# vocdoni/zk-franchise-proof-circuit

Hardware: AMD Instinct MI355X
Metric: zkCensus proofs/sec (nLevels=160) (higher is better)
Workload: dtype u256 (8 x u32 Montgomery, BN254 Fr/Fq)

## Files before the change

### include/zkcensus.h

```cpp
#ifndef ZKCENSUS_H
#define ZKCENSUS_H
#include <stddef.h>
#include <stdint.h>
#ifdef __cplusplus
extern "C" {
#endif

typedef struct zkc_ctx zkc_ctx;
typedef struct zkc_zkey zkc_zkey;

enum {
    ZKC_OK = 0,
    ZKC_ERR_GENERIC = 1,
    ZKC_ERR_SHORT_BUFFER = 2,
    ZKC_ERR_INVALID_WITNESS_LENGTH = 3,
    ZKC_ERR_BAD_ARG = 4,
    ZKC_ERR_FORMAT = 5,
    ZKC_ERR_HIP = 6,
    ZKC_ERR_WITNESS = 7
};
enum {
    ZKC_W_OK = 0, ZKC_W_ERR_WEIGHT = 1 , ZKC_W_ERR_SIK_ROOT = 2 ,
    ZKC_W_ERR_CENSUS_ROOT = 3 , ZKC_W_ERR_NULLIFIER = 4 , ZKC_W_ERR_LAST_SIBLING = 5 ,
    ZKC_W_ERR_INPUT_RANGE = 6 ,
// ... 70 lines not shown
int groth16_prover(const void* zkey_buffer, unsigned long zkey_size, const void* wtns_buffer, unsigned long wtns_size,
                   char* proof_buffer, unsigned long* proof_size, char* public_buffer, unsigned long* public_size,
                   char* error_msg, unsigned long error_msg_maxsize);

int groth16_fullprove(const void* zkey_buffer, unsigned long zkey_size, const void* wasm_buffer, unsigned long wasm_size, const char* inputs_json, unsigned long inputs_size,
                      char* proof_buffer, unsigned long* proof_size, char* public_buffer, unsigned long* public_size,
                      char* error_msg, unsigned long error_msg_maxsize);

int zkc_verify(const char* vkey_json, const char* public_json, const char* proof_json);
int zkc_verify_bin(const uint8_t* vk, int nPublic, const uint8_t* pub, const uint8_t* proof);

int zkc_pairing_bin(const uint8_t g1[64], const uint8_t g2[128], uint8_t out[384]);

int zkc_verify_batch(zkc_ctx* ctx, const uint8_t* vk, int nPublic, const uint8_t* pubs, const uint8_t* proofs, int N, const uint8_t* seed32);
const char* zkc_verify_last_error(void);

int zkc_proof_to_json(const uint8_t proof[256], const uint8_t* pub, int nPublic, char* proof_buf, unsigned long* proof_size,
                      char* public_buf, unsigned long* public_size);
int zkc_proof_from_json(const char* proof_json, const char* public_json, uint8_t proof[256], uint8_t* pub, int* nPublic);
int zkc_vkey_from_json(const char* vkey_json, uint8_t* vk, unsigned long* vk_size, int* nPublic);
int zkc_wtns_parse(const void* wtns_bytes, unsigned long size, const uint8_t** payload, uint32_t* nWitness);
unsigned long zkc_wtns_write(const void* payload, uint32_t nWitness, void* out, unsigned long out_size);

typedef struct zkc_msm zkc_msm;
int zkc_ntt_dev(zkc_ctx* ctx, const void* d_src, void* d_dst, int logn, int nvec, int inverse);
int zkc_g1_mul_batch_dev(zkc_ctx* ctx, const uint8_t base_std[64], const void* d_scalars, uint32_t n, void* d_out);
int zkc_msm_g1_load_dev(zkc_ctx* ctx, const void* d_bases_std, uint32_t n, zkc_msm** out);
int zkc_msm_g1_dev(zkc_msm* m, const void* d_scalars, uint8_t out[64]);
void zkc_msm_g1_free(zkc_msm* m);

int zkc_debug_stage(zkc_zkey* zk, const void* d_wtns, int stage, void* host_out);
unsigned long long zkc_debug_early_retries(void);
int zkc_msm_debug(zkc_zkey* zk, int which, const void* d_scalars, uint32_t count, void* host_out);
int zkc_debug_pairing_dev(zkc_ctx* ctx, const uint8_t* g1, const uint8_t* g2, const uint8_t* weights, int N, uint8_t product_out[384], uint8_t* folded_out,
                          int32_t* member_out, int* bad_out, const uint32_t* nodes, size_t count, uint8_t* node_out);

int zkc_poseidon_batch(zkc_ctx* ctx, int n_inputs, const void* inputs, size_t B, void* out);
int zkc_smt_build(zkc_ctx* ctx, const void* keys, const void* values, size_t n, int nLevels, uint8_t root[32], void* siblings, int32_t* depths);
int zkc_census_inputs(zkc_ctx* ctx, size_t n, int nLevels, const uint8_t election_id[64], const void* address, const void* password, const void* signature,
                      const void* available_weight, const void* vote_weight, const void* vote_hash, void* inputs_out, void* d_inputs_out, uint8_t* roots_out);

typedef struct zkc_tree zkc_tree;
enum {
    ZKC_TREE_OK = 0,
    ZKC_TREE_KEY_EXISTS = 1,
    ZKC_TREE_KEY_ABSENT = 2,
    ZKC_TREE_COLLISION = 3,
    ZKC_TREE_NOT_BELOW_R = 4,
    ZKC_TREE_NOT_IN_CENSUS = 5,
    ZKC_TREE_NOT_IN_SIK = 6,
    ZKC_TREE_SIK_MISMATCH = 7
};
int  zkc_tree_create(zkc_ctx* ctx, int nLevels, zkc_tree** out);
void zkc_tree_free(zkc_tree* tree);
int  zkc_tree_add(zkc_tree* tree, const void* keys, const void* values, size_t n, int32_t* status);
int  zkc_tree_update(zkc_tree* tree, const void* keys, const void* values, size_t n, int32_t* status);
int  zkc_tree_root(zkc_tree* tree, uint8_t root[32]);
int  zkc_tree_size(zkc_tree* tree, size_t* leaves);
int  zkc_tree_get(zkc_tree* tree, const void* keys, size_t n, void* values_out, int32_t* exists);
int  zkc_tree_gen_proof(zkc_tree* tree, const void* keys, size_t n, uint8_t root[32], void* siblings, int32_t* depths, int32_t* exists);
int  zkc_tree_census_inputs(zkc_tree* census, zkc_tree* sik, size_t n, const uint8_t election_id[64], const void* address, const void* password, const void* signature,
                            const void* vote_weight, const void* vote_hash, void* inputs_out, void* d_inputs_out, uint8_t roots_out[64], int32_t* status);
int  zkc_tree_stats(zkc_tree* tree, double ms[2]);

enum {
    ZKC_SMT_VALID = 0,
// ... 30 lines not shown
```

### zk-franchise-proof-circuit_amd/_native.py

```python
import ctypes
import os

_HERE = os.path.dirname(os.path.abspath(__file__))
LIB_PATH = os.environ.get('ZKCENSUS_LIB') or os.path.join(_HERE, 'libzkcensus.so')
_lib = None


class ZkcError(RuntimeError):
    def __init__(self, code, msg):
        super().__init__('libzkcensus error %d: %s' % (code, msg))
        self.code = code


def load():
    global _lib
    if _lib is not None:
        return _lib
    if not os.path.exists(LIB_PATH):
        raise ImportError('libzkcensus.so is not built (run `python -c "import __graft_entry__ as g; g.build()"`); '
                          'there is no CPU fallback for the product path')
    try:
        import torch
    except ImportError:
        pass
    L = ctypes.CDLL(LIB_PATH)
    vp, i32p = ctypes.c_void_p, ctypes.POINTER(ctypes.c_int32)
    L.zkc_ctx_create.argtypes = [ctypes.c_int, ctypes.POINTER(vp)]
    L.zkc_ctx_destroy.argtypes = [vp]
    L.zkc_last_error.argtypes = [vp]; L.zkc_last_error.restype = ctypes.c_char_p
    L.zkc_ctx_stream.argtypes = [vp]; L.zkc_ctx_stream.restype = vp
    L.zkc_witness.argtypes = [vp, ctypes.c_int, vp, ctypes.c_int, vp, i32p]
    L.zkc_witness_dev.argtypes = [vp, ctypes.c_int, vp, ctypes.c_int, vp, vp]
    u8p, u32p = ctypes.c_char_p, ctypes.POINTER(ctypes.c_uint32)
    L.zkc_zkey_load.argtypes = [vp, ctypes.c_char_p, ctypes.c_size_t, ctypes.POINTER(vp)]
    L.zkc_zkey_free.argtypes = [vp]; L.zkc_zkey_free.restype = None
    L.zkc_zkey_info.argtypes = [vp, u32p, u32p, u32p]
    L.zkc_zkey_pass_info.argtypes = [vp, ctypes.POINTER(ctypes.c_int), ctypes.POINTER(ctypes.c_int)]
    L.zkc_zkey_call_streams.argtypes = [vp, ctypes.POINTER(ctypes.c_int)]
    L.zkc_witness_status_text.argtypes = [ctypes.c_int, ctypes.c_int32]; L.zkc_witness_status_text.restype = ctypes.c_char_p
    L.zkc_prove.argtypes = [vp, ctypes.c_char_p, ctypes.c_uint32, u8p, u8p, ctypes.c_char_p, ctypes.c_char_p]
    L.zkc_prove_dev.argtypes = [vp, vp, ctypes.c_uint32, u8p, u8p, ctypes.c_char_p, ctypes.c_char_p]
    L.zkc_prove_batch_dev.argtypes = [vp, vp, ctypes.c_uint32, ctypes.c_int, ctypes.c_char_p, ctypes.c_char_p, ctypes.c_char_p]
    L.zkc_fullprove_batch_dev.argtypes = [vp, vp, ctypes.c_int, vp, vp, ctypes.c_char_p, ctypes.c_char_p, ctypes.c_char_p]
    L.zkc_debug_stage.argtypes = [vp, vp, ctypes.c_int, ctypes.c_char_p]
    L.zkc_debug_early_retries.argtypes = []; L.zkc_debug_early_retries.restype = ctypes.c_ulonglong
    L.zkc_msm_debug.argtypes = [vp, ctypes.c_int, vp, ctypes.c_uint32, ctypes.c_char_p]
    L.zkc_debug_pairing_dev.argtypes = [vp, ctypes.c_char_p, ctypes.c_char_p, ctypes.c_char_p, ctypes.c_int, ctypes.c_char_p, ctypes.c_char_p, i32p, ctypes.POINTER(ctypes.c_int),
                                        ctypes.POINTER(ctypes.c_uint32), ctypes.c_size_t, ctypes.c_char_p]
    ulp = ctypes.POINTER(ctypes.c_ulong)
    L.groth16_prover.argtypes = [ctypes.c_char_p, ctypes.c_ulong, ctypes.c_char_p, ctypes.c_ulong, ctypes.c_char_p, ulp, ctypes.c_char_p, ulp, ctypes.c_char_p, ctypes.c_ulong]
    L.zkc_verify.argtypes = [ctypes.c_char_p, ctypes.c_char_p, ctypes.c_char_p]
    L.zkc_verify_bin.argtypes = [ctypes.c_char_p, ctypes.c_int, ctypes.c_char_p, ctypes.c_char_p]
    L.zkc_verify_batch.argtypes = [vp, ctypes.c_char_p, ctypes.c_int, ctypes.c_char_p, ctypes.c_char_p, ctypes.c_int, ctypes.c_char_p]
    L.zkc_verify_batch_each.argtypes = [vp, ctypes.c_char_p, ctypes.c_int, ctypes.c_char_p, ctypes.c_char_p, ctypes.c_int, ctypes.c_char_p, i32p]
    L.zkc_verify_each_stats.argtypes = [vp, ctypes.POINTER(ctypes.c_uint64)]
    L.zkc_verify_last_error.restype = ctypes.c_char_p
    L.zkc_proof_to_json.argtypes = [ctypes.c_char_p, ctypes.c_char_p, ctypes.c_int, ctypes.c_char_p, ulp, ctypes.c_char_p, ulp]
    L.zkc_proof_from_json.argtypes = [ctypes.c_char_p, ctypes.c_char_p, ctypes.c_char_p, ctypes.c_char_p, ctypes.POINTER(ctypes.c_int)]
    L.zkc_vkey_from_json.argtypes = [ctypes.c_char_p, ctypes.c_char_p, ulp, ctypes.POINTER(ctypes.c_int)]
    L.zkc_wtns_parse.argtypes = [ctypes.c_char_p, ctypes.c_ulong, ctypes.POINTER(ctypes.c_void_p), ctypes.POINTER(ctypes.c_uint32)]
    L.zkc_wtns_write.argtypes = [ctypes.c_char_p, ctypes.c_uint32, ctypes.c_char_p, ctypes.c_ulong]; L.zkc_wtns_write.restype = ctypes.c_ulong
    L.zkc_poseidon_batch.argtypes = [vp, ctypes.c_int, ctypes.c_char_p, ctypes.c_size_t, ctypes.c_char_p]
    L.zkc_smt_build.argtypes = [vp, ctypes.c_char_p, ctypes.c_char_p, ctypes.c_size_t, ctypes.c_int, ctypes.c_char_p, ctypes.c_char_p, i32p]
    L.zkc_census_inputs.argtypes = [vp, ctypes.c_size_t, ctypes.c_int, ctypes.c_char_p, ctypes.c_char_p, ctypes.c_char_p, ctypes.c_char_p, ctypes.c_char_p, ctypes.c_char_p, ctypes.c_char_p, vp, vp, ctypes.c_char_p]
    sz = ctypes.c_size_t
    L.zkc_tree_create.argtypes = [vp, ctypes.c_int, ctypes.POINTER(vp)]
    L.zkc_tree_free.argtypes = [vp]; L.zkc_tree_free.restype = None
    L.zkc_tree_add.argtypes = [vp, ctypes.c_char_p, ctypes.c_char_p, sz, i32p]
    L.zkc_tree_update.argtypes = [vp, ctypes.c_char_p, ctypes.c_char_p, sz, i32p]
    L.zkc_tree_delete.argtypes = [vp, ctypes.c_char_p, sz, i32p]
    L.zkc_tree_refs.argtypes = [vp, ctypes.POINTER(sz)]
    L.zkc_tree_snapshot.argtypes = [vp, ctypes.POINTER(vp)]
    L.zkc_tree_snapshot_count.argtypes = [vp, ctypes.POINTER(sz)]
    L.zkc_tree_gen_absence_proof.argtypes = [vp, ctypes.c_char_p, sz, ctypes.c_char_p, vp, i32p, vp, vp, i32p, i32p]
    L.zkc_tree_root.argtypes = [vp, ctypes.c_char_p]
    L.zkc_tree_size.argtypes = [vp, ctypes.POINTER(sz)]
    L.zkc_tree_get.argtypes = [vp, ctypes.c_char_p, sz, vp, i32p]
    L.zkc_tree_gen_proof.argtypes = [vp, ctypes.c_char_p, sz, ctypes.c_char_p, vp, i32p, i32p]
    L.zkc_tree_census_inputs.argtypes = [vp, vp, sz, ctypes.c_char_p, ctypes.c_char_p, ctypes.c_char_p, ctypes.c_char_p, ctypes.c_char_p, ctypes.c_char_p, vp, vp, ctypes.c_char_p, i32p]
# ... 88 lines not shown
```

### zk-franchise-proof-circuit_amd/csrc/zkc_fold.hip

```cpp
#include "zkc_prover.h"
#include "zkc_host_util.h"
#include "zkc_kernels.h"
#include <ctime>
#include <cstdio>
#include <algorithm>

using namespace zkc;

extern "C" __global__ void __launch_bounds__(64)
zkc_fold_check(WitnessLayout L, const uint32_t* __restrict__ wtns, const uint32_t* __restrict__ tmpl, uint32_t* __restrict__ flags, int B, int stride) {
    const int n = L.n, g = blockIdx.x, tree = blockIdx.y, b = blockIdx.z;
    const int blk = tree == 0 ? L.off_census : L.off_sikver;
    int start, end;
    if (g < n - 1) {
        const int nctrl = (g == n - 3) + (g > 0 && g < n - 2) + 1;
        start = blk + L.lvl_off(g) + nctrl; end = blk + (g + 1 < n - 1 ? L.lvl_off(g + 1) : L.lvl_off(n - 1));
    } else { start = blk + L.off_n2bold; end = start + 253 + 127 + 133; }
    const uint4* w = reinterpret_cast<const uint4*>(wtns + (size_t)b * L.nWires * 8) + 2 * (size_t)start;
    const uint4* t = reinterpret_cast<const uint4*>(tmpl) + 2 * (size_t)start;
    uint32_t diff = 0;
    for (int i = threadIdx.x; i < 2 * (end - start); i += 64) { uint4 x = w[i], y = t[i]; diff |= (x.x ^ y.x) | (x.y ^ y.y) | (x.z ^ y.z) | (x.w ^ y.w); }
    if (g == n - 1 && tree == 0 && threadIdx.x < 2) {
        const uint4 x = reinterpret_cast<const uint4*>(wtns + (size_t)b * L.nWires * 8)[threadIdx.x], y = reinterpret_cast<const uint4*>(tmpl)[threadIdx.x];
        diff |= (x.x ^ y.x) | (x.y ^ y.y) | (x.z ^ y.z) | (x.w ^ y.w);
    }
    const unsigned long long any = __ballot(diff != 0);
    if (threadIdx.x == 0) flags[(size_t)b * stride + (size_t)tree * n + g] = any ? 1u : 0u;
}

extern "C" __global__ void __launch_bounds__(256)
zkc_top_check(TopCheckArgs a, const uint32_t* __restrict__ wtns, uint32_t* __restrict__ flags, int stride, int off) {
    __shared__ uint32_t s_valid;
    const int tree = blockIdx.x, b = blockIdx.y;
    const uint32_t* w = wtns + (size_t)b * a.nWires * 8;
    uint32_t h = 2166136261u;
// ... 215 lines not shown
    zkc_ctx* ctx = zk->ctx; const uint32_t nv = zk->nVars, np = zk->nPub;
    std::vector<uint32_t> v; zkc_zkey::Fold::VMap m;
    m.offA = 0; for (uint32_t w = 0; w < nv; w++) if (!zk->fold.infA[w]) v.push_back(w); m.nA = (uint32_t)v.size();
    m.offB = (uint32_t)v.size(); for (uint32_t w = 0; w < nv; w++) if (!zk->fold.infB[w]) v.push_back(w); m.nB = (uint32_t)v.size() - m.offB;
    m.offC = (uint32_t)v.size(); for (uint32_t w = np + 1; w < nv; w++) if (!zk->fold.infC[w]) v.push_back(w); m.nC = (uint32_t)v.size() - m.offC;
    if ((size_t)m.nA + m.nB + m.nC + (size_t)nv / 50 < 3 * (size_t)nv - np - 1) {
        if (int rc = list_upload(ctx, v, ctx->stream, &m.d)) return rc;
    }
    zk->fold.vmaps[{-1, -1, -1, -1}] = m; *out = m;
    return ZKC_OK;
}

int zkc::abc_template(zkc_zkey* zk, const uint32_t* tmpl) {
    if (zk->fold.d_abc_tmpl) return ZKC_OK;
    zkc_ctx* ctx = zk->ctx; const uint32_t n = zk->n; Fr *d_abc = nullptr, *d_wm = nullptr; int rc;
    if ((rc = dmalloc(ctx, &d_abc, 3 * (size_t)n))) return rc;
    if ((rc = dmalloc(ctx, &d_wm, 3 * (size_t)n))) { (void)hipFree(d_abc); return rc; }
    matvec_launch(zk, d_abc, d_wm, tmpl, 1, ctx->stream);
    hipError_t e = hipGetLastError(); if (e == hipSuccess) e = hipStreamSynchronize(ctx->stream);
    (void)hipFree(d_wm);
    if (e != hipSuccess) { (void)hipFree(d_abc); return zkc_fail(ctx, ZKC_ERR_HIP, std::string("abc_template: ") + hipGetErrorString(e)); }
    zk->fold.d_abc_tmpl = d_abc;
    return ZKC_OK;
}
int zkc::abc_rows(zkc_zkey* zk, int Dc, int Ds, zkc_zkey::Fold::AbcRows* out) {
    auto& f = zk->fold;
    auto it = f.abc_rows.find({Dc, Ds});
    if (it != f.abc_rows.end()) { *out = it->second; return ZKC_OK; }
    zkc_ctx* ctx = zk->ctx;
    const abc::VoterRows v = abc::voter_rows(f.abc_cls, f.abc_perm.data(), zk->nlong, zk->n, f.abc_rowptr.data(), f.abc_col.data(), zk->nVars, Dc, Ds);
    zkc_zkey::Fold::AbcRows m; m.nrows = (uint32_t)v.rows.size(); m.nlong = v.nlong; m.offC = m.nrows; m.nC = (uint32_t)v.crows.size(); m.offW = m.offC + m.nC; m.nW = (uint32_t)v.wires.size();
    std::vector<uint32_t> all(v.rows); all.insert(all.end(), v.crows.begin(), v.crows.end()); all.insert(all.end(), v.wires.begin(), v.wires.end());
    if (int rc = list_upload(ctx, all, ctx->stream, &m.d)) return rc;
    if (sw::on<sw::ZKC_TRACE_HOST>()) fprintf(stderr, "[zkc host] abc rows at depths (%d, %d): %u of %zu A/B rows listed (%u long), %u C rows, %u wires\n", Dc, Ds, m.nrows, f.abc_cls.size(), m.nlong, m.nC, m.nW);
    f.abc_rows[{Dc, Ds}] = m; *out = m;
    return ZKC_OK;
}
void zkc::fold_free(zkc_zkey* zk) {
    for (auto& kv : zk->fold.vmaps) if (kv.second.d) (void)hipFree(kv.second.d);
    for (auto& kv : zk->fold.abc_rows) if (kv.second.d) (void)hipFree(kv.second.d);
    if (zk->fold.d_abc_tmpl) (void)hipFree(zk->fold.d_abc_tmpl);
    { auto& tp = zk->fold.top; for (void* q : {(void*)tp.d_copy[0], (void*)tp.d_copy[1], (void*)tp.d_valid, (void*)tp.d_A, (void*)tp.d_B1, (void*)tp.d_C, (void*)tp.d_B2}) if (q) (void)hipFree(q); }
    for (void* q : {(void*)zk->fold.d_foldA, (void*)zk->fold.d_foldB1, (void*)zk->fold.d_foldC, (void*)zk->fold.d_foldB2}) if (q) (void)hipFree(q);
}
```

### zk-franchise-proof-circuit_amd/csrc/zkc_kernels.h

```cpp
#pragma once
#include "zkc_field.h"
#include "zkc_curve.h"
#include "zkc_device.h"
#include "zkc_jds.h"

namespace zkc {

__device__ __forceinline__ Fr ld_fr(const Fr* p) {
    const uint4* d = reinterpret_cast<const uint4*>(p); uint4 a = d[0], b = d[1];
    Fr r; r.v[0] = a.x; r.v[1] = a.y; r.v[2] = a.z; r.v[3] = a.w; r.v[4] = b.x; r.v[5] = b.y; r.v[6] = b.z; r.v[7] = b.w; return r;
}
__device__ __forceinline__ void st_fr(Fr* p, const Fr& r) {
    uint4* d = reinterpret_cast<uint4*>(p);
    d[0] = make_uint4(r.v[0], r.v[1], r.v[2], r.v[3]); d[1] = make_uint4(r.v[4], r.v[5], r.v[6], r.v[7]);
}
__device__ __forceinline__ Fr mv_term(const Fr* __restrict__ val, const Fr* __restrict__ w, const Fr* __restrict__ wm, uint32_t idx, uint32_t c) {
    if (wm && (c & MV_UNIT)) { const Fr x = ld_fr(wm + (c & MV_COL)); return (c & MV_NEG) ? fp_neg(x) : x; }
    return ld_fr(val + idx) * ld_fr(w + (c & MV_COL));
}

extern "C" __global__ void zkc_wtns_mont(const Fr* wtns_std, size_t wtns_stride, Fr* wm, size_t wm_stride, uint32_t nv);
extern "C" __global__ void zkc_wtns_mont_list(const Fr* wtns_std, size_t wtns_stride, Fr* wm, size_t wm_stride, const uint32_t* list, uint32_t nlist);
extern "C" __global__ void zkc_abc_fill(const uint4* tmpl, uint4* abc, uint32_t per);
extern "C" __global__ void zkc_matvec_jds(const uint32_t* perm, const uint32_t* rowlen, const uint32_t* jdptr, const uint32_t* col, const Fr* val, const Fr* wtns_std,
                                          size_t wtns_stride, Fr* abc, int n, uint32_t nlong, const Fr* wm_all, size_t wm_stride, const uint32_t* list, uint32_t nrows);
extern "C" __global__ void zkc_pointwise_mul(Fr* abc, int n, const uint32_t* list, uint32_t count);
extern "C" __global__ void zkc_join_abc(const Fr* abc, uint32_t* p_std, int n);

struct TopCheckArgs;
extern "C" __global__ void zkc_fold_check(WitnessLayout L, const uint32_t* wtns, const uint32_t* tmpl, uint32_t* flags, int B, int stride);
extern "C" __global__ void zkc_top_check(TopCheckArgs a, const uint32_t* wtns, uint32_t* flags, int stride, int off);
extern "C" __global__ void zkc_input_depths(const uint32_t* inputs, int nInputs, int n, uint32_t* out);

extern "C" __global__ void zkc_witness_chains(WitnessLayout L, PoseidonTable tab, const uint32_t* inputs, uint32_t* wtns, int32_t* status, int B, int tmpl_mode);
extern "C" __global__ void zkc_witness_chains_wave(WitnessLayout L, PoseidonTable tab, const uint32_t* inputs, uint32_t* wtns, int32_t* status, int B, int tmpl_mode);
extern "C" __global__ void zkc_witness_fill(const uint4* tmpl, uint4* wtns, int nWires, int B);
extern "C" __global__ void zkc_witness_tostd(uint32_t* wtns, size_t nwires_total);
extern "C" __global__ void zkc_poseidon_batch_kernel(PoseidonTable tab, const uint32_t* in, uint32_t* out, int nin, size_t B);

extern "C" __global__ void zkc_census_hash(PoseidonTable tab, int kind, const uint32_t* a, const uint32_t* b, const uint32_t* c, uint32_t* out, size_t n);
extern "C" __global__ void zkc_tree_leaves(PoseidonTable tab, const uint32_t* slot, const uint32_t* key, const uint32_t* value, uint32_t count, uint32_t* val);
extern "C" __global__ void zkc_tree_level(PoseidonTable tab, const uint32_t* trip, uint32_t count, uint32_t* val);
extern "C" __global__ void zkc_tree_narrow(PoseidonTable tab, const uint32_t* trip, const uint32_t* off, uint32_t ndepths, uint32_t count, uint32_t* val);
extern "C" __global__ void zkc_census_scatter(const uint32_t* val, const uint2* pairs, size_t count, uint32_t* out);
extern "C" __global__ void zkc_census_scalars(const uint32_t* eid, const uint32_t* nullifier, const uint32_t* avail, const uint32_t* vhash, const uint32_t* sik_root,
                                              const uint32_t* census_root, const uint32_t* address, const uint32_t* password, const uint32_t* signature,
                                              const uint32_t* vweight, size_t n, int nIn, uint32_t* out);

extern "C" __global__ void zkc_smt_check(PoseidonTable tab, const uint32_t* keys, const uint32_t* values, const uint32_t* roots, uint32_t root_stride, const uint32_t* off,
                                         const uint32_t* sib, uint32_t count, int32_t* status);
extern "C" __global__ void zkc_smt_check_wave(PoseidonTable tab, const uint32_t* keys, const uint32_t* values, const uint32_t* roots, uint32_t root_stride,
                                              const uint32_t* off, const uint32_t* sib, uint32_t count, int32_t* status);
extern "C" __global__ void zkc_smt_check_absent(PoseidonTable tab, const uint32_t* keys, const uint32_t* old_keys, const uint32_t* values, const uint32_t* old0,
                                                const uint32_t* roots, uint32_t root_stride, const uint32_t* off, const uint32_t* sib, uint32_t count, int32_t* status);
extern "C" __global__ void zkc_smt_check_absent_wave(PoseidonTable tab, const uint32_t* keys, const uint32_t* old_keys, const uint32_t* values, const uint32_t* old0,
                                                     const uint32_t* roots, uint32_t root_stride, const uint32_t* off, const uint32_t* sib, uint32_t count, int32_t* status);

extern "C" __global__ void zkc_r1cs_range(const Fr* wtns_std, size_t wtns_stride, uint32_t nWires, uint32_t* flag);
extern "C" __global__ void zkc_r1cs_check_rows(const uint4* rows, const uint32_t* jdptr, const uint32_t* col, const Fr* val, const Fr* wtns_std, size_t wtns_stride,
                                               const Fr* wm_all, size_t wm_stride, uint32_t nCons, uint32_t nlong, uint32_t* first, uint32_t* count, const uint32_t* flag);
// ... 3 lines not shown
```

### zk-franchise-proof-circuit_amd/csrc/zkc_msm.hip

```cpp
#include <cstdio>
#include <cstddef>
#include <ctime>
#include <cstdlib>
#include <cstring>
#include <string.h>
#include <vector>
#include "zkc_prover.h"
#include "zkc_f29.h"
#include "zkc_f29_g1.h"
#include "zkc_f29_g2.h"
#include "zkc_point_ops.h"

namespace zkc {

template <class F> struct PointIO;
template <class PP> struct PointIO<Fp<PP>> {
    typedef Fp<PP> Fq;
    static __device__ __forceinline__ Affine<Fq> load(const Affine<Fq>* p) {
        const uint4* d = reinterpret_cast<const uint4*>(p); uint4 a = d[0], b = d[1], c = d[2], e = d[3];
        Affine<Fq> r;
        r.x.v[0] = a.x; r.x.v[1] = a.y; r.x.v[2] = a.z; r.x.v[3] = a.w; r.x.v[4] = b.x; r.x.v[5] = b.y; r.x.v[6] = b.z; r.x.v[7] = b.w;
        r.y.v[0] = c.x; r.y.v[1] = c.y; r.y.v[2] = c.z; r.y.v[3] = c.w; r.y.v[4] = e.x; r.y.v[5] = e.y; r.y.v[6] = e.z; r.y.v[7] = e.w;
        return r;
    }
// ... 381 lines not shown
        if (!b.is_inf()) Sk = f29g2_pt_from_xyzz(b);
    }
    sh[threadIdx.x] = Sk; __syncthreads();
    for (int o = 1; o < nt; o <<= 1) {
        Acc29G2 v; f29g2_pt_set_inf(v);
        if ((int)threadIdx.x + o < nt) v = sh[threadIdx.x + o];
        __syncthreads();
        if ((int)threadIdx.x + o < nt) { Acc29G2 t = sh[threadIdx.x]; f29g2_pt_add(t, t, v); sh[threadIdx.x] = t; }
        __syncthreads();
    }
    Acc29G2 y; f29g2_pt_set_inf(y);
    if (threadIdx.x >= 1 && (int)threadIdx.x < nt) { y = sh[threadIdx.x]; if (!f29g2_pt_is_inf(y)) for (uint32_t k = vw; k > 1; k >>= 1) f29g2_pt_dbl(y, y); }
    f29g2_pt_add(y, y, Wk);
    __syncthreads();
    sh[threadIdx.x] = y; __syncthreads();
    for (int st = nt / 2; st > 0; st >>= 1) {
        if ((int)threadIdx.x < st) { Acc29G2 t = sh[threadIdx.x]; f29g2_pt_add(t, t, sh[threadIdx.x + st]); sh[threadIdx.x] = t; }
        __syncthreads();
    }
    if (threadIdx.x == 0) results[j] = f29g2_pt_is_inf(sh[0]) ? XYZZ<Fq2>::inf() : f29g2_pt_to_xyzz(sh[0]);
}

template <class F>
__global__ void __launch_bounds__(128)
zkc_msm_shift_bases(const Affine<F>* __restrict__ prev, Affine<F>* __restrict__ next, uint32_t count, int c) {
    const uint32_t i = blockIdx.x * blockDim.x + threadIdx.x;
    if (i >= count) return;
    Affine<F> a = PointIO<F>::load(prev + i);
    XYZZ<F> p = xyzz_dbl_affine(a);
    for (int k = 1; k < c; k++) p = xyzz_dbl(p);
    next[i] = xyzz_to_affine(p);
}
template <class F>
static int precompute(zkc_ctx* ctx, uint32_t count, Affine<F>* d_table, int c) {
    for (int w = 1; w < msm_nw(c); w++) {
        hipLaunchKernelGGL(HIP_KERNEL_NAME(zkc_msm_shift_bases<F>), dim3((count + 127) / 128), dim3(128), 0, ctx->stream,
                           d_table + (size_t)(w - 1) * count, d_table + (size_t)w * count, count, c);
        hipError_t e = hipGetLastError();
        if (e != hipSuccess) return zkc_fail(ctx, ZKC_ERR_HIP, std::string("zkc_msm_shift_bases: ") + hipGetErrorString(e));
    }
    return ZKC_OK;
}
int msm_precompute_g1(zkc_ctx* ctx, uint32_t count, G1Affine* d_table, int c) { return precompute<Fq>(ctx, count, d_table, c); }
int msm_precompute_g2(zkc_ctx* ctx, uint32_t count, G2Affine* d_table, int c) { return precompute<Fq2>(ctx, count, d_table, c); }
int msm_g2_rows29(zkc_ctx* ctx, const G2Affine* d_points, size_t n, const char* what, uint32_t** out) {
    DevBuf rows; int rc;
    if ((rc = rows.alloc(ctx, n * G2ROW_WORDS * sizeof(uint32_t))) || (rc = msm_g2_table29(ctx, d_points, rows.as<uint32_t>(), n))) return rc;
    const hipError_t e = hipStreamSynchronize(ctx->stream);
    if (e != hipSuccess) return zkc_fail(ctx, ZKC_ERR_HIP, std::string(what) + ": " + hipGetErrorString(e));
    *out = (uint32_t*)rows.release();
    return ZKC_OK;
}
int msm_g2_window_table29(zkc_ctx* ctx, const G2Affine* d_bases, uint32_t count, int c, const char* what, uint32_t** out) {
    const size_t n = (size_t)msm_nw(c) * count;
    DevBuf shifted; int rc;
    if ((rc = shifted.alloc(ctx, n * sizeof(G2Affine)))) return rc;
    const hipError_t e = hipMemcpyAsync(shifted.p, d_bases, (size_t)count * sizeof(G2Affine), hipMemcpyDeviceToDevice, ctx->stream);
    if (e != hipSuccess) return zkc_fail(ctx, ZKC_ERR_HIP, std::string(what) + ": " + hipGetErrorString(e));
    if ((rc = msm_precompute_g2(ctx, count, shifted.as<G2Affine>(), c))) return rc;
    return msm_g2_rows29(ctx, shifted.as<G2Affine>(), n, what, out);
}

__device__ __forceinline__ uint32_t limb_of(const uint32_t k[8], int i) {
    uint32_t w = 0;
#pragma unroll
    for (int q = 0; q < 8; q++) w = (q == i) ? k[q] : w;
    return w;
}
template <class F>
__global__ void __launch_bounds__(64)
zkc_fold_mul(const Affine<F>* __restrict__ tbl, const uint32_t* __restrict__ scalars, const uint32_t* __restrict__ wires, uint32_t nw,
             int32_t pt_shift, XYZZ<F>* __restrict__ out, uint32_t pt_mod) {
    const uint32_t i = blockIdx.x * blockDim.x + threadIdx.x;
    if (i >= nw) return;
    const uint32_t wire = wires[i];
    const uint4* sp = reinterpret_cast<const uint4*>(scalars + 8 * (size_t)wire); uint4 a = sp[0], b = sp[1];
// ... 8 lines not shown
        if ((limb_of(k, bit >> 5) >> (bit & 31)) & 1) r = xyzz_add_affine(r, p);
    }
    out[i] = r;
}
template <class F>
__global__ void __launch_bounds__(64)
zkc_fold_gsum(const XYZZ<F>* __restrict__ in, const uint32_t* __restrict__ gstart, uint32_t ngroups, XYZZ<F>* __restrict__ out) {
    const uint32_t g = blockIdx.x * blockDim.x + threadIdx.x;
    if (g >= ngroups) return;
    XYZZ<F> acc = XYZZ<F>::inf();
    for (uint32_t i = gstart[g], e = gstart[g + 1]; i < e; i++) acc = xyzz_add(acc, in[i]);
    out[g] = acc;
}
template <class F>
static int fold_group_sums_ws(zkc_ctx* ctx, const Affine<F>* tbl, const uint32_t* d_scalars, const uint32_t* d_wires, uint32_t nw, int32_t pt_shift,
                              const uint32_t* d_gstart, uint32_t ngroups, XYZZ<F>* tmp, XYZZ<F>* out, XYZZ<F>* h_out, uint32_t pt_mod, hipStream_t st) {
    hipLaunchKernelGGL(HIP_KERNEL_NAME(zkc_fold_mul<F>), dim3((nw + 63) / 64), dim3(64), 0, st, tbl, d_scalars, d_wires, nw, pt_shift, tmp, pt_mod);
    ZKC_HIP_CHECK(ctx, hipGetLastError());
    hipLaunchKernelGGL(HIP_KERNEL_NAME(zkc_fold_gsum<F>), dim3((ngroups + 63) / 64), dim3(64), 0, st, tmp, d_gstart, ngroups, out);
    ZKC_HIP_CHECK(ctx, hipGetLastError());
    ZKC_HIP_CHECK(ctx, hipMemcpyAsync(h_out, out, (size_t)ngroups * sizeof(XYZZ<F>), hipMemcpyDeviceToHost, st));
    ZKC_HIP_CHECK(ctx, hipStreamSynchronize(st));
    return ZKC_OK;
}
template <class F>
static int fold_group_sums(zkc_ctx* ctx, const Affine<F>* tbl, const uint32_t* d_scalars, const uint32_t* d_wires, uint32_t nw, int32_t pt_shift,
                           const uint32_t* d_gstart, uint32_t ngroups, XYZZ<F>* h_out, uint32_t pt_mod, hipStream_t st) {
    DevBuf tmp, out; int rc;
    if ((rc = tmp.alloc(ctx, (size_t)nw * sizeof(XYZZ<F>))) || (rc = out.alloc(ctx, (size_t)ngroups * sizeof(XYZZ<F>)))) return rc;
    return fold_group_sums_ws<F>(ctx, tbl, d_scalars, d_wires, nw, pt_shift, d_gstart, ngroups, tmp.as<XYZZ<F>>(), out.as<XYZZ<F>>(), h_out, pt_mod, st ? st : ctx->stream);
}
int fold_group_sums_g1(zkc_ctx* ctx, const G1Affine* tbl, const uint32_t* s, const uint32_t* w, uint32_t nw, int32_t sh, const uint32_t* gs, uint32_t ng, G1XYZZ* o, uint32_t pt_mod, hipStream_t st) {
    return fold_group_sums<Fq>(ctx, tbl, s, w, nw, sh, gs, ng, o, pt_mod, st);
}
int fold_group_sums_g1_ws(zkc_ctx* ctx, const G1Affine* tbl, const uint32_t* s, const uint32_t* w, uint32_t nw, const uint32_t* gs, uint32_t ng, G1XYZZ* d_tmp, G1XYZZ* d_out, G1XYZZ* h_out) {
    return fold_group_sums_ws<Fq>(ctx, tbl, s, w, nw, 0, gs, ng, d_tmp, d_out, h_out, 0u, ctx->stream);
}
int fold_group_sums_g2(zkc_ctx* ctx, const G2Affine* tbl, const uint32_t* s, const uint32_t* w, uint32_t nw, int32_t sh, const uint32_t* gs, uint32_t ng, G2XYZZ* o, uint32_t pt_mod, hipStream_t st) {
    return fold_group_sums<Fq2>(ctx, tbl, s, w, nw, sh, gs, ng, o, pt_mod, st);
}

static int msm_work_alloc_impl(zkc_ctx* ctx, MsmWork& w, size_t max_entries, size_t max_buckets, int max_jobs, bool g2) {
    w.max_entries = max_entries; w.max_jobs = max_jobs; w.max_buckets = max_buckets; w.xyzz_size = g2 ? sizeof(G2XYZZ) : sizeof(G1XYZZ);
    const size_t nb = max_buckets;
    w.max_segments = std::max<size_t>(max_entries / MSM_SEG + 1, (size_t)32 * 8192) + nb + 64;
    w.max_bins = (size_t)max_jobs << MSM_MAX_HBITS;
    ZKC_HIP_CHECK(ctx, hipMalloc((void**)&w.vals, max_entries * 4 + 16)); ZKC_HIP_CHECK(ctx, hipMalloc((void**)&w.vals2, max_entries * 4 + 16));
    ZKC_HIP_CHECK(ctx, hipMalloc((void**)&w.hist, w.max_bins * 4)); ZKC_HIP_CHECK(ctx, hipMalloc((void**)&w.bin_start, w.max_bins * 4));
    w.max_tilecnt = max_entries / 8 + ((size_t)max_jobs << MSM_MAX_HBITS);
    ZKC_HIP_CHECK(ctx, hipMalloc((void**)&w.tilecnt, w.max_tilecnt * 4));
    ZKC_HIP_CHECK(ctx, hipMalloc((void**)&w.off, (nb + 2) * 4)); ZKC_HIP_CHECK(ctx, hipMalloc((void**)&w.bcnt, (nb + 2) * 4)); ZKC_HIP_CHECK(ctx, hipMalloc((void**)&w.segcnt, (nb + 2) * 4));
    ZKC_HIP_CHECK(ctx, hipMalloc((void**)&w.segoff, (nb + 2) * 4)); ZKC_HIP_CHECK(ctx, hipMalloc((void**)&w.seg2bucket, w.max_segments * 4));
    ZKC_HIP_CHECK(ctx, hipMalloc((void**)&w.seglen, w.max_segments * 4)); ZKC_HIP_CHECK(ctx, hipMalloc((void**)&w.perm, w.max_segments * 4));
    w.max_lencnt = (size_t)(MSM_SEG + 1) * (w.max_segments / 256 + 2);
    ZKC_HIP_CHECK(ctx, hipMalloc((void**)&w.lencnt, w.max_lencnt * 4));
    ZKC_HIP_CHECK(ctx, hipMalloc((void**)&w.scan_blk, (std::max(nb + 2, w.max_lencnt) / 1024 + 2) * 4));
    ZKC_HIP_CHECK(ctx, hipMalloc((void**)&w.heavy, (MSM_MAX_HEAVY + 1) * 4));
    ZKC_HIP_CHECK(ctx, hipMalloc((void**)&w.d_jobs, sizeof(MsmJobList)));
    ZKC_HIP_CHECK(ctx, hipMalloc(&w.partial, w.max_segments * w.xyzz_size));
    const size_t max_vw = max_buckets / MSM_VW_MIN + (size_t)max_jobs;
    ZKC_HIP_CHECK(ctx, hipMalloc(&w.wres, 2 * max_vw * w.xyzz_size));
    ZKC_HIP_CHECK(ctx, hipMalloc((void**)&w.d_windows, max_vw * sizeof(MsmWindow))); w.max_windows = max_vw;
    w.max_tiles = max_entries / (8 * MSM_TILE_SCALARS) + (size_t)max_jobs + 1;
    ZKC_HIP_CHECK(ctx, hipMalloc((void**)&w.d_tilejob, w.max_tiles * 2));
    for (int s = 0; s < 2; s++) {
        ZKC_HIP_CHECK(ctx, hipHostMalloc((void**)&w.h_tilejob[s], w.max_tiles * 2));
// ... 22 lines not shown
static const bool g_debug_sync = sw::on<sw::ZKC_DEBUG_SYNC>();
#define ZKC_LAUNCH_CHECK(ctx, name)                                                                        \
    do { hipError_t _e = hipGetLastError(); if (_e != hipSuccess)                                          \
        return zkc_fail((ctx), ZKC_ERR_HIP, std::string(name ": ") + hipGetErrorString(_e));               \
        if (g_debug_sync) { timespec _t0, _t1; clock_gettime(CLOCK_MONOTONIC, &_t0);                        \
            _e = hipStreamSynchronize(st); clock_gettime(CLOCK_MONOTONIC, &_t1);                \
            fprintf(stderr, "[zkc] %-22s %8.3f ms  %s\n", name, (_t1.tv_sec - _t0.tv_sec) * 1e3 + (_t1.tv_nsec - _t0.tv_nsec) * 1e-6, \
                    hipGetErrorString(_e)); fflush(stderr); } } while (0)

template <class F>
static int msm_pass(zkc_zkey* zk, MsmWork& w, const Affine<F>* table, const MsmJobList& jl_in, int slot, bool to_host, hipStream_t st, hipEvent_t ev_sorted, hipEvent_t wait_before_acc = nullptr, hipEvent_t ev_acc = nullptr,
                    hipStream_t st_red = nullptr, hipEvent_t ev_red = nullptr) {
    zkc_ctx* ctx = zk->ctx;
    const int nj = jl_in.njobs;
    if (nj <= 0 || nj > w.max_jobs) return zkc_fail(ctx, ZKC_ERR_BAD_ARG, "msm_pass: job count");
    static thread_local MsmJobList jl;
    jl = jl_in;
    if (!jl.finish()) {
        std::string d = "msm_pass: jobs need at most two window sizes (the larger first) and tables that fit the entry word [" + std::to_string(nj) + " jobs:";
        for (int j = 0; j < nj && j < 16; j++) d += " c" + std::to_string(jl.job[j].c) + "/" + std::to_string(jl.job[j].count) + "/" + std::to_string(jl.job[j].tbl_count);
        return zkc_fail(ctx, ZKC_ERR_BAD_ARG, d + "]");
    }
    const size_t total = jl.total_entries;
    const uint32_t nb = jl.total_buckets;
    if (total > w.max_entries || nb > w.max_buckets) return zkc_fail(ctx, ZKC_ERR_BAD_ARG, "msm_pass: too many entries for the work space");
    const uint32_t seg = (uint32_t)std::min<size_t>(MSM_SEG, std::max<size_t>(MSM_SEG_MIN, total / 131072));
    typedef typename GroupOf<F>::Ops G; constexpr bool kG2 = GroupOf<F>::g2;
    const uint32_t bw_slices = (uint32_t)std::min<size_t>(32, w.max_segments / std::max<uint32_t>(nb, 1u));
    const uint32_t* const g2_table29 = (kG2 && jl.job[0].c == (uint32_t)MSM_C_G2_LONE) ? zk->d_g2_29_lone : (kG2 && zk->c_deep && jl.job[0].c == (uint32_t)zk->c_deep) ? zk->d_g2_29_deep : zk->d_g2_29;
    const bool bucket_wave = kG2 && sw::on<sw::ZKC_G2_BUCKET_WAVE>() && nb <= 8192 && bw_slices >= 1;
    uint64_t alg_bytes = 0; uint32_t maxcount = 0;
    uint64_t streamed_bytes = 0;
    for (int j = 0; j < nj; j++) {
        alg_bytes += (uint64_t)jl.job[j].tbl_count * (sizeof(Affine<F>) + 32);
        streamed_bytes += (uint64_t)jl.job[j].count * (sizeof(Affine<F>) + 32);
        maxcount = std::max(maxcount, jl.job[j].count);
    }
    const size_t seg_bound = total / seg + nb;
    if (!bucket_wave && seg_bound > w.max_segments) return zkc_fail(ctx, ZKC_ERR_BAD_ARG, "msm_pass: more segments than the work space holds");
    {
        zkc_prof_scope _ps(ctx, ZKC_PROF_MSM_SORT, 0, st);
        if (jl.total_windows > w.max_windows) return zkc_fail(ctx, ZKC_ERR_BAD_ARG, "msm_pass: too many virtual windows for the work space");
        const int hs = w.h_next; w.h_next ^= 1;
        ZKC_HIP_CHECK(ctx, zkc_wait_event(w.h_ev[hs]));
        MsmWindow* wins = w.h_windows[hs]; uint32_t nwin = 0;
        for (int j = 0; j < nj; j++) for (uint32_t k = 0; k < (uint32_t)msm_half((int)jl.job[j].c) / jl.job[j].vw; k++)
            wins[nwin++] = MsmWindow{jl.id_of(k * jl.job[j].vw, (uint32_t)j), jl.job[j].win_off + k, jl.job[j].vw / 64};
        memcpy(w.h_jobs[hs], &jl, offsetof(MsmJobList, job) + (size_t)nj * sizeof(MsmJob)); w.h_jobs[hs]->njobs = jl.njobs;
        memcpy(&w.h_jobs[hs]->njobs, &jl.njobs, sizeof(MsmJobList) - offsetof(MsmJobList, njobs));
        ZKC_HIP_CHECK(ctx, hipMemcpyAsync(w.d_jobs, w.h_jobs[hs], sizeof(MsmJobList), hipMemcpyHostToDevice, st));
        ZKC_HIP_CHECK(ctx, hipMemcpyAsync(w.d_windows, wins, (size_t)nwin * sizeof(MsmWindow), hipMemcpyHostToDevice, st));
        if (jl.total_tiles > w.max_tiles) return zkc_fail(ctx, ZKC_ERR_BAD_ARG, "msm_pass: too many tiles for the work space");
        { uint16_t* tj = w.h_tilejob[hs]; uint32_t k = 0; for (int j = 0; j < nj; j++) { const uint32_t nt = (jl.job[j].count + MSM_TILE_SCALARS - 1) / MSM_TILE_SCALARS; for (uint32_t i = 0; i < nt; i++) tj[k++] = (uint16_t)j; } }
        ZKC_HIP_CHECK(ctx, hipMemcpyAsync(w.d_tilejob, w.h_tilejob[hs], (size_t)jl.total_tiles * 2, hipMemcpyHostToDevice, st));
        ZKC_HIP_CHECK(ctx, hipEventRecord(w.h_ev[hs], st));
        unsigned long long* ectr = (!kG2 && ((ctx->prof.mask >> ZKC_PROF_MSM_ACC_G1) & 1)) ? ctx->d_prof_entries : nullptr;
        int rc = msm_bucket_entries(ctx, w, jl, st, ectr); if (rc) return rc;
        if (g_debug_sync) { hipError_t _e = hipStreamSynchronize(st); fprintf(stderr, "[zkc] bucket entries: %s\n", hipGetErrorString(_e)); }
        if (!bucket_wave) { rc = msm_build_segments(ctx, w, jl, seg, seg_bound, st); if (rc) return rc; }
        if (g_debug_sync) { hipError_t _e = hipStreamSynchronize(st); fprintf(stderr, "[zkc] segments: %s\n", hipGetErrorString(_e)); }
        if (ev_sorted) ZKC_HIP_CHECK(ctx, hipEventRecord(ev_sorted, st));
    }
    XYZZ<F>* partial = reinterpret_cast<XYZZ<F>*>(w.partial);
    XYZZ<F>* wres = reinterpret_cast<XYZZ<F>*>(w.wres);
    XYZZ<F>* results = reinterpret_cast<XYZZ<F>*>(w.results) + (size_t)slot * w.max_jobs;
    if (wait_before_acc) ZKC_HIP_CHECK(ctx, hipStreamWaitEvent(st, wait_before_acc, 0));
    const bool acc_chain = !kG2 && sw::on<sw::ZKC_ACC_CHAIN>() && total >= ((size_t)1 << 22);
// ... 66 lines not shown
```

### zk-franchise-proof-circuit_amd/csrc/zkc_ntt.hip

```cpp
#include "zkc_internal.h"
#include "zkc_prover.h"
#include "zkc_f29.h"
#include "zkc_host_util.h"
#include "zkc_kernels.h"

namespace zkc {

extern "C" __global__ void __launch_bounds__(256)
zkc_wtns_mont(const Fr* __restrict__ wtns_std, size_t wtns_stride, Fr* __restrict__ wm, size_t wm_stride, uint32_t nv) {
    const uint32_t i = blockIdx.x * blockDim.x + threadIdx.x;
    if (i >= nv) return;
    Fr r2;
#pragma unroll
    for (int k = 0; k < 8; k++) r2.v[k] = FrParams::r2[k];
    st_fr(wm + (size_t)blockIdx.y * wm_stride + i, ld_fr(wtns_std + (size_t)blockIdx.y * wtns_stride + i) * r2);
}
extern "C" __global__ void __launch_bounds__(256)
zkc_wtns_mont_list(const Fr* __restrict__ wtns_std, size_t wtns_stride, Fr* __restrict__ wm, size_t wm_stride, const uint32_t* __restrict__ list, uint32_t nlist) {
    const uint32_t e = blockIdx.x * blockDim.x + threadIdx.x;
    if (e >= nlist) return;
    const uint32_t i = list[e];
    Fr r2;
#pragma unroll
    for (int k = 0; k < 8; k++) r2.v[k] = FrParams::r2[k];
    st_fr(wm + (size_t)blockIdx.y * wm_stride + i, ld_fr(wtns_std + (size_t)blockIdx.y * wtns_stride + i) * r2);
}
extern "C" __global__ void __launch_bounds__(256)
zkc_abc_fill(const uint4* __restrict__ tmpl, uint4* __restrict__ abc, uint32_t per) {
    uint4* __restrict__ dst = abc + (size_t)blockIdx.y * per;
    for (uint32_t i = blockIdx.x * blockDim.x + threadIdx.x; i < per; i += gridDim.x * blockDim.x) dst[i] = tmpl[i];
}
extern "C" __global__ void __launch_bounds__(256)
zkc_matvec_jds(const uint32_t* __restrict__ perm, const uint32_t* __restrict__ rowlen, const uint32_t* __restrict__ jdptr,
               const uint32_t* __restrict__ col, const Fr* __restrict__ val, const Fr* __restrict__ wtns_std, size_t wtns_stride,
               Fr* __restrict__ abc, int n, uint32_t nlong, const Fr* __restrict__ wm_all, size_t wm_stride, const uint32_t* __restrict__ list, uint32_t nrows) {
    const uint32_t t = blockIdx.x * blockDim.x + threadIdx.x, lane = threadIdx.x & 63u;
    const Fr* __restrict__ w = wtns_std + (size_t)blockIdx.y * wtns_stride;
    const Fr* __restrict__ wm = wm_all ? wm_all + (size_t)blockIdx.y * wm_stride : nullptr;
    Fr acc = Fr::zero();
    if ((t >> 6) < nlong) {
        const uint32_t r = list ? list[t >> 6] : t >> 6, len = rowlen[r];
        for (uint32_t k = lane; k < len; k += 64) { const uint32_t idx = jdptr[k] + r; acc = acc + mv_term(val, w, wm, idx, col[idx]); }
        for (int d = 32; d > 0; d >>= 1) {
            Fr o;
#pragma unroll
            for (int i = 0; i < 8; i++) o.v[i] = (uint32_t)__shfl_down((int)acc.v[i], d, 64);
            acc = acc + o;
        }
        if (lane == 0) st_fr(abc + (size_t)blockIdx.y * 3 * n + perm[r], acc);
        return;
    }
    const uint32_t e = t - nlong * 63u;
    if (e >= nrows) return;
    const uint32_t r = list ? list[e] : e;
    const uint32_t len = rowlen[r];
    for (uint32_t k = 0; k < len; k++) { const uint32_t idx = jdptr[k] + r; acc = acc + mv_term(val, w, wm, idx, col[idx]); }
    st_fr(abc + (size_t)blockIdx.y * 3 * n + perm[r], acc);
}
extern "C" __global__ void __launch_bounds__(256)
zkc_pointwise_mul(Fr* __restrict__ abc, int n, const uint32_t* __restrict__ list, uint32_t count) {
    const uint32_t e = blockIdx.x * blockDim.x + threadIdx.x;
    Fr* a = abc + (size_t)blockIdx.y * 3 * n;
    if (e >= count) return;
    const uint32_t i = list ? list[e] : e;
    st_fr(a + 2 * (size_t)n + i, ld_fr(a + i) * ld_fr(a + n + i));
}
struct JoinDom { static constexpr L9 D27 = f29_dominator<FrParams>(1u << 29, 1u << 27); };
extern "C" __global__ void __launch_bounds__(256)
zkc_join_abc(const Fr* __restrict__ abc, uint32_t* __restrict__ p_std, int n) {
    const int i = blockIdx.x * blockDim.x + threadIdx.x;
    if (i >= n) return;
    const Fr* a = abc + (size_t)blockIdx.y * 3 * n;
    const Fr av = ld_fr(a + i), bv = ld_fr(a + n + i), cv = ld_fr(a + 2 * (size_t)n + i);
    uint32_t A[9], B[9], C[9], T[9];
    f29_from_fp_shl5(A, av.v); f29_from_fp_shl5(B, bv.v); f29_from_fp_shl5(C, cv.v);
#pragma unroll
    for (int k = 0; k < 9; k++) C[k] = JoinDom::D27.l[k] - C[k];
    f29_mul_addhi<FrParams>(T, A, B, C);
    uint64_t col[18];
#pragma unroll
    for (int k = 0; k < 9; k++) { col[k] = T[k]; col[9 + k] = 0; }
    f29_reduce_cols<FrParams>(T, col);
    Fr r;
    r.v[0] = f29_word<0>(T); r.v[1] = f29_word<32>(T); r.v[2] = f29_word<64>(T); r.v[3] = f29_word<96>(T);
    r.v[4] = f29_word<128>(T); r.v[5] = f29_word<160>(T); r.v[6] = f29_word<192>(T); r.v[7] = f29_word<224>(T);
    fp_reduce_once<FrParams>(r.v);
    uint4* d = reinterpret_cast<uint4*>(p_std + 8 * ((size_t)blockIdx.y * n + i));
    d[0] = make_uint4(r.v[0], r.v[1], r.v[2], r.v[3]); d[1] = make_uint4(r.v[4], r.v[5], r.v[6], r.v[7]);
}

constexpr int NTT_TILE = 1024;
constexpr int TW29_WORDS = 12;
extern "C" __global__ void __launch_bounds__(256) zkc_tw29(const Fr* __restrict__ tw, uint32_t* __restrict__ out, uint32_t count) {
    const uint32_t i = blockIdx.x * blockDim.x + threadIdx.x;
    if (i >= count) return;
    const Fr x = ld_fr(tw + i);
    uint32_t t[9], r[9]; f29_from_fp_shl5(t, x.v); f29_mul<FrParams>(r, t, F29K<FrParams>::one.l);
    uint4* o = reinterpret_cast<uint4*>(out + (size_t)TW29_WORDS * i);
    o[0] = make_uint4(r[0], r[1], r[2], r[3]); o[1] = make_uint4(r[4], r[5], r[6], r[7]); o[2] = make_uint4(r[8], 0, 0, 0);
}
struct NttDom { static constexpr L9 D24 = f29_dominator<FrParams>(1u << 29, 1u << 24); static constexpr L9 D27 = f29_dominator<FrParams>(1u << 29, 1u << 27); };
__device__ __forceinline__ void ntt_ld_w(uint32_t w[9], const uint32_t* __restrict__ tw29, size_t e) {
    const uint4* wp = reinterpret_cast<const uint4*>(tw29 + (size_t)TW29_WORDS * e);
    const uint4 w0 = wp[0], w1 = wp[1], w2 = wp[2];
    w[0] = w0.x; w[1] = w0.y; w[2] = w0.z; w[3] = w0.w; w[4] = w1.x; w[5] = w1.y; w[6] = w1.z; w[7] = w1.w; w[8] = w2.x;
}
__device__ __forceinline__ void ntt_bfly(uint32_t* pu, uint32_t* pv, const uint32_t w[9], bool plain, bool carry) {
    uint32_t u[9], v[9], tt[9];
#pragma unroll
    for (int i = 0; i < 9; i++) { u[i] = pu[i]; v[i] = pv[i]; }
    if (plain) {
#pragma unroll
        for (int i = 0; i < 9; i++) { const uint32_t vi = v[i]; v[i] = u[i] + NttDom::D27.l[i] - vi; u[i] += vi; }
    } else {
        f29_mul<FrParams>(tt, v, w);
#pragma unroll
        for (int i = 0; i < 9; i++) { v[i] = u[i] + NttDom::D24.l[i] - tt[i]; u[i] += tt[i]; }
    }
    if (carry) { f29_carry(u); f29_carry(v); }
#pragma unroll
    for (int i = 0; i < 9; i++) { pu[i] = u[i]; pv[i] = v[i]; }
}
__device__ __forceinline__ void ntt_r4(uint32_t* p0, uint32_t* p1, uint32_t* p2, uint32_t* p3, const uint32_t wa[9], const uint32_t wb[9], const uint32_t wc[9], bool swap_mid) {
    uint32_t a[9], b[9], c[9], d[9], t[9];
#pragma unroll
    for (int i = 0; i < 9; i++) { a[i] = p0[i]; b[i] = p1[i]; c[i] = p2[i]; d[i] = p3[i]; }
    f29_mul<FrParams>(t, b, wa);
#pragma unroll
    for (int i = 0; i < 9; i++) { b[i] = a[i] + NttDom::D24.l[i] - t[i]; a[i] += t[i]; }
    f29_mul<FrParams>(t, d, wa);
#pragma unroll
    for (int i = 0; i < 9; i++) { d[i] = c[i] + NttDom::D24.l[i] - t[i]; c[i] += t[i]; }
    f29_mul<FrParams>(t, c, wb);
#pragma unroll
    for (int i = 0; i < 9; i++) { c[i] = a[i] + NttDom::D24.l[i] - t[i]; a[i] += t[i]; }
    f29_mul<FrParams>(t, d, wc);
#pragma unroll
    for (int i = 0; i < 9; i++) { d[i] = b[i] + NttDom::D24.l[i] - t[i]; b[i] += t[i]; }
    f29_carry(a); f29_carry(b); f29_carry(c); f29_carry(d);
    (void)swap_mid;
#pragma unroll
    for (int i = 0; i < 9; i++) { p0[i] = a[i]; p1[i] = b[i]; p2[i] = c[i]; p3[i] = d[i]; }
}
extern "C" __global__ void __launch_bounds__(256)
zkc_ntt_pass(const Fr* src_all, Fr* dst_all, const uint32_t* __restrict__ tw29, const Fr* __restrict__ scale,
             int logn, int s0, int b, int first) {
    const Fr* src = src_all + ((size_t)blockIdx.y << logn);
    Fr* dst = dst_all + ((size_t)blockIdx.y << logn);
    extern __shared__ uint32_t tile[];
    const int mid_n = 1 << b;
    const int lo_bits = s0;
    const int lo_t = (NTT_TILE >> b) < (1 << lo_bits) ? (NTT_TILE >> b) : (1 << lo_bits);
    const int tiles_per_hi = (1 << lo_bits) / lo_t;
    const int hi = blockIdx.x / tiles_per_hi, lo0 = (blockIdx.x % tiles_per_hi) * lo_t;
    const int elems = mid_n * lo_t;
    const size_t base = (size_t)hi << (s0 + b);
    for (int e = threadIdx.x; e < elems; e += blockDim.x) {
        const int mid = e / lo_t, l = e - mid * lo_t;
        size_t gi = base + ((size_t)mid << s0) + lo0 + l;
        if (first) gi = __brev((unsigned)gi) >> (32 - logn);
        const Fr x = ld_fr(src + gi);
        uint32_t t[9]; f29_from_fp_shl5(t, x.v);
#pragma unroll
        for (int k = 0; k < 9; k++) tile[9 * e + k] = t[k];
    }
    __syncthreads();
    int t = 1;
    auto single = [&](int t1, bool carry) {
        const int half = 1 << (t1 - 1);
        const int s = s0 + t1;
        for (int q = threadIdx.x; q < elems / 2; q += blockDim.x) {
            const int l = q % lo_t, pr = q / lo_t;
            const int j = pr & (half - 1), blk = pr >> (t1 - 1);
            const int m0 = (blk << t1) + j, m1 = m0 + half;
            const unsigned k = ((unsigned)j << s0) + lo0 + l;
            uint32_t w[9]; ntt_ld_w(w, tw29, (size_t)k << (logn - s));
            ntt_bfly(tile + 9 * (m0 * lo_t + l), tile + 9 * (m1 * lo_t + l), w, s == 1, carry);
        }
        __syncthreads();
    };
    if (s0 == 0) { single(1, true); t = 2; }
// ... 38 lines not shown
            uint32_t w[9] = {0, 0, 0, 0, 0, 0, 0, 0, 0};
            ntt_bfly(tile + 9 * slot(j, l), tile + 9 * slot(j + span, l), w, true, true);
        }
        __syncthreads();
        r = 1;
    }
    for (; RADIX >= 4 && r + 1 < b; r += 2) {
        const int q = q0 + r, span = mid_n >> (r + 1), hspan = span >> 1, units = (mid_n >> 2) * lo_t;
        for (int x = threadIdx.x; x < units; x += blockDim.x) {
            const int l = x % lo_t, u = x / lo_t;
            const int blk = u / hspan, j = u - blk * hspan;
            const int m = blk * 2 * span + j;
            const uint32_t i = ((prefix_of_l0 + (uint32_t)(prefix_per_l * l)) << r) | (uint32_t)blk;
            uint32_t wa[9], wb[9], wc[9];
            ntt_ld_w(wa, tw29, tw_of(q, i)); ntt_ld_w(wb, tw29, tw_of(q + 1, 2 * i)); ntt_ld_w(wc, tw29, tw_of(q + 1, 2 * i + 1));
            ntt_r4(tile + 9 * slot(m, l), tile + 9 * slot(m + span, l), tile + 9 * slot(m + hspan, l), tile + 9 * slot(m + span + hspan, l), wa, wb, wc, false);
        }
        __syncthreads();
    }
    for (; r < b; r++) {
        const int q = q0 + r, span = mid_n >> (r + 1), pairs = (mid_n >> 1) * lo_t;
        for (int x = threadIdx.x; x < pairs; x += blockDim.x) {
            const int l = x % lo_t, pr = x / lo_t;
            const int blk = pr / span, j = pr - blk * span;
            const int m0 = blk * 2 * span + j;
            const uint32_t i = ((prefix_of_l0 + (uint32_t)(prefix_per_l * l)) << r) | (uint32_t)blk;
            uint32_t w[9]; ntt_ld_w(w, tw29, tw_of(q, i));
            ntt_bfly(tile + 9 * slot(m0, l), tile + 9 * slot(m0 + span, l), w, false, RADIX >= 4 || (r & 1) == 1 || r == b - 1);
        }
        __syncthreads();
    }
}
template <int RADIX>
__device__ __forceinline__ void ntt_nr_head_body(const Fr* src_all, Fr* dst_all, const uint32_t* __restrict__ tw29, int logn, int q0, int b) {
    const Fr* src = src_all + ((size_t)blockIdx.y << logn);
    Fr* dst = dst_all + ((size_t)blockIdx.y << logn);
    extern __shared__ uint32_t tile[];
    const int mid_n = 1 << b, sh = logn - q0 - b, lo_t = NTT_TILE >> b, elems = mid_n * lo_t;
    const int bpp = (1 << sh) / lo_t;
    const uint32_t prefix = blockIdx.x / bpp;
    const size_t base = ((size_t)prefix << (logn - q0)) + (size_t)(blockIdx.x % bpp) * lo_t;
    for (int e = threadIdx.x; e < elems; e += blockDim.x) {
        const int mid = e / lo_t, l = e - mid * lo_t;
        const Fr x = ld_fr(src + (base + ((size_t)mid << sh) + l));
        uint32_t t[9]; f29_from_fp_shl5(t, x.v);
#pragma unroll
        for (int k = 0; k < 9; k++) tile[9 * e + k] = t[k];
    }
    __syncthreads();
    ntt_nr_stages<RADIX>(tile, [lo_t](int mid, int l) { return mid * lo_t + l; }, b, lo_t, q0, prefix, 0, tw29, logn, q0 == 0);
    for (int e = threadIdx.x; e < elems; e += blockDim.x) {
        const int mid = e / lo_t, l = e - mid * lo_t;
        uint32_t r[9];
#pragma unroll
        for (int k = 0; k < 9; k++) r[k] = tile[9 * e + k];
        f29_reduce_small<FrParams>(r);
        st_fr(dst + (base + ((size_t)mid << sh) + l), f29_to_fp<FrParams>(r));
    }
}
extern "C" __global__ void __launch_bounds__(256)
zkc_ntt_nr_head(const Fr* src_all, Fr* dst_all, const uint32_t* __restrict__ tw29, int logn, int q0, int b) { ntt_nr_head_body<1>(src_all, dst_all, tw29, logn, q0, b); }
extern "C" __global__ void __launch_bounds__(256)
zkc_ntt_nr_head_r4(const Fr* src_all, Fr* dst_all, const uint32_t* __restrict__ tw29, int logn, int q0, int b) { ntt_nr_head_body<4>(src_all, dst_all, tw29, logn, q0, b); }
extern "C" __global__ void __launch_bounds__(256)
zkc_ntt_mid(Fr* __restrict__ data_all, const uint32_t* __restrict__ tw_inv29, const uint32_t* __restrict__ tw_fwd29, const Fr* __restrict__ scale_br, int logn) {
    Fr* __restrict__ data = data_all + ((size_t)blockIdx.y << logn);
    extern __shared__ uint32_t tile[];
    constexpr int B = 9, MID = 1 << B, NSUB = NTT_TILE / MID;
    const size_t base = (size_t)blockIdx.x * NTT_TILE;
    for (int e = threadIdx.x; e < NTT_TILE; e += blockDim.x) {
        const Fr x = ld_fr(data + base + e);
        uint32_t t[9]; f29_from_fp_shl5(t, x.v);
#pragma unroll
        for (int k = 0; k < 9; k++) tile[9 * e + k] = t[k];
    }
    __syncthreads();
    ntt_nr_stages<4>(tile, [](int mid, int l) { return l * MID + mid; }, B, NSUB, logn - B, (uint32_t)blockIdx.x * NSUB, 1, tw_inv29, logn, false);
    for (int e = threadIdx.x; e < NTT_TILE; e += blockDim.x) {
        uint32_t r[9], s29[9], o[9];
#pragma unroll
        for (int k = 0; k < 9; k++) r[k] = tile[9 * e + k];
        const Fr sc = ld_fr(scale_br + base + e);
        f29_from_fp_shl5(s29, sc.v); f29_mul<FrParams>(o, r, s29);
#pragma unroll
        for (int k = 0; k < 9; k++) tile[9 * e + k] = o[k];
    }
    __syncthreads();
    for (int x = threadIdx.x; x < NTT_TILE / 2; x += blockDim.x) {
        const int l = x / (MID / 2), pr = x - l * (MID / 2);
        uint32_t w[9] = {0, 0, 0, 0, 0, 0, 0, 0, 0};
        ntt_bfly(tile + 9 * (l * MID + 2 * pr), tile + 9 * (l * MID + 2 * pr + 1), w, true, true);
    }
    __syncthreads();
    for (int t = 2; t + 1 <= B; t += 2) {
        const int half = 1 << (t - 1);
        for (int x = threadIdx.x; x < NTT_TILE / 4; x += blockDim.x) {
            const int l = x / (MID / 4), u = x - l * (MID / 4);
            const int j = u & (half - 1), blk = u >> (t - 1);
            const int m = (blk << (t + 1)) + j;
            uint32_t wa[9], wb[9], wc[9];
            ntt_ld_w(wa, tw_fwd29, (size_t)j << (logn - t)); ntt_ld_w(wb, tw_fwd29, (size_t)j << (logn - t - 1)); ntt_ld_w(wc, tw_fwd29, (size_t)(j + half) << (logn - t - 1));
            uint32_t* p = tile + 9 * (l * MID + m);
            ntt_r4(p, p + 9 * half, p + 9 * 2 * half, p + 9 * 3 * half, wa, wb, wc, false);
        }
        __syncthreads();
    }
    for (int e = threadIdx.x; e < NTT_TILE; e += blockDim.x) {
        uint32_t r[9];
#pragma unroll
        for (int k = 0; k < 9; k++) r[k] = tile[9 * e + k];
        f29_reduce_small<FrParams>(r);
        st_fr(data + base + e, f29_to_fp<FrParams>(r));
    }
}
extern "C" __global__ void __launch_bounds__(256)
zkc_bitrev_copy(const Fr* __restrict__ src, Fr* __restrict__ dst, int logn) {
    const uint32_t i = blockIdx.x * blockDim.x + threadIdx.x;
    if (i >> logn) return;
    st_fr(dst + i, ld_fr(src + (__brev(i) >> (32 - logn))));
}
int ntt_bitrev_table(zkc_ctx* ctx, const Fr* d_src, Fr** out, int logn) {
    ZKC_HIP_CHECK(ctx, hipMalloc((void**)out, sizeof(Fr) << logn));
    hipLaunchKernelGGL(zkc_bitrev_copy, dim3(((1u << logn) + 255) / 256), dim3(256), 0, ctx->stream, d_src, *out, logn);
    ZKC_HIP_CHECK(ctx, hipGetLastError());
    return ZKC_OK;
}
int ntt_pair_run(zkc_ctx* ctx, hipStream_t st, Fr* data, const uint32_t* tw_inv29, const uint32_t* tw_fwd29, const Fr* scale_br, int logn, int nvec) {
    if (logn < 12 || logn > 27) return zkc_fail(ctx, ZKC_ERR_BAD_ARG, "ntt_pair_run: 12 <= logn <= 27");
    const int bh = logn - 9;
    const int b1 = bh <= 9 ? bh : (bh + 1) / 2, b2 = bh - b1;
    const unsigned blocks = (1u << logn) / NTT_TILE;
    const int radix = (int)sw::value<sw::ZKC_NTT_RADIX>(4);
    auto head = radix >= 4 ? zkc_ntt_nr_head_r4 : zkc_ntt_nr_head;
    hipLaunchKernelGGL(head, dim3(blocks, nvec), dim3(256), (size_t)NTT_TILE * 36, st, (const Fr*)data, data, tw_inv29, logn, 0, b1);
    if (b2) hipLaunchKernelGGL(head, dim3(blocks, nvec), dim3(256), (size_t)NTT_TILE * 36, st, (const Fr*)data, data, tw_inv29, logn, b1, b2);
    hipLaunchKernelGGL(zkc_ntt_mid, dim3(blocks, nvec), dim3(256), (size_t)NTT_TILE * 36, st, data, tw_inv29, tw_fwd29, scale_br, logn);
    hipLaunchKernelGGL(zkc_ntt_pass, dim3(blocks, nvec), dim3(256), (size_t)NTT_TILE * 36, st, (const Fr*)data, data, tw_fwd29, (const Fr*)nullptr, logn, 9, b1, 0);
    if (b2) hipLaunchKernelGGL(zkc_ntt_pass, dim3(blocks, nvec), dim3(256), (size_t)NTT_TILE * 36, st, (const Fr*)data, data, tw_fwd29, (const Fr*)nullptr, logn, 9 + b1, b2, 0);
    hipError_t e = hipGetLastError();
    if (e != hipSuccess) return zkc_fail(ctx, ZKC_ERR_HIP, std::string("ntt_pair_run: ") + hipGetErrorString(e));
    return ZKC_OK;
}

int ntt_make_tw29(zkc_ctx* ctx, const Fr* d_tw, uint32_t count, uint32_t** out) {
    ZKC_HIP_CHECK(ctx, hipMalloc((void**)out, (size_t)count * TW29_WORDS * 4));
    hipLaunchKernelGGL(zkc_tw29, dim3((count + 255) / 256), dim3(256), 0, ctx->stream, d_tw, *out, count);
    ZKC_HIP_CHECK(ctx, hipGetLastError());
    ZKC_HIP_CHECK(ctx, hipStreamSynchronize(ctx->stream));
    return ZKC_OK;
}

int ntt_twiddle_tables(zkc_ctx* ctx, int logn, bool keep_fr, TwiddleTables* out, bool with_29) {
    const uint32_t half = 1u << (logn - 1);
    const Fr w = fr_root_of_unity(logn), wi = fp_inv<FrParams>(w);
    std::vector<Fr> f(half), b(half);
    f[0] = b[0] = Fr::one(); for (uint32_t i = 1; i < half; i++) { f[i] = f[i - 1] * w; b[i] = b[i - 1] * wi; }
    DevBuf d_f, d_b, d_f29, d_b29; int rc;
    if ((rc = d_f.alloc(ctx, half * sizeof(Fr))) || (rc = d_b.alloc(ctx, half * sizeof(Fr)))) return rc;
    ZKC_HIP_CHECK(ctx, hipMemcpy(d_f.p, f.data(), half * sizeof(Fr), hipMemcpyHostToDevice));
    ZKC_HIP_CHECK(ctx, hipMemcpy(d_b.p, b.data(), half * sizeof(Fr), hipMemcpyHostToDevice));
    if (with_29 && ((rc = ntt_make_tw29(ctx, d_f.as<Fr>(), half, (uint32_t**)&d_f29.p)) || (rc = ntt_make_tw29(ctx, d_b.as<Fr>(), half, (uint32_t**)&d_b29.p)))) return rc;
    out->fwd29 = (uint32_t*)d_f29.release(); out->inv29 = (uint32_t*)d_b29.release();
    out->fwd = keep_fr ? (Fr*)d_f.release() : nullptr; out->inv = keep_fr ? (Fr*)d_b.release() : nullptr;
    return ZKC_OK;
}

int ntt_run(zkc_ctx* ctx, hipStream_t st, const Fr* src, Fr* dst, const uint32_t* tw29, const Fr* scale, int logn, int nvec) {
    int s0 = 0; bool first = true;
    while (s0 < logn) {
        int b = logn - s0 < 9 ? logn - s0 : 9;
        if (logn - s0 > 9 && logn - s0 < 18) b = (logn - s0 + 1) / 2;
        if (b > 9) b = 9;
        const int lo_t = (NTT_TILE >> b) < (1 << s0) ? (NTT_TILE >> b) : (1 << s0);
        const int nblocks = (1 << logn) / ((1 << b) * lo_t);
        const bool last = s0 + b == logn;
        hipLaunchKernelGGL(zkc_ntt_pass, dim3(nblocks, nvec), dim3(256), (size_t)(1 << b) * lo_t * 36, st,
                           first ? src : dst, dst, tw29, last ? scale : nullptr, logn, s0, b, first ? 1 : 0);
        hipError_t e = hipGetLastError();
        if (e != hipSuccess) return zkc_fail(ctx, ZKC_ERR_HIP, std::string("zkc_ntt_pass: ") + hipGetErrorString(e));
        s0 += b; first = false;
    }
    return ZKC_OK;
}

}
```

### zk-franchise-proof-circuit_amd/csrc/zkc_pass_plan.h

```cpp
#pragma once
#include "zkc_top_fold.h"
#include <cstddef>
#include <cstdint>
#include <vector>

namespace zkc {
constexpr int MSM_C_G2_LONE = 8;
constexpr int msm_nw(int c) { return (254 + c) / c; }
constexpr int msm_half(int c) { return 1 << (c - 1); }

namespace plan {

struct CallSplit { int npasses, per_pass; };
inline CallSplit call_split(int B, int max_inflight) {
    const int npasses = (B + max_inflight - 1) / max_inflight;
    return {npasses, (B + npasses - 1) / npasses};
}

constexpr int FOREIGN = -1;
inline int row_depth(const uint32_t* f, int n) {
    if (f[n - 1]) return FOREIGN;
    int D = 0; for (int g = 0; g < n - 1; g++) if (f[g]) D = g + 1;
    return D;
}
// ... 36 lines not shown
};
struct PassShape {
    uint32_t vws, vwb, vw_g2;
    bool deep; int cw;
    uint32_t oA, oB1, oC;
    int c2;
    bool tree; int per;
};
template <class Lists> inline PassShape pass_shape(const KeyShape& k, int nb, const Lists* lists, const LaneCaps& cap, const Switches& s) {
    const uint32_t nv = k.nv, nc = nv - k.np - 1;
    PassShape p;
    p.vws = nb <= 4 ? 64u : s.vw_small ? s.vw_small : nb < 32 ? 256u : 2048u; p.vwb = nb <= 4 ? 256u : s.vw_big ? s.vw_big : nb < 32 ? 1024u : 4096u;
    size_t lone_entries = 0; for (int q = 0; q < nb; q++) lone_entries += (size_t)msm_nw(MSM_C_G2_LONE) * (lists ? lists[q].nB : nv);
    size_t live_wires = 0; for (int q = 0; q < nb; q++) live_wires += lists ? (size_t)lists[q].nA + lists[q].nB + lists[q].nC : 2 * (size_t)nv + nc;
    p.deep = k.c_deep != 0 && nb > 2 && live_wires >= 3 * s.deep_wires * (size_t)nb;
    p.cw = p.deep ? k.c_deep : k.c_sec;
    p.oA = p.deep ? k.offA_deep : k.offA; p.oB1 = p.deep ? k.offB1_deep : k.offB1; p.oC = p.deep ? k.offC_deep : k.offC;
    p.c2 = (nb <= 2 && k.lone_table && lone_entries <= cap.w2_entries) ? MSM_C_G2_LONE : p.cw;
    p.vw_g2 = p.c2 == MSM_C_G2_LONE ? 128u : (s.vw_g2 && nb >= 32) ? s.vw_g2 : p.vws;
    size_t tree_entries = 0; for (int q = 0; q < nb; q++) tree_entries += (size_t)msm_nw(k.c_h) * k.n + (size_t)msm_nw(k.c_sec) * (lists ? 2 * (size_t)lists[q].nA + 2 * (size_t)lists[q].nB + lists[q].nC : 4 * (size_t)nv + nc);
    p.tree = k.fb4 && nb <= 2 && 6 * nb <= cap.w1_jobs && tree_entries <= cap.w1_entries && (size_t)nb * (5 * msm_half(k.c_sec) + msm_half(k.c_h)) <= cap.w1_buckets;
    p.per = p.tree ? 5 : 3;
    return p;
}

struct SectionView { const uint32_t* scalars; const uint32_t* vmap; uint32_t count, tbl_off, tbl_count; int32_t pt_shift; };
struct ProofViews { SectionView A, B1, C; };
template <class Lists> inline ProofViews proof_views(const KeyShape& k, const PassShape& p, const uint32_t* w, const Lists* vm) {
    const uint32_t nv = k.nv, np = k.np, nc = nv - np - 1;
    if (vm) return {{w, vm->d + vm->offA, vm->nA, p.oA, nv, 0}, {w, vm->d + vm->offB, vm->nB, p.oB1, nv, 0}, {w, vm->d + vm->offC, vm->nC, p.oC, nc, (int32_t)np + 1}};
    return {{w, nullptr, nv, p.oA, nv, 0}, {w, nullptr, nv, p.oB1, nv, 0}, {w + 8ull * (np + 1), nullptr, nc, p.oC, nc, 0}};
}

struct StreamOrder {
    bool mv_prefetch;
    bool mv_done;
    bool g2_acc_with_sort;
    bool red_split;
    bool blind_on_st;
};
inline StreamOrder stream_order(int nb, bool one_lane, int pass, int npasses, int lane0, bool tree, const Switches& s) {
    StreamOrder o;
    o.mv_prefetch = !s.matvec_inline && one_lane;
    o.mv_done = o.mv_prefetch && pass > 0;
    o.g2_acc_with_sort = s.g2_acc_hold || ((nb < 32 || !one_lane) && !s.g2_acc_early);
    o.red_split = s.reduce_stream && !s.serial_streams && nb >= 32;
    o.blind_on_st = (tree || lane0 >= 0) && npasses == 1;
    return o;
}

enum LaneStream { ON_ST = 0, ON_ST2 = 1, ON_FIN = 2, ON_RED = 3 };
struct LaneRoles {
    int g1;
    int g2;
    int blind;
    int red;
    int streams;
};
inline LaneRoles lane_roles(int nb, bool one_lane, int pass, int npasses, int lane0, bool tree, int lanes, const Switches& s) {
    const StreamOrder o = stream_order(nb, one_lane, pass, npasses, lane0, tree, s);
    const bool rotates = !one_lane && lanes > 1;
    const int want = !rotates ? 3 : (s.lane_streams >= 1 && s.lane_streams <= 3) ? s.lane_streams : 1;
    LaneRoles r;
    r.g1 = ON_ST;
    r.g2 = want >= 2 ? ON_ST2 : ON_ST;
    r.blind = (o.blind_on_st || want <= 2) ? ON_ST : ON_FIN;
// ... 7 lines not shown
```

### zk-franchise-proof-circuit_amd/csrc/zkc_prove.hip

```cpp
#include "zkc_prover.h"
#include "zkc_fixedbase.h"
#include "zkc_hostparse.h"
#include "zkc_host_util.h"
#include "zkc_kernels.h"
#include "zkc_f29_g2.h"
#include <cstring>
#include <ctime>
#include <cstdio>
#include <algorithm>
#include <atomic>

using namespace zkc;

void zkc::matvec_launch(zkc_zkey* zk, Fr* d_abc, Fr* d_wm, const uint32_t* d_wtns0, int nb, hipStream_t mv, const zkc_zkey::Fold::AbcRows* al) {
    const uint32_t n = zk->n, nv = zk->nVars;
    const bool units = zk->n_unit_coeffs > 0 && nv <= 3 * (size_t)n && sw::on<sw::ZKC_MATVEC_UNITS>();
    const Fr* wm = units ? (const Fr*)d_wm : (const Fr*)nullptr;
    if (al) {
        const uint32_t per = 6 * n;
        hipLaunchKernelGGL(zkc_abc_fill, dim3((per + 1023) / 1024, nb), dim3(256), 0, mv, (const uint4*)zk->fold.d_abc_tmpl, (uint4*)d_abc, per);
        if (units && al->nW) hipLaunchKernelGGL(zkc_wtns_mont_list, dim3((al->nW + 255) / 256, nb), dim3(256), 0, mv, (const Fr*)d_wtns0, (size_t)nv, d_wm, 3 * (size_t)n, al->d + al->offW, al->nW);
        if (al->nrows) hipLaunchKernelGGL(zkc_matvec_jds, dim3((al->nrows + 63 * al->nlong + 255) / 256, nb), dim3(256), 0, mv, zk->d_perm, zk->d_rowlen, zk->d_jdptr, zk->d_col, zk->d_val,
                                          (const Fr*)d_wtns0, (size_t)nv, d_abc, (int)n, al->nlong, wm, 3 * (size_t)n, (const uint32_t*)al->d, al->nrows);
        if (al->nC) hipLaunchKernelGGL(zkc_pointwise_mul, dim3((al->nC + 255) / 256, nb), dim3(256), 0, mv, d_abc, (int)n, (const uint32_t*)(al->d + al->offC), al->nC);
        return;
    }
    if (units) hipLaunchKernelGGL(zkc_wtns_mont, dim3((nv + 255) / 256, nb), dim3(256), 0, mv, (const Fr*)d_wtns0, (size_t)nv, d_wm, 3 * (size_t)n, nv);
    hipLaunchKernelGGL(zkc_matvec_jds, dim3((2 * n + 63 * zk->nlong + 255) / 256, nb), dim3(256), 0, mv, zk->d_perm, zk->d_rowlen, zk->d_jdptr, zk->d_col, zk->d_val,
                       (const Fr*)d_wtns0, (size_t)nv, d_abc, (int)n, zk->nlong, wm, 3 * (size_t)n, (const uint32_t*)nullptr, 2 * n);
    hipLaunchKernelGGL(zkc_pointwise_mul, dim3((n + 255) / 256, nb), dim3(256), 0, mv, d_abc, (int)n, (const uint32_t*)nullptr, n);
}
static constexpr uint32_t MATVEC_LONG = 16;

namespace {
uint32_t rd32(const uint8_t* p) { uint32_t v; memcpy(&v, p, 4); return v; }
uint64_t rd64(const uint8_t* p) { uint64_t v; memcpy(&v, p, 8); return v; }
G1Affine rd_g1(const uint8_t* p) { G1Affine a; (void)rd_g1_mont(a, p); return a; }
G2Affine rd_g2(const uint8_t* p) { G2Affine a; (void)rd_g2_mont(a, p); return a; }
}

extern "C" void zkc_zkey_free(zkc_zkey* zk) {
    if (!zk) return;
    ZKC_LOCK(zk->ctx);
    (void)hipSetDevice(zk->ctx->device);
    (void)hipStreamSynchronize(zk->ctx->stream);
    void* ptrs[] = {zk->d_perm, zk->d_rowlen, zk->d_jdptr, zk->d_col, zk->d_val, zk->d_tw_fwd, zk->d_tw_inv, zk->d_tw_fwd29, zk->d_tw_inv29, zk->d_coset, zk->d_coset_br, zk->d_g1, zk->d_g2, zk->d_g2_29, zk->d_g2_29_lone, zk->d_g2_29_deep,
                    zk->d_tblDelta1, zk->d_tblAlpha1, zk->d_tblBeta1, zk->d_tblDelta2, zk->d_fb4, zk->d_fb4g2, zk->d_depths};
    for (void* p : ptrs) if (p) (void)hipFree(p);
    fold_free(zk);
    if (zk->h_depths) (void)hipHostFree(zk->h_depths);
    for (auto& c : zk->call) { for (void* q : {(void*)c.d_rs, (void*)c.d_proofs, (void*)c.d_flags, (void*)c.d_status3}) if (q) (void)hipFree(q); if (c.h_flags) (void)hipHostFree(c.h_flags); if (c.h_out) (void)hipHostFree(c.h_out); if (c.h_rs) (void)hipHostFree(c.h_rs); if (c.h_xyzz) (void)hipHostFree(c.h_xyzz); if (c.h_early) (void)hipHostFree(c.h_early); if (c.d_xyzz) (void)hipFree(c.d_xyzz); for (hipEvent_t e : c.ev_done) if (e) (void)hipEventDestroy(e); for (hipEvent_t e : c.ev_chunk) (void)hipEventDestroy(e); }
    if (zk->ctx->lanes) for (int l = 0; l < zk->nlanes; l++) for (hipStream_t q : {zk->ctx->lanes[l].st, zk->ctx->lanes[l].st2, zk->ctx->lanes[l].fin, zk->ctx->lanes[l].red}) if (q) (void)hipStreamSynchronize(q);
    delete zk;
}

static size_t dev_free_bytes() { size_t f = 0, t = 0; if (hipMemGetInfo(&f, &t) != hipSuccess) { (void)hipGetLastError(); return 0; } return f; }
struct LaneNeed { size_t abc, p, fin, bs, e1, b1, e2, b2; int j1, j2; };
static LaneNeed lane_need(const zkc_zkey* zk, int inflight) {
    const uint32_t n = zk->n, nv = zk->nVars; const int NWS = msm_nw(zk->c_sec), NWB = msm_nw(zk->c_h);
    const size_t per_proof_entries = (size_t)NWS * 3 * nv + (size_t)NWB * n;
    const size_t per_proof_buckets = 3 * (size_t)msm_half(std::max(zk->c_sec, zk->c_deep)) + msm_half(zk->c_h);
    LaneNeed nd; nd.abc = 3 * (size_t)n * inflight; nd.p = 8 * (size_t)n * inflight; nd.fin = finalize_scratch_bytes(inflight); nd.bs = 2 * 2 * 8 * (size_t)nv;
    nd.e1 = per_proof_entries * inflight; nd.b1 = per_proof_buckets * inflight; nd.j1 = 4 * inflight;
    nd.e2 = (size_t)NWS * nv * inflight; nd.b2 = (size_t)msm_half(std::max(zk->c_sec, zk->c_deep)) * inflight; nd.j2 = inflight;
    return nd;
}
static bool lane_holds(const zkc_lane& L, const LaneNeed& nd) {
    return L.cap_abc >= nd.abc && L.cap_p >= nd.p && L.cap_fin >= nd.fin && L.cap_bs >= nd.bs && L.w1.max_entries >= nd.e1 && L.w1.max_buckets >= nd.b1 && L.w1.max_jobs >= nd.j1 &&
           L.w2.max_entries >= nd.e2 && L.w2.max_buckets >= nd.b2 && L.w2.max_jobs >= nd.j2;
}
static void lane_release(zkc_lane& L) {
    for (void** q : {(void**)&L.d_abc, (void**)&L.d_t, (void**)&L.d_p, &L.d_fin, (void**)&L.d_bs}) if (*q) { (void)hipFree(*q); *q = nullptr; }
    msm_work_free(L.w1); msm_work_free(L.w2);
    L.cap_abc = L.cap_p = L.cap_fin = L.cap_bs = 0; L.bytes = 0;
}
static zkc_lane* ctx_lanes(zkc_ctx* ctx) { if (!ctx->lanes) ctx->lanes = new zkc_lane[MAX_LANES]; return ctx->lanes; }
static size_t ctx_work_bytes(const zkc_ctx* ctx) { size_t t = 0; if (ctx->lanes) for (int l = 0; l < MAX_LANES; l++) t += ctx->lanes[l].bytes; return t; }
void zkc_ctx_lanes_destroy(zkc_ctx* ctx) {
    if (!ctx->lanes) return;
    for (int l = 0; l < MAX_LANES; l++) {
        zkc_lane& L = ctx->lanes[l];
        lane_release(L);
        for (hipEvent_t e : {L.ev_msm, L.ev_msm2, L.ev_sorted, L.ev_ntt, L.ev_mv, L.ev_acc, L.ev_fin[0], L.ev_fin[1], L.ev_red}) if (e) (void)hipEventDestroy(e);
    }
    delete[] ctx->lanes; ctx->lanes = nullptr;
}
static int lane_init(zkc_ctx* ctx, int l) {
    zkc_lane& L = ctx_lanes(ctx)[l];
    if (L.made) return ZKC_OK;
    zkc_ctx::LaneStreams ls; int rc = zkc_lane_streams(ctx, l, sw::on<sw::ZKC_REDUCE_STREAM>(), &ls); if (rc) return rc;
    L.st = ls.st; L.st2 = ls.st2; L.fin = ls.fin; L.red = ls.red;
    for (hipEvent_t* e : {&L.ev_msm, &L.ev_msm2, &L.ev_sorted, &L.ev_ntt, &L.ev_mv, &L.ev_acc, &L.ev_fin[0], &L.ev_fin[1], &L.ev_red}) if (!*e) ZKC_HIP_CHECK(ctx, hipEventCreateWithFlags(e, hipEventDisableTiming));
    L.made = true; return ZKC_OK;
}
struct LaneSt { hipStream_t st, st2, fin, red; };
// ... 98 lines not shown
            (rc = dmalloc(ctx, &zk->d_col, jcol.size() + 1)) || (rc = dmalloc(ctx, &zk->d_val, jval.size() + 1))) return bail(rc);
        ZKC_UP(zk->d_perm, perm.data(), nrows * 4); ZKC_UP(zk->d_rowlen, rowlen.data(), nrows * 4); ZKC_UP(zk->d_jdptr, jdptr.data(), jdptr.size() * 4);
        ZKC_UP(zk->d_col, jcol.data(), jcol.size() * 4);
        ZKC_UP(zk->d_val, jval.data(), jval.size() * sizeof(Fr));
        if (zk->nLevels >= 0 && sw::on<sw::ZKC_ABC_FOLD>()) {
            const WitnessLayout WL = WitnessLayout::make(zk->nLevels);
            const std::vector<std::pair<int, int>> rg[2] = {abc::fold_group_ranges(WL, 0), abc::fold_group_ranges(WL, 1)};
            zk->fold.abc_cls = abc::classify_rows(nrows, rowptr.data(), col.data(), abc::wire_groups(nv, rg), WL.n);
            zk->fold.abc_rowptr = std::move(rowptr); zk->fold.abc_col = std::move(col); zk->fold.abc_perm = perm;
            if (sw::on<sw::ZKC_TRACE_HOST>()) { const abc::RowCounts rc0 = abc::row_counts(zk->fold.abc_cls);
                fprintf(stderr, "[zkc host] abc rows: %zu of %zu A/B rows never constant, %zu constant when every level folds\n", rc0.never, nrows, rc0.constant_at_0); }
        }
    }
    {
        TwiddleTables tw;
        if ((rc = ntt_twiddle_tables(ctx, (int)zk->logn, true, &tw))) return bail(rc);
        zk->d_tw_fwd = tw.fwd; zk->d_tw_inv = tw.inv; zk->d_tw_fwd29 = tw.fwd29; zk->d_tw_inv29 = tw.inv29;
        const Fr g = fr_root_of_unity((int)zk->logn + 1), ninv = fp_inv<FrParams>(fp_from_u32<FrParams>(n));
        std::vector<Fr> cs(n);
        cs[0] = ninv; for (uint32_t i = 1; i < n; i++) cs[i] = cs[i - 1] * g;
        if ((rc = dmalloc(ctx, &zk->d_coset, n))) return bail(rc);
        ZKC_UP(zk->d_coset, cs.data(), cs.size() * sizeof(Fr));
        if ((rc = ntt_bitrev_table(ctx, zk->d_coset, &zk->d_coset_br, (int)zk->logn))) return bail(rc);
    }
    { const auto e_c = sw::given<sw::ZKC_C_SECTIONS>(); zk->c_sec = e_c ? (int)*e_c : zk->nLevels >= 0 ? MSM_C_SMALL : msm_c_for(nv); }
    { const auto e_h = sw::given<sw::ZKC_C_H>(); zk->c_h = e_h ? (int)*e_h : zk->nLevels >= 0 ? MSM_C_BIG : std::max(msm_c_for(n), n >= 12000 ? 15 : 12); }
    const int NWS = msm_nw(zk->c_sec);
    { const int dt = (int)sw::value<sw::ZKC_DEEP_TABLES>(1); const auto e_c = sw::given<sw::ZKC_C_DEEP>();
      const int cd = e_c ? (int)*e_c : msm_c_for(dt == 2 ? (size_t)40000 : (size_t)nv * 4 / 5);
      zk->c_deep = (zk->nLevels >= 0 && (nv >= (1u << 16) || dt == 2) && zk->c_sec < cd && dt != 0) ? cd : 0; }
    zk->c_h = std::max(zk->c_h, std::max(zk->c_sec, zk->c_deep));
    const int NWB = msm_nw(zk->c_h);
    zk->offA = 0; zk->offB1 = NWS * nv; zk->offC = 2 * NWS * nv; zk->offH = 2 * NWS * nv + NWS * nc;
    const int NWD = zk->c_deep ? msm_nw(zk->c_deep) : 0;
    zk->offA_deep = zk->offH + NWB * n; zk->offB1_deep = zk->offA_deep + NWD * nv; zk->offC_deep = zk->offB1_deep + NWD * nv;
    const size_t g1_points = (size_t)NWS * (2 * (size_t)nv + nc) + (size_t)NWB * n + (size_t)NWD * (2 * (size_t)nv + nc);
    if (g1_points >= (1ull << 31)) return bail(zkc_fail(ctx, ZKC_ERR_FORMAT, "zkey too large for 31-bit point indices"));
    if ((rc = dmalloc(ctx, &zk->d_g1, g1_points)) || (rc = dmalloc(ctx, &zk->d_g2, (size_t)NWS * nv))) return bail(rc);
    ZKC_UP(zk->d_g1 + zk->offA, sec[5], 64ull * nv); ZKC_UP(zk->d_g1 + zk->offB1, sec[6], 64ull * nv);
    ZKC_UP(zk->d_g1 + zk->offC, sec[8], 64ull * nc); ZKC_UP(zk->d_g1 + zk->offH, sec[9], 64ull * n);
    ZKC_UP(zk->d_g2, sec[7], 128ull * nv);
    if ((rc = msm_precompute_g1(ctx, nv, zk->d_g1 + zk->offA, zk->c_sec)) || (rc = msm_precompute_g1(ctx, nv, zk->d_g1 + zk->offB1, zk->c_sec)) ||
        (rc = msm_precompute_g1(ctx, nc, zk->d_g1 + zk->offC, zk->c_sec)) || (rc = msm_precompute_g1(ctx, n, zk->d_g1 + zk->offH, zk->c_h)) ||
        (rc = msm_precompute_g2(ctx, nv, zk->d_g2, zk->c_sec))) return bail(rc);
    if ((rc = dmalloc(ctx, &zk->d_g2_29, G2ROW_WORDS * (size_t)NWS * nv)) || (rc = msm_g2_table29(ctx, zk->d_g2, zk->d_g2_29, (size_t)NWS * nv))) return bail(rc);
    if (zk->c_deep) {
        ZKC_UP(zk->d_g1 + zk->offA_deep, sec[5], 64ull * nv); ZKC_UP(zk->d_g1 + zk->offB1_deep, sec[6], 64ull * nv); ZKC_UP(zk->d_g1 + zk->offC_deep, sec[8], 64ull * nc);
        if ((rc = msm_precompute_g1(ctx, nv, zk->d_g1 + zk->offA_deep, zk->c_deep)) || (rc = msm_precompute_g1(ctx, nv, zk->d_g1 + zk->offB1_deep, zk->c_deep)) ||
            (rc = msm_precompute_g1(ctx, nc, zk->d_g1 + zk->offC_deep, zk->c_deep))) return bail(rc);
        if ((rc = msm_g2_window_table29(ctx, zk->d_g2, nv, zk->c_deep, "second section tables", &zk->d_g2_29_deep))) return bail(rc);
    }
    {
        if (sw::on<sw::ZKC_G2_LONE_TABLE>() && (zk->nLevels >= 0 || nv < (1u << 16))) {
            if ((rc = msm_g2_window_table29(ctx, zk->d_g2, nv, MSM_C_G2_LONE, "lone-proof G2 table", &zk->d_g2_29_lone))) return bail(rc);
        }
    }
    const auto e_inf = sw::given<sw::ZKC_INFLIGHT>();
    zk->max_inflight = opt_inflight > 0 ? std::min(opt_inflight, MSM_MAX_JOBS / 4) : e_inf ? (int)*e_inf : zk->nLevels >= 0 ? 64 : 96;
    {
        const size_t per_proof_entries = (size_t)NWS * 3 * nv + (size_t)NWB * n, census_pass = 96ull * (22ull * 3 * 82754 + 15ull * 131072);
        const int fit = (int)std::max<size_t>(1, census_pass / std::max<size_t>(per_proof_entries, 1));
        zk->max_inflight = std::min(zk->max_inflight, fit);
    }
    { const auto e_l = sw::given<sw::ZKC_LANES>(); zk->nlanes = opt_lanes > 0 ? std::min(opt_lanes, (int)MAX_LANES) : e_l ? (int)*e_l : zk->nLevels >= 0 ? (int)MAX_LANES : 1; }
    zk->serial_streams = sw::on<sw::ZKC_SERIAL_STREAMS>();
    zk->lane_streams = (int)sw::value<sw::ZKC_LANE_STREAMS>(0);
    if ((rc = lanes_ensure(zk, 1, 0, 1))) return bail(rc);
    {
        FixedBase<Fq> td(zk->delta1), ta(zk->alpha1), tb(zk->beta1); FixedBase<Fq2> t2(zk->delta2);
        if ((rc = dmalloc(ctx, &zk->d_tblDelta1, td.tab.size())) || (rc = dmalloc(ctx, &zk->d_tblAlpha1, ta.tab.size())) ||
            (rc = dmalloc(ctx, &zk->d_tblBeta1, tb.tab.size())) || (rc = dmalloc(ctx, &zk->d_tblDelta2, t2.tab.size()))) return bail(rc);
        ZKC_UP(zk->d_tblDelta1, td.tab.data(), td.tab.size() * sizeof(G1Affine)); ZKC_UP(zk->d_tblAlpha1, ta.tab.data(), ta.tab.size() * sizeof(G1Affine));
        ZKC_UP(zk->d_tblBeta1, tb.tab.data(), tb.tab.size() * sizeof(G1Affine)); ZKC_UP(zk->d_tblDelta2, t2.tab.data(), t2.tab.size() * sizeof(G2Affine));
    }
    ZKC_HIP_BAIL(hipStreamSynchronize(ctx->stream));
    if (zk->nLevels >= 0 && (rc = fold_prepare(zk))) return bail(rc);
    if (zk->nLevels >= 0 && (rc = top_prepare(zk))) return bail(rc);
    if ((rc = fb4_prepare(zk))) return bail(rc);
    { const size_t f = dev_free_bytes(), grown = ctx_work_bytes(ctx) > work_at_entry ? ctx_work_bytes(ctx) - work_at_entry : 0; zk->bytes_tables = free_at_entry > f + grown ? free_at_entry - f - grown : 0; }
    *out = zk;
    return ZKC_OK;
#undef ZKC_UP
#undef ZKC_HIP_BAIL
}

int zkc::prove_reserve(zkc_zkey* zk, int inflight) {
    if (!zk) return ZKC_ERR_BAD_ARG;
    ZKC_LOCK(zk->ctx);
    ZKC_HIP_CHECK(zk->ctx, hipSetDevice(zk->ctx->device));
    return lanes_ensure(zk, inflight);
}
extern "C" int zkc_zkey_pass_info(const zkc_zkey* zk, int* pass_size, int* lanes) {
    if (!zk) return ZKC_ERR_BAD_ARG;
    if (pass_size) *pass_size = zk->max_inflight; if (lanes) *lanes = zk->nlanes;
    return ZKC_OK;
}
extern "C" int zkc_zkey_call_streams(const zkc_zkey* zk, int* streams) {
    if (!zk || !streams) return ZKC_ERR_BAD_ARG;
    ZKC_LOCK(zk->ctx);
    *streams = zk->last_call_streams;
    return ZKC_OK;
}
extern "C" int zkc_zkey_info(const zkc_zkey* zk, uint32_t* nVars, uint32_t* nPublic, uint32_t* domainSize) {
    if (!zk) return ZKC_ERR_BAD_ARG;
    if (nVars) *nVars = zk->nVars; if (nPublic) *nPublic = zk->nPub; if (domainSize) *domainSize = zk->n;
    return ZKC_OK;
}

static int h_matvec_dev(zkc_zkey* zk, zkc_lane& L, const uint32_t* d_wtns0, int nb, hipStream_t mv, const zkc_zkey::Fold::AbcRows* al = nullptr) {
    zkc_ctx* ctx = zk->ctx; const uint32_t n = zk->n, nv = zk->nVars;
    zkc_prof_scope _ps(ctx, ZKC_PROF_MATVEC, (uint64_t)nb * ((uint64_t)zk->nCoeffs * 68 + 3ull * n * 32), mv);
    matvec_launch(zk, L.d_abc, L.d_t, d_wtns0, nb, mv, al);
    ZKC_HIP_CHECK(ctx, hipGetLastError());
    return ZKC_OK;
}
static int h_evals_dev(zkc_zkey* zk, zkc_lane& L, hipStream_t st, const uint32_t* d_wtns0, int nb, bool with_matvec = true, const zkc_zkey::Fold::AbcRows* al = nullptr) {
    zkc_ctx* ctx = zk->ctx; const uint32_t n = zk->n;
    if (with_matvec) { int rc0 = h_matvec_dev(zk, L, d_wtns0, nb, st, al); if (rc0) return rc0; }
    zkc_prof_scope _pn(ctx, ZKC_PROF_NTT, (uint64_t)nb * (6ull * 2 * n * 32 + 4ull * n * 32), st);
    int rc;
    if (!sw::on<sw::ZKC_NTT_SEPARATE>() && zk->logn >= 12 && zk->logn <= 27) {
        if ((rc = ntt_pair_run(ctx, st, L.d_abc, zk->d_tw_inv29, zk->d_tw_fwd29, zk->d_coset_br, (int)zk->logn, 3 * nb))) return rc;
    } else {
        if ((rc = ntt_run(ctx, st, L.d_abc, L.d_t, zk->d_tw_inv29, zk->d_coset, (int)zk->logn, 3 * nb))) return rc;
        if ((rc = ntt_run(ctx, st, L.d_t, L.d_abc, zk->d_tw_fwd29, nullptr, (int)zk->logn, 3 * nb))) return rc;
    }
    hipLaunchKernelGGL(zkc_join_abc, dim3((n + 255) / 256, nb), dim3(256), 0, st, L.d_abc, L.d_p, (int)n);
    ZKC_HIP_CHECK(ctx, hipGetLastError());
    return ZKC_OK;
}

extern "C" int zkc_debug_stage(zkc_zkey* zk, const void* d_wtns, int stage, void* host_out) {
    if (!zk || !d_wtns || !host_out) return ZKC_ERR_BAD_ARG;
    zkc_ctx* ctx = zk->ctx; const uint32_t n = zk->n;
    ZKC_LOCK(ctx);
    ZKC_HIP_CHECK(ctx, hipSetDevice(ctx->device)); ZKC_HIP_CHECK(ctx, hipStreamSynchronize(ctx->stream));
    { int rc0 = lanes_ensure(zk, 1, 0, 1); if (rc0) return rc0; }
    zkc_lane& L0 = ctx->lanes[0]; const hipStream_t st0 = lane_st(zk, L0).st;
    if (stage == 0) {
        matvec_launch(zk, L0.d_abc, L0.d_t, (const uint32_t*)d_wtns, 1, st0);
        ZKC_HIP_CHECK(ctx, hipGetLastError());
        ZKC_HIP_CHECK(ctx, hipMemcpyAsync(host_out, L0.d_abc, 96ull * n, hipMemcpyDeviceToHost, st0));
    } else {
        int rc = h_evals_dev(zk, L0, st0, (const uint32_t*)d_wtns, 1); if (rc) return rc;
        ZKC_HIP_CHECK(ctx, hipMemcpyAsync(host_out, L0.d_p, 32ull * n, hipMemcpyDeviceToHost, st0));
    }
    ZKC_HIP_CHECK(ctx, hipStreamSynchronize(st0));
    return ZKC_OK;
}

extern "C" int zkc_msm_debug(zkc_zkey* zk, int which, const void* d_scalars, uint32_t count, void* host_out) {
    if (!zk || !d_scalars || !host_out || which < 0 || which > 4) return ZKC_ERR_BAD_ARG;
    zkc_ctx* ctx = zk->ctx;
    ZKC_LOCK(ctx);
    ZKC_HIP_CHECK(ctx, hipSetDevice(ctx->device)); ZKC_HIP_CHECK(ctx, hipStreamSynchronize(ctx->stream));
    { int rc0 = lanes_ensure(zk, 1, 0, 1); if (rc0) return rc0; }
    zkc_lane& L0 = ctx->lanes[0]; const hipStream_t st_l0 = lane_st(zk, L0).st;
    const uint32_t full = which == 3 ? zk->nVars - zk->nPub - 1 : which == 4 ? zk->n : zk->nVars;
    if (count != full) return zkc_fail(ctx, ZKC_ERR_BAD_ARG, "zkc_msm_debug: count must equal the section size");
    static thread_local MsmJobList jl; jl.clear(256, 1024, which == 2 ? (uint32_t)MSM_MAX_VW_PER_JOB : (uint32_t)MSM_MAX_VW_G1);
    const uint32_t offs[5] = {zk->offA, zk->offB1, 0, zk->offC, zk->offH};
    jl.add((const uint32_t*)d_scalars, nullptr, count, offs[which], full, 0, which == 4 ? zk->c_h : zk->c_sec);
    int rc = which == 2 ? msm_pass_g2(zk, L0.w2, jl, 0, true, st_l0) : msm_pass_g1(zk, L0.w1, jl, 0, true, st_l0); if (rc) return rc;
    ZKC_HIP_CHECK(ctx, hipStreamSynchronize(st_l0));
    if (which == 2) wr_g2_std((uint8_t*)host_out, xyzz_to_affine(*(G2XYZZ*)L0.w2.h_results));
    else wr_g1_std((uint8_t*)host_out, xyzz_to_affine(*(G1XYZZ*)L0.w1.h_results));
    return ZKC_OK;
}

int zkc::prove_batch_begin(zkc_zkey* zk, int cs, const void* d_wtns, uint32_t nWitness, int B, const uint8_t* rs, bool want_publics, const void* d_inputs, int32_t* d_status,
                           int lane0, hipEvent_t wait_first, const uint8_t* host_depths, bool no_early) {
    if (!zk || !d_wtns || !rs || B <= 0 || cs < 0 || cs >= CALL_SLOTS || lane0 >= zk->nlanes) return zkc_fail(zk ? zk->ctx : nullptr, ZKC_ERR_BAD_ARG, "zkc_prove_batch_dev: bad argument");
    zkc_ctx* ctx = zk->ctx;
    ZKC_LOCK(ctx);
    if (nWitness != zk->nVars) return zkc_fail(ctx, ZKC_ERR_INVALID_WITNESS_LENGTH, "Invalid witness length. Circuit: " + std::to_string(zk->nVars) + ", witness: " + std::to_string(nWitness));
    for (int b = 0; b < 2 * B; b++) { uint32_t t[8]; memcpy(t, rs + 32 * (size_t)b, 32); if (!fp_std_lt_p<FrParams>(t)) return zkc_fail(ctx, ZKC_ERR_BAD_ARG, "r or s >= field order"); }
    ZKC_HIP_CHECK(ctx, hipSetDevice(ctx->device));
    const uint32_t nv = zk->nVars, np = zk->nPub, n = zk->n;
    const bool can_fold = zk->nLevels >= 0;
    WitnessLayout L{}; int rc;
    const plan::CallSplit split = plan::call_split(B, zk->max_inflight); const int npasses = split.npasses, per_pass = split.per_pass;
    if ((rc = lanes_ensure(zk, per_pass, lane0 >= 0 ? lane0 : 0, lane0 >= 0 ? 1 : std::min(zk->nlanes, npasses)))) return rc;
    hipStream_t st0 = (lane0 >= 0 && !zk->serial_streams && B <= zk->max_inflight) ? ctx->lanes[lane0].st : ctx->stream;
    zkc_zkey::CallSlot& CS = zk->call[cs];
    if (CS.pending) return zkc_fail(ctx, ZKC_ERR_BAD_ARG, "prove_batch_begin: this call slot has a call in flight (finish it first)");
    if (CS.cap < (size_t)B) {
        if (CS.d_rs) { ZKC_HIP_CHECK(ctx, hipFree(CS.d_rs)); ZKC_HIP_CHECK(ctx, hipFree(CS.d_proofs)); ZKC_HIP_CHECK(ctx, hipHostFree(CS.h_out)); ZKC_HIP_CHECK(ctx, hipHostFree(CS.h_rs)); ZKC_HIP_CHECK(ctx, hipFree(CS.d_xyzz)); ZKC_HIP_CHECK(ctx, hipHostFree(CS.h_xyzz));
                       CS.d_rs = CS.d_proofs = CS.h_out = CS.h_rs = CS.d_xyzz = CS.h_xyzz = nullptr; CS.cap = 0; }
        const size_t want = std::max<size_t>((size_t)B, std::max<size_t>(256, std::min<size_t>(2 * CS.cap, 4096)));
        ZKC_HIP_CHECK(ctx, hipMalloc((void**)&CS.d_rs, 64 * want)); ZKC_HIP_CHECK(ctx, hipMalloc((void**)&CS.d_proofs, 256 * want));
        ZKC_HIP_CHECK(ctx, hipHostMalloc((void**)&CS.h_out, (256 + 32 * (size_t)zk->nPub) * want)); ZKC_HIP_CHECK(ctx, hipHostMalloc((void**)&CS.h_rs, 64 * want));
        ZKC_HIP_CHECK(ctx, hipMalloc((void**)&CS.d_xyzz, 512 * want)); ZKC_HIP_CHECK(ctx, hipHostMalloc((void**)&CS.h_xyzz, 512 * want)); CS.cap = want;
    }
    static const unsigned ev_host_flags = hipEventDisableTiming;
    for (int l = 0; l < zk->nlanes; l++) if (!CS.ev_done[l]) ZKC_HIP_CHECK(ctx, hipEventCreateWithFlags(&CS.ev_done[l], ev_host_flags));
    CS.as_xyzz.assign((size_t)B, 0); CS.lanes_used = 0;
    if (wait_first) ZKC_HIP_CHECK(ctx, hipStreamWaitEvent(st0, wait_first, 0));
    uint8_t* const h_pub = CS.h_out + 256ull * CS.cap;
    if (rs != CS.h_rs_copy.data()) CS.h_rs_copy.assign(rs, rs + 64 * (size_t)B);
// ... 84 lines not shown
        tr[1] = now_ms();
        const uint32_t* w0 = (const uint32_t*)d_wtns + (size_t)p0 * nv * 8;
        uint8_t dcq[MSM_MAX_JOBS / 4], dsq[MSM_MAX_JOBS / 4]; bool fold = can_fold;
        if (early) for (int q = 0; q < nb; q++) { dcq[q] = CS.early_depth[2 * q]; dsq[q] = CS.early_depth[2 * q + 1]; }
        else for (int q = 0; q < nb && fold; q++) for (int t = 0; t < 2; t++) {
            const int D = plan::row_depth(CS.h_flags + (size_t)(p0 + q) * fstride + (size_t)t * L.n, L.n);
            if (D == plan::FOREIGN) { fold = false; break; }
            (t == 0 ? dcq : dsq)[q] = (uint8_t)D;
        }
        static thread_local zkc_zkey::Fold::VMap vms[MSM_MAX_JOBS / 4];
        uint16_t tcq[MSM_MAX_JOBS / 4], tsq[MSM_MAX_JOBS / 4];
        const auto& tp = zk->fold.top; const int TK = tp.K;
        plan::top_fold(dcq, dsq, CS.h_flags + (size_t)p0 * fstride + 2 * (size_t)L.n, fstride, fold ? TK : 0, tp.nslots, tp.valid.data(), early, nb, tcq, tsq, seeds);
        if (!seeds.empty() && (rc = top_seed(zk, w0, seeds))) return rc;
        if (fold) for (int q = 0; q < nb; q++) if ((rc = fold_vmap(zk, tcq[q] != top::NO_SLOT ? TK : 0, dcq[q], tsq[q] != top::NO_SLOT ? TK : 0, dsq[q], &vms[q]))) return rc;
        const bool nofold_lists = sw::on<sw::ZKC_NOFOLD_LISTS>();
        if (!fold && nofold_lists) {
            zkc_zkey::Fold::VMap nf; if ((rc = nofold_vmap(zk, &nf))) return rc;
            for (int q = 0; q < nb; q++) vms[q] = nf;
        }
        const bool listed = fold || (nofold_lists && vms[0].d != nullptr);
        const plan::PassShape PS = plan::pass_shape(KS, nb, listed ? vms : (const zkc_zkey::Fold::VMap*)nullptr, plan::LaneCaps{LN.w1.max_entries, LN.w1.max_buckets, LN.w1.max_jobs, LN.w2.max_entries}, SW);
        const plan::StreamOrder SO = plan::stream_order(nb, one_lane, pass, npasses, lane0, PS.tree, SW);
        const PassSt PT = pass_st(LS, plan::lane_roles(nb, one_lane, pass, npasses, lane0, PS.tree, lanes, SW));
        const hipStream_t st = PT.st, st2 = PT.st2, bl = PT.bl, fin = LS.fin;
        touch(st); touch(st2); touch(bl); touch(PT.red);
        ZKC_HIP_CHECK(ctx, hipStreamWaitEvent(st, CS.ev_chunk[pass], 0)); if (st2 != st) ZKC_HIP_CHECK(ctx, hipStreamWaitEvent(st2, CS.ev_chunk[pass], 0));
        if (LN.npass >= 2) { ZKC_HIP_CHECK(ctx, wait_unless_same(st, LN.ev_fin[slot], LN.fin_on[slot])); if (st2 != st) ZKC_HIP_CHECK(ctx, wait_unless_same(st2, LN.ev_fin[slot], LN.fin_on[slot])); }
        LN.npass++;
        const bool tree = PS.tree, mv_done = SO.mv_done;
        if (mv_done) ZKC_HIP_CHECK(ctx, hipStreamWaitEvent(st, LN.ev_mv, 0));
        zkc_zkey::Fold::AbcRows ar; const bool abc_fold = fold && !mv_done && !zk->fold.abc_cls.empty() && zk->fold.d_abc_tmpl != nullptr;
        if (abc_fold) { int Dc = 0, Ds = 0; for (int q = 0; q < nb; q++) { Dc = std::max(Dc, (int)dcq[q]); Ds = std::max(Ds, (int)dsq[q]); } if ((rc = abc_rows(zk, Dc, Ds, &ar))) return rc; }
        if ((rc = h_evals_dev(zk, LN, st, w0, nb, !mv_done, abc_fold ? &ar : nullptr))) return rc;
        if (st2 != st || SO.mv_prefetch) ZKC_HIP_CHECK(ctx, hipEventRecord(LN.ev_ntt, st));
        tr[2] = now_ms();
        static thread_local MsmJobList j1, j2;
        j1.clear(PS.vws, PS.vwb, MSM_MAX_VW_G1); j2.clear(PS.vw_g2, 1024, MSM_MAX_VW_PER_JOB);
        for (int q = 0; q < nb; q++) j1.add(LN.d_p + 8 * (size_t)n * q, nullptr, n, zk->offH, n, 0, zk->c_h);
        auto add = [](MsmJobList& jl, const uint32_t* scalars, const plan::SectionView& v, int c) { jl.add(scalars, v.vmap, v.count, v.tbl_off, v.tbl_count, v.pt_shift, c); };
        BlindArgs ba{}; ba.rs = CS.d_rs + 64 * (size_t)p0; ba.nv = nv;
        for (int q = 0; q < nb; q++) {
            const uint32_t* w = w0 + (size_t)q * nv * 8;
            uint32_t* bs = tree ? LN.d_bs + (size_t)q * 2 * nv * 8 : nullptr;
            const plan::ProofViews v = plan::proof_views(KS, PS, w, listed ? &vms[q] : nullptr);
            add(j1, v.A.scalars, v.A, PS.cw); add(j1, v.B1.scalars, v.B1, PS.cw); add(j1, v.C.scalars, v.C, PS.cw);
            if (tree) { add(j1, bs, v.A, PS.cw); add(j1, bs + 8ull * nv, v.B1, PS.cw); }
            j2.add(w, v.B1.vmap, v.B1.count, 0, nv, 0, PS.c2);
            if (tree) { ba.w[q] = w; ba.out[q] = bs; ba.mapA[q] = v.A.vmap; ba.nA[q] = v.A.count; ba.mapB[q] = v.B1.vmap; ba.nB[q] = v.B1.count; }
        }
        if (tree && (rc = blind_scalars_launch(ctx, st, ba, nb))) return rc;
        FinalizeArgs fa{};
        fa.r1 = (const G1XYZZ*)LN.w1.results + (size_t)slot * LN.w1.max_jobs; fa.r2 = (const G2XYZZ*)LN.w2.results + (size_t)slot * LN.w2.max_jobs;
        fa.foldA = zk->fold.d_foldA; fa.foldB1 = zk->fold.d_foldB1; fa.foldC = zk->fold.d_foldC; fa.foldB2 = zk->fold.d_foldB2; fa.fold_n = can_fold ? L.n : 0;
        for (int q = 0; q < nb; q++) { fa.dc[q] = fold ? dcq[q] : (uint8_t)255; fa.ds[q] = fold ? dsq[q] : (uint8_t)255; fa.tc[q] = tcq[q]; fa.ts[q] = tsq[q]; }
        fa.topA = tp.d_A; fa.topB1 = tp.d_B1; fa.topC = tp.d_C; fa.topB2 = tp.d_B2;
        fa.tblDelta1 = zk->d_tblDelta1; fa.tblAlpha1 = zk->d_tblAlpha1; fa.tblBeta1 = zk->d_tblBeta1; fa.tblDelta2 = zk->d_tblDelta2;
        fa.alpha1 = zk->alpha1; fa.beta2 = zk->beta2; fa.rs = CS.d_rs + 64 * (size_t)p0; fa.out = CS.d_proofs + 256 * (size_t)p0; fa.scratch = LN.d_fin;
        fa.per = PS.per; fa.fb4 = zk->d_fb4; fa.fb4g2 = zk->d_fb4g2; fa.out_xyzz = CS.d_xyzz + 512 * (size_t)p0;
        const bool g2_early = !sw::on<sw::ZKC_G2_LATE>();
        auto g2_side = [&](hipEvent_t acc_after) -> int {
            if (LN.g2_done) ZKC_HIP_CHECK(ctx, wait_unless_same(st2, LN.g2_done, LN.g2_on));
            if ((rc = msm_pass_g2(zk, LN.w2, j2, slot, false, st2, acc_after))) return rc;
            if (tree && (rc = finalize_tree_g2_launch(ctx, st2, fa, nb))) return rc;
            if (st2 != bl) ZKC_HIP_CHECK(ctx, hipEventRecord(LN.ev_msm2, st2));
            LN.g2_on = st2; LN.g2_done = st2 != bl ? LN.ev_msm2 : LN.ev_fin[slot];
            return ZKC_OK;
        };
        if (g2_early && (rc = g2_side(SO.g2_acc_with_sort && st2 != st ? LN.ev_ntt : nullptr))) return rc;
        tr[3] = now_ms();
        ZKC_HIP_CHECK(ctx, wait_unless_same(st, LN.ev_red, LN.red_on));
        const bool want_sorted = SO.mv_prefetch || (!g2_early && st2 != st);
// ... 108 lines not shown
```

### zk-franchise-proof-circuit_amd/csrc/zkc_prover.h

```cpp
#pragma once
#include <cstring>
#include "zkc_internal.h"
#include "zkc_curve.h"
#include "zkc_abc_rows.h"
#include "zkc_top_fold.h"
#include "zkc_pass_plan.h"
#include <array>

namespace zkc {
constexpr int MSM_C_BIG = 17, MSM_C_SMALL = 12;
inline long long first_unreduced_wire(const void* w, size_t count) {
    const uint8_t* p = (const uint8_t*)w;
    for (size_t i = 0; i < count; i++) {
        uint32_t t[8]; memcpy(t, p + 32 * i, 32);
        if (t[7] >= FrParams::p[7] && !fp_std_lt_p<FrParams>(t)) return (long long)i;
    }
    return -1;
}
inline std::string unreduced_wire_msg(long long wire) { return "Witness value at wire " + std::to_string(wire) + " is not below the field order r"; }
inline int msm_c_for(size_t W) { return W < 12000 ? 12 : W < 22000 ? 13 : W < 90000 ? 15 : W < 180000 ? 16 : 17; }
constexpr int MSM_VW_MIN = 64, MSM_MAX_VW_PER_JOB = 64;
constexpr int MSM_MAX_VW_G1 = 256;
constexpr int MSM_SEG_MIN = 16;
#ifndef ZKC_MSM_SEG
// ... 113 lines not shown
    size_t max_entries = 0, max_segments = 0; int max_jobs = 0; size_t xyzz_size = 0;
};
}

struct zkc_lane {
    hipStream_t st = nullptr, st2 = nullptr, fin = nullptr;
    hipStream_t red = nullptr; hipEvent_t ev_red = nullptr;
    zkc::Fr *d_abc = nullptr, *d_t = nullptr; uint32_t* d_p = nullptr;
    void* d_fin = nullptr;
    uint32_t* d_bs = nullptr;
    zkc::MsmWork w1, w2;
    size_t cap_abc = 0, cap_p = 0, cap_fin = 0, cap_bs = 0, bytes = 0; bool made = false;
    hipEvent_t ev_msm = nullptr, ev_msm2 = nullptr, ev_sorted = nullptr, ev_ntt = nullptr, ev_mv = nullptr, ev_acc = nullptr, ev_fin[2] = {nullptr, nullptr}; int npass = 0;
    hipStream_t g2_on = nullptr; hipEvent_t g2_done = nullptr;
    hipStream_t fin_on[2] = {nullptr, nullptr}, red_on = nullptr;
};

struct zkc_zkey {
    zkc_ctx* ctx = nullptr;
    uint32_t nVars = 0, nPub = 0, n = 0, logn = 0, nCoeffs = 0;
    int nLevels = -1;
    zkc::G1Affine alpha1, beta1, delta1;
    zkc::G2Affine beta2, gamma2, delta2;
    std::vector<zkc::G1Affine> ic;
    uint32_t *d_perm = nullptr, *d_rowlen = nullptr, *d_jdptr = nullptr, *d_col = nullptr; zkc::Fr* d_val = nullptr; uint32_t nlong = 0;
    uint32_t n_unit_coeffs = 0;
    zkc::Fr *d_tw_fwd = nullptr, *d_tw_inv = nullptr, *d_coset = nullptr;
    zkc::Fr *d_coset_br = nullptr;
    uint32_t *d_tw_fwd29 = nullptr, *d_tw_inv29 = nullptr;
    zkc::G1Affine* d_g1 = nullptr; zkc::G2Affine* d_g2 = nullptr;
    uint32_t* d_g2_29 = nullptr;
    uint32_t* d_g2_29_lone = nullptr;
    uint32_t offA = 0, offB1 = 0, offC = 0, offH = 0;
    int c_deep = 0; uint32_t offA_deep = 0, offB1_deep = 0, offC_deep = 0; uint32_t* d_g2_29_deep = nullptr;
    int c_h = zkc::MSM_C_BIG;
    int c_sec = zkc::MSM_C_SMALL;
    int max_inflight = 0;
    uint8_t sha256[32] = {0};
    size_t bytes_tables = 0;
    uint8_t fingerprint[32] = {0};
    int nlanes = 1; bool serial_streams = false;
    int lane_streams = 0;
    int last_call_streams = 0;
    zkc::G1Affine *d_tblDelta1 = nullptr, *d_tblAlpha1 = nullptr, *d_tblBeta1 = nullptr; zkc::G2Affine* d_tblDelta2 = nullptr;
    uint32_t *d_depths = nullptr, *h_depths = nullptr; size_t depths_cap = 0;
    zkc::G1XYZZ* d_fb4 = nullptr; zkc::G2XYZZ* d_fb4g2 = nullptr; int fb4_bases = 0;
    struct CallSlot {
        uint8_t *d_rs = nullptr, *d_proofs = nullptr; size_t cap = 0;
        uint8_t* h_out = nullptr;
        uint8_t* h_rs = nullptr;
        uint8_t *d_xyzz = nullptr, *h_xyzz = nullptr; std::vector<uint8_t> as_xyzz;
        hipEvent_t ev_done[zkc::MAX_LANES] = {};
        std::vector<hipEvent_t> ev_chunk;
        uint32_t lanes_used = 0;
        int B = 0; bool pending = false;
        uint32_t *d_flags = nullptr, *h_flags = nullptr; size_t flags_cap = 0;
        int32_t* d_status3 = nullptr; size_t status3_cap = 0;
        int early_n = 0; std::vector<uint8_t> early_depth; uint32_t* h_early = nullptr; size_t early_cap = 0;
        const void* arg_wtns = nullptr; uint32_t arg_nw = 0; bool arg_publics = false, arg_inputs = false; int arg_lane0 = -1; hipEvent_t arg_wait = nullptr; std::vector<uint8_t> h_rs_copy;
    } call[zkc::CALL_SLOTS];
    struct Fold {
        std::vector<zkc::G1XYZZ> baseA, baseB1, baseC; std::vector<zkc::G2XYZZ> baseB2;
        std::vector<zkc::G1XYZZ> sufA[2], sufB1[2], sufC[2]; std::vector<zkc::G2XYZZ> sufB2[2];
        struct VMap { uint32_t* d = nullptr; uint32_t offA = 0, nA = 0, offB = 0, nB = 0, offC = 0, nC = 0; };
        std::map<std::array<int, 4>, VMap> vmaps;
        std::vector<uint8_t> infA, infB, infC;
        zkc::G1XYZZ *d_foldA = nullptr, *d_foldB1 = nullptr, *d_foldC = nullptr; zkc::G2XYZZ* d_foldB2 = nullptr;
        bool ready = false;
        std::vector<zkc::abc::RowClass> abc_cls; std::vector<uint32_t> abc_rowptr, abc_col, abc_perm;
        zkc::Fr* d_abc_tmpl = nullptr;
        struct AbcRows { uint32_t* d = nullptr; uint32_t nrows = 0, nlong = 0, offC = 0, nC = 0, offW = 0, nW = 0; };
        std::map<std::pair<int, int>, AbcRows> abc_rows;
        struct Top {
            int K = 0; uint32_t nslots = 0;
            zkc::TopCheckArgs args{};
            uint32_t *d_copy[2] = {nullptr, nullptr}, *d_valid = nullptr;
            zkc::G1XYZZ *d_A = nullptr, *d_B1 = nullptr, *d_C = nullptr; zkc::G2XYZZ* d_B2 = nullptr;
            std::vector<uint8_t> valid;
            std::vector<uint32_t> wA[2], wB[2], wC[2], gA[2], gB[2], gC[2];
            uint64_t seeded = 0; double seed_ms = 0;
        } top;
    } fold;
};

namespace zkc {
int ntt_run(zkc_ctx* ctx, hipStream_t st, const Fr* src, Fr* dst, const uint32_t* tw29, const Fr* scale, int logn, int nvec);
int ntt_make_tw29(zkc_ctx* ctx, const Fr* d_tw, uint32_t count, uint32_t** out);
struct TwiddleTables { Fr *fwd = nullptr, *inv = nullptr; uint32_t *fwd29 = nullptr, *inv29 = nullptr; };
int ntt_twiddle_tables(zkc_ctx* ctx, int logn, bool keep_fr, TwiddleTables* out, bool with_29 = true);
int msm_g2_window_table29(zkc_ctx* ctx, const G2Affine* d_bases, uint32_t count, int c, const char* what, uint32_t** out);
int msm_g2_rows29(zkc_ctx* ctx, const G2Affine* d_points, size_t n, const char* what, uint32_t** out);
int ntt_pair_run(zkc_ctx* ctx, hipStream_t st, Fr* data, const uint32_t* tw_inv29, const uint32_t* tw_fwd29, const Fr* scale_br, int logn, int nvec);
int ntt_bitrev_table(zkc_ctx* ctx, const Fr* d_src, Fr** out, int logn);
int msm_work_alloc(zkc_ctx* ctx, MsmWork& w, size_t max_entries, size_t max_buckets, int max_jobs, bool g2);
void msm_work_free(MsmWork& w);
int msm_pass_g1(zkc_zkey* zk, MsmWork& w, const MsmJobList& jl, int slot, bool to_host, hipStream_t st, hipEvent_t ev_sorted = nullptr, hipEvent_t ev_acc = nullptr,
                hipStream_t st_red = nullptr, hipEvent_t ev_red = nullptr);
int msm_pass_g2(zkc_zkey* zk, MsmWork& w, const MsmJobList& jl, int slot, bool to_host, hipStream_t st, hipEvent_t wait_before_acc = nullptr);
int msm_bucket_entries(zkc_ctx* ctx, MsmWork& w, const MsmJobList& jl, hipStream_t st, unsigned long long* d_entry_counter = nullptr);
int msm_build_segments(zkc_ctx* ctx, MsmWork& w, const MsmJobList& jl, uint32_t seg, size_t seg_bound, hipStream_t st);
int finalize_launch(zkc_ctx* ctx, hipStream_t st, const FinalizeArgs& a, int nproofs);
int finalize_tree_g2_launch(zkc_ctx* ctx, hipStream_t st, const FinalizeArgs& a, int nproofs);
int fb4_build(zkc_ctx* ctx, hipStream_t st, const G1XYZZ* d_bases, int nbases, G1XYZZ* d_out, const G2XYZZ& delta2, const G2XYZZ& beta2, const G2XYZZ& beta2_base, G2XYZZ* d_out2);
int blind_scalars_launch(zkc_ctx* ctx, hipStream_t st, const BlindArgs& a, int nproofs);
template <class T> inline int dmalloc(zkc_ctx* ctx, T** p, size_t count) { ZKC_HIP_CHECK(ctx, hipMalloc((void**)p, count * sizeof(T))); return ZKC_OK; }
int fold_prepare(zkc_zkey* zk);
int top_prepare(zkc_zkey* zk);
int fb4_prepare(zkc_zkey* zk);
void fold_free(zkc_zkey* zk);
int fold_vmap(zkc_zkey* zk, int Tc, int Dc, int Ts, int Ds, zkc_zkey::Fold::VMap* out);
int nofold_vmap(zkc_zkey* zk, zkc_zkey::Fold::VMap* out);
int top_seed(zkc_zkey* zk, const uint32_t* w0, const std::vector<plan::TopSeed>& seeds);
int abc_template(zkc_zkey* zk, const uint32_t* tmpl);
int abc_rows(zkc_zkey* zk, int Dc, int Ds, zkc_zkey::Fold::AbcRows* out);
void matvec_launch(zkc_zkey* zk, Fr* d_abc, Fr* d_wm, const uint32_t* d_wtns0, int nb, hipStream_t mv, const zkc_zkey::Fold::AbcRows* al = nullptr);
int prove_batch_begin(zkc_zkey* zk, int cs, const void* d_wtns, uint32_t nWitness, int B, const uint8_t* rs, bool want_publics, const void* d_inputs, int32_t* d_status,
                      int lane0 = -1, hipEvent_t wait_first = nullptr, const uint8_t* host_depths = nullptr, bool no_early = false);
int prove_batch_finish(zkc_zkey* zk, int cs, uint8_t* proofs, uint8_t* publics);
int prove_reserve(zkc_zkey* zk, int inflight);
int zkey_load_opts(zkc_ctx* ctx, const void* zkey_bytes, size_t len, int nlanes, int max_inflight, zkc_zkey** out);
size_t zkey_device_bytes(const zkc_zkey* zk, size_t* tables, size_t* work);
size_t finalize_scratch_bytes(int nproofs);
int msm_precompute_g1(zkc_ctx* ctx, uint32_t count, G1Affine* d_table, int c);
int msm_precompute_g2(zkc_ctx* ctx, uint32_t count, G2Affine* d_table, int c);
int msm_g2_table29(zkc_ctx* ctx, const G2Affine* d_table, uint32_t* d_out, size_t count);
int fold_group_sums_g1(zkc_ctx* ctx, const G1Affine* tbl, const uint32_t* d_scalars, const uint32_t* d_wires, uint32_t nw, int32_t pt_shift,
                       const uint32_t* d_gstart, uint32_t ngroups, G1XYZZ* h_out, uint32_t pt_mod = 0, hipStream_t st = nullptr);
int fold_group_sums_g1_ws(zkc_ctx* ctx, const G1Affine* tbl, const uint32_t* d_scalars, const uint32_t* d_wires, uint32_t nw, const uint32_t* d_gstart, uint32_t ngroups,
                          G1XYZZ* d_tmp , G1XYZZ* d_out , G1XYZZ* h_out);
int fold_group_sums_g2(zkc_ctx* ctx, const G2Affine* tbl, const uint32_t* d_scalars, const uint32_t* d_wires, uint32_t nw, int32_t pt_shift,
                       const uint32_t* d_gstart, uint32_t ngroups, G2XYZZ* h_out, uint32_t pt_mod = 0, hipStream_t st = nullptr);
}
```

### zk-franchise-proof-circuit_amd/csrc/zkc_switches.h

```cpp
#pragma once
#include <climits>
#include <cstdlib>
#include <optional>

namespace zkc { namespace sw {

enum Kind { SET, OFF_IF_ZERO, ON_IF_ONE, NUMBER, NUMBER_LONG, NUMBER_U64, TEXT };
enum When { PROCESS, LIVE };
constexpr long long ANY = LLONG_MIN;

#define ZKC_SWITCHES(X)                                                                                                                                                   \
                                                                                                                                            \
    X(ZKC_DEVICE,               TEXT,        ANY, ANY,   LIVE,    "service creation: the GPUs of the default proving service: \"2\", \"0,1,2,3\", \"all\"; unset: every visible device") \
    X(ZKC_INFLIGHT,             NUMBER,      1,   128,   LIVE,    "key load: proofs per pipeline pass (census key 64, any other 96, fewer for a large circuit); at most MSM_MAX_JOBS / 4") \
    X(ZKC_LANES,                NUMBER,      1,   4,     LIVE,    "key load: pipeline lanes the passes of a batch call rotate over (census key MAX_LANES = 4, any other 1)")      \
    X(ZKC_LANE_STREAMS,         NUMBER,      1,   3,     LIVE,    "key load: streams of a lane that a pass of a call rotating over several lanes uses: 1 all on the G1 stream (default), 2 the G2 MSM on its own, 3 the blinding too") \
    X(ZKC_DEEP_TABLES,          NUMBER,      ANY, ANY,   LIVE,    "key load: 0 leaves out the second section tables that passes of deep voters take, 2 builds them for a census key of any size (default 1)") \
    X(ZKC_G2_LONE_TABLE,        OFF_IF_ZERO, ANY, ANY,   LIVE,    "key load: =0 skips the 8-bit-window G2 table of the lone-proof path")                                          \
    X(ZKC_BLIND_TREE,           OFF_IF_ZERO, ANY, ANY,   LIVE,    "key load: =0 gives a key whose passes of one or two proofs take the general blinding kernels")                 \
    X(ZKC_SERVICE_WORKERS,      NUMBER,      1,   4,     LIVE,    "service creation: workers (= lanes of a service key) per GPU (4); at most MAX_LANES")                          \
    X(ZKC_SERVICE_PASS,         NUMBER,      1,   128,   LIVE,    "service creation: proofs per pass of a service key (64); at most MSM_MAX_JOBS / 4")                            \
    X(ZKC_SERVICE_KEYS,         NUMBER,      1,   64,    LIVE,    "service creation: keys kept resident per GPU (4)")                                                             \
    X(ZKC_SERVICE_MAX_BATCH,    NUMBER,      1,   4096,  LIVE,    "service creation: requests one worker takes per call (256)")                                                   \
    X(ZKC_SERVICE_MIN_BATCH,    NUMBER,      1,   ANY,   LIVE,    "service creation: requests a collecting worker waits for before it goes (16)")                                 \
    X(ZKC_SERVICE_SPILL,        NUMBER,      1,   ANY,   LIVE,    "service creation: queue length at which a cold GPU is brought up (32)")                                        \
    X(ZKC_SERVICE_BUSY_WAIT_US, NUMBER,      0,   ANY,   LIVE,    "service creation: microseconds a collecting worker waits for more requests (300)")                             \
    X(ZKC_SERVICE_RESERVE,      OFF_IF_ZERO, ANY, ANY,   PROCESS, "=0: a service key load does not reserve a full pass of work space on every lane; the lanes grow on demand")    \
    X(ZKC_DEVICE_BLOCKING_SYNC, ON_IF_ONE,   ANY, ANY,   LIVE,    "context creation: =1 asks HIP for blocking waits on the device (hipDeviceScheduleBlockingSync)")               \
    X(ZKC_SPIN_WAIT,            SET,         ANY, ANY,   PROCESS, "set (any value, 0 included): host waits use hipEventSynchronize instead of polling with short sleeps")         \
    X(ZKC_VERIFY_BATCH_GPU,     NUMBER,      ANY, ANY,   LIVE,    "per verify call: 0 keeps the Miller loops of zkc_verify_batch on the host, positive forces the GPU, negative or unset: GPU from 128 proofs") \
    X(ZKC_NO_SHA_NI,            SET,         ANY, ANY,   PROCESS, "set (any value, 0 included): portable SHA-256 instead of the CPU's SHA extensions")                            \
                                                                                                                              \
    X(ZKC_NO_FOLD,              SET,         ANY, ANY,   LIVE,    "key load: set (any value, 0 included): no constant folding of the voter-independent witness part for this key") \
    X(ZKC_SERIAL_STREAMS,       SET,         ANY, ANY,   LIVE,    "key load: set (any value, 0 included): every stage of this key's passes on the context's one stream (isolated stage times)") \
    X(ZKC_C_SECTIONS,           NUMBER,      8,   17,    LIVE,    "key load: window bits of the witness sections (census key 12, any other by its wire count); at most MSM_C_BIG") \
    X(ZKC_C_H,                  NUMBER,      8,   17,    LIVE,    "key load: window bits of the H section (census key 17, any other by its domain size); at most MSM_C_BIG")      \
    X(ZKC_C_DEEP,               NUMBER,      13,  17,    LIVE,    "key load: window bits of the second section tables (by the wire count); at most MSM_C_BIG")                    \
    X(ZKC_DEEP_WIRES,           NUMBER_LONG, ANY, ANY,   PROCESS, "live wires per section and proof from which a pass takes the second section tables (16000)")                   \
    X(ZKC_WITNESS_GROUP,        NUMBER,      1,   ANY,   PROCESS, "passes whose voters share one witness launch in a batch call (8)")                                             \
    X(ZKC_VW_BIG,               NUMBER,      ANY, ANY,   PROCESS, "buckets per reduction wave of the H jobs in passes of more than four proofs (0 or unset: 4096, 1024 below 32 proofs)") \
    X(ZKC_VW_SMALL,             NUMBER,      ANY, ANY,   PROCESS, "the same for the witness sections (0 or unset: 2048, 256 below 32 proofs)")                                    \
    X(ZKC_VW_G2,                NUMBER,      ANY, ANY,   PROCESS, "the same for the G2 jobs of passes of 32 proofs and more (0 or unset: as the witness sections)")              \
    X(ZKC_G2_ACC,               NUMBER,      ANY, ANY,   PROCESS, "form of the G2 accumulation: 0 registers hold the next row, 1 / 2 LDS-DMA prefetch at one / two waves per SIMD (0)") \
    X(ZKC_G2_BUCKET_WAVE,       OFF_IF_ZERO, ANY, ANY,   PROCESS, "=0: small G2 passes keep lane-per-segment accumulation instead of half a wave per bucket")                     \
    X(ZKC_G2_LATE,              SET,         ANY, ANY,   PROCESS, "set (any value, 0 included): the G2 MSM of a pass starts after the G1 sort instead of with the pass")          \
    X(ZKC_G2_ACC_HOLD,          SET,         ANY, ANY,   PROCESS, "set (any value, 0 included): the G2 accumulation always waits for the G1 stream to leave its transforms")      \
    X(ZKC_G2_ACC_EARLY,         SET,         ANY, ANY,   PROCESS, "set (any value, 0 included): the G2 accumulation never waits for them (ZKC_G2_ACC_HOLD wins)")                 \
    X(ZKC_ACC_CHAIN,            OFF_IF_ZERO, ANY, ANY,   PROCESS, "=0: the G1 accumulations of a context's lanes are not chained one behind the other")                           \
    X(ZKC_REDUCE_STREAM,        ON_IF_ONE,   ANY, ANY,   PROCESS, "=1: the bucket reduction of a full pass runs on a stream of its own (the lanes then get that stream)")         \
    X(ZKC_MATVEC_UNITS,         OFF_IF_ZERO, ANY, ANY,   PROCESS, "=0: buildABC multiplies by its +-1 coefficients instead of adding the wire")                                   \
    X(ZKC_ABC_FOLD,             OFF_IF_ZERO, ANY, ANY,   PROCESS, "=0: buildABC of a folded pass computes every row instead of copying the voter-independent ones from the template") \
    X(ZKC_TOP_FOLD,             NUMBER,      0,   12,    LIVE,    "key load: census tree levels below the root whose MSM terms are summed once per subtree instead of per voter (8; 0: off)") \
    X(ZKC_MATVEC_INLINE,        SET,        ANY, ANY,   PROCESS, "set (any value, 0 included): buildABC of the next pass is not prefetched on the blinding stream")              \
    X(ZKC_MV_PREFETCH_AT_NTT,   ON_IF_ONE,   ANY, ANY,   PROCESS, "=1: that prefetch starts beside the pass' bucketing instead of beside its accumulation")                       \
    X(ZKC_EARLY_LAYOUT,         OFF_IF_ZERO, ANY, ANY,   PROCESS, "=0: one-pass calls of more than two voters wait for their fold flags instead of reading the depths off the inputs") \
    X(ZKC_NOFOLD_LISTS,         OFF_IF_ZERO, ANY, ANY,   PROCESS, "=0: unfolded passes keep the wires whose bases are at infinity")                                               \
    X(ZKC_NTT_SEPARATE,         SET,         ANY, ANY,   PROCESS, "set (any value, 0 included): two self-contained transforms instead of the fused pair")                         \
    X(ZKC_NTT_RADIX,            NUMBER,      ANY, ANY,   PROCESS, "below 4: the head transform kernel runs one stage at a time instead of two (4)")                               \
    X(ZKC_FINALIZE_WAVES,       SET,         ANY, ANY,   PROCESS, "set (any value, 0 included): the one-wave-per-task blinding kernel for every pass")                            \
    X(ZKC_VERIFY_CHUNK,         NUMBER,      2,   16384, LIVE,    "per verify call: pairs per round of Miller-loop kernels (16384)")                                              \
    X(ZKC_SMT_WAVE_MAX,         NUMBER_U64,  ANY, ANY,   LIVE,    "per check call: census proof batches up to this size take the wave-per-proof form (64; 0: never)")            \
    X(ZKC_TRACE_HOST,           SET,         ANY, ANY,   PROCESS, "set (any value, 0 included): prints where the enqueueing thread spends its time, per pass")                    \
    X(ZKC_VERIFY_TRACE,         SET,         ANY, ANY,   LIVE,    "per verify call: set (any value, 0 included): prints the stage times of zkc_verify_batch")                     \
    X(ZKC_DEBUG_SYNC,           SET,         ANY, ANY,   PROCESS, "set (any value, 0 included): synchronises after and logs every MSM launch; read when the library is loaded")   \
                                                                                                                                                \
    X(ZKC_TEST_FAIL_ALLOC,      NUMBER,      ANY, ANY,   LIVE,    "lane growth: the work-space allocation for this many proofs in flight or more fails")                          \
    X(ZKC_TEST_TOP_SLOTS,       NUMBER,      1,   16384, LIVE,    "key load: slots per tree of the top-of-tree table instead of 8 x 2^K (1: every subtree lands on one slot)")    \
    X(ZKC_TEST_FAIL_KEY_LOADS,  NUMBER,      ANY, ANY,   LIVE,    "service key load: fails as out of memory while the device holds this many keys or more")

enum Id {
#define X(name, kind, lo, hi, when, doc) name,
    ZKC_SWITCHES(X)
#undef X
    COUNT
};
struct Row { const char* name; Kind kind; long long lo, hi; When when; const char* doc; };
inline constexpr Row rows[COUNT] = {
#define X(name, kind, lo, hi, when, doc) {#name, kind, lo, (hi) == ANY ? LLONG_MAX : (hi), when, doc},
    ZKC_SWITCHES(X)
#undef X
};

struct Raw { bool set; long long num; const char* str; };
inline Raw read(const Row& r) {
    const char* e = getenv(r.name);
// ... 28 lines not shown
```

Measured before the change: 3512.

## Skip C transform pair in folded passes by folding voter C rows into H MSM

For folded passes, the prover no longer runs the inverse/forward NTT pair on the C vector. The template C contribution is transformed once at key load, and a second H-like base table is built from -H' via EC-NTTs. Per voter, only the C rows that differ from the template are written as delta scalars and appended to the H MSM job. The transform of A and B uses an ab_only mode, and a size rule with a beta parameter decides per pass whether to take this path. In exchange, the H MSM grows by the number of voter C rows and key load does extra precomputation and uses more table memory.

New measurement: 3666 (median of 6 runs). 4.4% higher.

```diff
diff --git a/include/zkcensus.h b/include/zkcensus.h
--- a/include/zkcensus.h
+++ b/include/zkcensus.h
@@ -126,6 +126,7 @@
 int zkc_debug_stage(zkc_zkey* zk, const void* d_wtns, int stage, void* host_out);
 unsigned long long zkc_debug_early_retries(void);
 int zkc_msm_debug(zkc_zkey* zk, int which, const void* d_scalars, uint32_t count, void* host_out);
+int zkc_debug_c_rows(zkc_zkey* zk, int what, uint32_t first, uint32_t count, void* host_out);
 int zkc_debug_pairing_dev(zkc_ctx* ctx, const uint8_t* g1, const uint8_t* g2, const uint8_t* weights, int N, uint8_t product_out[384], uint8_t* folded_out,
                           int32_t* member_out, int* bad_out, const uint32_t* nodes, size_t count, uint8_t* node_out);
 
diff --git a/zk-franchise-proof-circuit_amd/_native.py b/zk-franchise-proof-circuit_amd/_native.py
--- a/zk-franchise-proof-circuit_amd/_native.py
+++ b/zk-franchise-proof-circuit_amd/_native.py
@@ -45,6 +45,7 @@
     L.zkc_debug_stage.argtypes = [vp, vp, ctypes.c_int, ctypes.c_char_p]
     L.zkc_debug_early_retries.argtypes = []; L.zkc_debug_early_retries.restype = ctypes.c_ulonglong
     L.zkc_msm_debug.argtypes = [vp, ctypes.c_int, vp, ctypes.c_uint32, ctypes.c_char_p]
+    L.zkc_debug_c_rows.argtypes = [vp, ctypes.c_int, ctypes.c_uint32, ctypes.c_uint32, ctypes.c_char_p]
     L.zkc_debug_pairing_dev.argtypes = [vp, ctypes.c_char_p, ctypes.c_char_p, ctypes.c_char_p, ctypes.c_int, ctypes.c_char_p, ctypes.c_char_p, i32p, ctypes.POINTER(ctypes.c_int),
                                         ctypes.POINTER(ctypes.c_uint32), ctypes.c_size_t, ctypes.c_char_p]
     ulp = ctypes.POINTER(ctypes.c_ulong)
diff --git a/zk-franchise-proof-circuit_amd/csrc/zkc_fold.hip b/zk-franchise-proof-circuit_amd/csrc/zkc_fold.hip
--- a/zk-franchise-proof-circuit_amd/csrc/zkc_fold.hip
+++ b/zk-franchise-proof-circuit_amd/csrc/zkc_fold.hip
@@ -1,6 +1,8 @@
 #include "zkc_prover.h"
 #include "zkc_host_util.h"
 #include "zkc_kernels.h"
+#include "zkc_fixedbase_dev.h"
+#include "zkc_ecntt.h"
 #include <ctime>
 #include <cstdio>
 #include <algorithm>
@@ -282,13 +284,44 @@
     zkc_zkey::Fold::AbcRows m; m.nrows = (uint32_t)v.rows.size(); m.nlong = v.nlong; m.offC = m.nrows; m.nC = (uint32_t)v.crows.size(); m.offW = m.offC + m.nC; m.nW = (uint32_t)v.wires.size();
     std::vector<uint32_t> all(v.rows); all.insert(all.end(), v.crows.begin(), v.crows.end()); all.insert(all.end(), v.wires.begin(), v.wires.end());
     if (int rc = list_upload(ctx, all, ctx->stream, &m.d)) return rc;
+    if (zk->h_rows == 2 * zk->n) { if (int rc = list_upload(ctx, plan::h_vmap(zk->n, v.crows.data(), m.nC), ctx->stream, &m.d_hv)) { (void)hipFree(m.d); return rc; } }
     if (sw::on<sw::ZKC_TRACE_HOST>()) fprintf(stderr, "[zkc host] abc rows at depths (%d, %d): %u of %zu A/B rows listed (%u long), %u C rows, %u wires\n", Dc, Ds, m.nrows, f.abc_cls.size(), m.nlong, m.nC, m.nW);
     f.abc_rows[{Dc, Ds}] = m; *out = m;
     return ZKC_OK;
 }
+int zkc::c_rows_prepare(zkc_zkey* zk) {
+    auto& f = zk->fold; zkc_ctx* ctx = zk->ctx;
+    if (f.c_rows_ready) return ZKC_OK;
+    const uint32_t n = zk->n, logn = zk->logn; int rc;
+    if (!f.d_abc_tmpl || zk->h_rows != 2 * n || logn < 12 || logn > 27) return zkc_fail(ctx, ZKC_ERR_BAD_ARG, "c_rows_prepare: the key has no template abc or no wide H table");
+    timespec ts0; clock_gettime(CLOCK_MONOTONIC, &ts0);
+    DevBuf chat, t, s, xy, sc, wi;
+    if ((rc = chat.alloc(ctx, (size_t)n * sizeof(Fr)))) return rc;
+    ZKC_HIP_CHECK(ctx, hipMemcpyAsync(chat.p, f.d_abc_tmpl + 2 * (size_t)n, (size_t)n * sizeof(Fr), hipMemcpyDeviceToDevice, ctx->stream));
+    if ((rc = ntt_pair_run(ctx, ctx->stream, chat.as<Fr>(), zk->d_tw_inv29, zk->d_tw_fwd29, zk->d_coset_br, (int)logn, 1))) return rc;
+    std::vector<uint32_t> h_sc(8 * (size_t)n), h_wi(n);
+    { const Fr g = fr_root_of_unity((int)logn + 1); Fr c = Fr::zero() - fp_from_u32<FrParams>(n);
+      for (uint32_t k = 0; k < n; k++) { const uint32_t p = (n - k) & (n - 1); fp_to_std<FrParams>(h_sc.data() + 8 * (size_t)p, c); h_wi[k] = p; c = c * g; } }
+    G1Affine* const H0 = zk->d_g1 + zk->offH;
+    if ((rc = t.alloc(ctx, (size_t)n * sizeof(G1Affine))) || (rc = s.alloc(ctx, (size_t)n * sizeof(G1Affine))) || (rc = xy.alloc(ctx, (size_t)n * sizeof(G1XYZZ))) ||
+        (rc = sc.alloc(ctx, h_sc.size() * 4)) || (rc = wi.alloc(ctx, h_wi.size() * 4))) return rc;
+    ZKC_HIP_CHECK(ctx, hipMemcpyAsync(sc.p, h_sc.data(), h_sc.size() * 4, hipMemcpyHostToDevice, ctx->stream));
+    ZKC_HIP_CHECK(ctx, hipMemcpyAsync(wi.p, h_wi.data(), h_wi.size() * 4, hipMemcpyHostToDevice, ctx->stream));
+    if ((rc = ecntt<Fq>(ctx, H0, logn, zk->d_tw_inv, logn, t.p, true, nullptr))) return rc;
+    if ((rc = g1_scale_each(ctx, t.as<G1Affine>(), sc.as<uint32_t>(), wi.as<uint32_t>(), n, xy.as<G1XYZZ>()))) return rc;
+    if ((rc = fixed_affine<Fq>(ctx, xy.as<G1XYZZ>(), n, s.p, true))) return rc;
+    if ((rc = ecntt<Fq>(ctx, s.p, logn, zk->d_tw_inv, logn, H0 + n, true, nullptr))) return rc;
+    if ((rc = msm_precompute_g1(ctx, n, H0 + n, zk->c_h, 2 * (size_t)n))) return rc;
+    ZKC_HIP_CHECK(ctx, hipStreamSynchronize(ctx->stream));
+    f.d_c_hat = (Fr*)chat.release(); f.c_rows_ready = true;
+    if (sw::on<sw::ZKC_TRACE_HOST>()) { timespec ts1; clock_gettime(CLOCK_MONOTONIC, &ts1);
+        fprintf(stderr, "[zkc host] c rows: transformed template C and -H' (%u points, %d windows) in %.1f ms\n", n, msm_nw(zk->c_h), (ts1.tv_sec - ts0.tv_sec) * 1e3 + (ts1.tv_nsec - ts0.tv_nsec) * 1e-6); }
+    return ZKC_OK;
+}
 void zkc::fold_free(zkc_zkey* zk) {
+    if (zk->fold.d_c_hat) (void)hipFree(zk->fold.d_c_hat);
     for (auto& kv : zk->fold.vmaps) if (kv.second.d) (void)hipFree(kv.second.d);
-    for (auto& kv : zk->fold.abc_rows) if (kv.second.d) (void)hipFree(kv.second.d);
+    for (auto& kv : zk->fold.abc_rows) { if (kv.second.d) (void)hipFree(kv.second.d); if (kv.second.d_hv) (void)hipFree(kv.second.d_hv); }
     if (zk->fold.d_abc_tmpl) (void)hipFree(zk->fold.d_abc_tmpl);
     { auto& tp = zk->fold.top; for (void* q : {(void*)tp.d_copy[0], (void*)tp.d_copy[1], (void*)tp.d_valid, (void*)tp.d_A, (void*)tp.d_B1, (void*)tp.d_C, (void*)tp.d_B2}) if (q) (void)hipFree(q); }
     for (void* q : {(void*)zk->fold.d_foldA, (void*)zk->fold.d_foldB1, (void*)zk->fold.d_foldC, (void*)zk->fold.d_foldB2}) if (q) (void)hipFree(q);
diff --git a/zk-franchise-proof-circuit_amd/csrc/zkc_kernels.h b/zk-franchise-proof-circuit_amd/csrc/zkc_kernels.h
--- a/zk-franchise-proof-circuit_amd/csrc/zkc_kernels.h
+++ b/zk-franchise-proof-circuit_amd/csrc/zkc_kernels.h
@@ -21,11 +21,13 @@
 
 extern "C" __global__ void zkc_wtns_mont(const Fr* wtns_std, size_t wtns_stride, Fr* wm, size_t wm_stride, uint32_t nv);
 extern "C" __global__ void zkc_wtns_mont_list(const Fr* wtns_std, size_t wtns_stride, Fr* wm, size_t wm_stride, const uint32_t* list, uint32_t nlist);
-extern "C" __global__ void zkc_abc_fill(const uint4* tmpl, uint4* abc, uint32_t per);
+extern "C" __global__ void zkc_abc_fill(const uint4* tmpl, uint4* abc, uint32_t per, uint32_t stride);
 extern "C" __global__ void zkc_matvec_jds(const uint32_t* perm, const uint32_t* rowlen, const uint32_t* jdptr, const uint32_t* col, const Fr* val, const Fr* wtns_std,
                                           size_t wtns_stride, Fr* abc, int n, uint32_t nlong, const Fr* wm_all, size_t wm_stride, const uint32_t* list, uint32_t nrows);
 extern "C" __global__ void zkc_pointwise_mul(Fr* abc, int n, const uint32_t* list, uint32_t count);
 extern "C" __global__ void zkc_join_abc(const Fr* abc, uint32_t* p_std, int n);
+extern "C" __global__ void zkc_join_abc_ct(const Fr* abc, const Fr* c_hat, uint32_t* p_std, int n);
+extern "C" __global__ void zkc_c_rows_delta(const Fr* abc, const Fr* c_tmpl, uint32_t* p_std, int n, const uint32_t* list, uint32_t count);
 
 struct TopCheckArgs;
 extern "C" __global__ void zkc_fold_check(WitnessLayout L, const uint32_t* wtns, const uint32_t* tmpl, uint32_t* flags, int B, int stride);
diff --git a/zk-franchise-proof-circuit_amd/csrc/zkc_msm.hip b/zk-franchise-proof-circuit_amd/csrc/zkc_msm.hip
--- a/zk-franchise-proof-circuit_amd/csrc/zkc_msm.hip
+++ b/zk-franchise-proof-circuit_amd/csrc/zkc_msm.hip
@@ -437,16 +437,17 @@
     next[i] = xyzz_to_affine(p);
 }
 template <class F>
-static int precompute(zkc_ctx* ctx, uint32_t count, Affine<F>* d_table, int c) {
+static int precompute(zkc_ctx* ctx, uint32_t count, Affine<F>* d_table, int c, size_t stride = 0) {
+    if (!stride) stride = count;
     for (int w = 1; w < msm_nw(c); w++) {
         hipLaunchKernelGGL(HIP_KERNEL_NAME(zkc_msm_shift_bases<F>), dim3((count + 127) / 128), dim3(128), 0, ctx->stream,
-                           d_table + (size_t)(w - 1) * count, d_table + (size_t)w * count, count, c);
+                           d_table + (size_t)(w - 1) * stride, d_table + (size_t)w * stride, count, c);
         hipError_t e = hipGetLastError();
         if (e != hipSuccess) return zkc_fail(ctx, ZKC_ERR_HIP, std::string("zkc_msm_shift_bases: ") + hipGetErrorString(e));
     }
     return ZKC_OK;
 }
-int msm_precompute_g1(zkc_ctx* ctx, uint32_t count, G1Affine* d_table, int c) { return precompute<Fq>(ctx, count, d_table, c); }
+int msm_precompute_g1(zkc_ctx* ctx, uint32_t count, G1Affine* d_table, int c, size_t window_stride) { return precompute<Fq>(ctx, count, d_table, c, window_stride); }
 int msm_precompute_g2(zkc_ctx* ctx, uint32_t count, G2Affine* d_table, int c) { return precompute<Fq2>(ctx, count, d_table, c); }
 int msm_g2_rows29(zkc_ctx* ctx, const G2Affine* d_points, size_t n, const char* what, uint32_t** out) {
     DevBuf rows; int rc;
@@ -521,6 +522,11 @@
 }
 int fold_group_sums_g1(zkc_ctx* ctx, const G1Affine* tbl, const uint32_t* s, const uint32_t* w, uint32_t nw, int32_t sh, const uint32_t* gs, uint32_t ng, G1XYZZ* o, uint32_t pt_mod, hipStream_t st) {
     return fold_group_sums<Fq>(ctx, tbl, s, w, nw, sh, gs, ng, o, pt_mod, st);
+}
+int g1_scale_each(zkc_ctx* ctx, const G1Affine* tbl, const uint32_t* d_scalars, const uint32_t* d_wires, uint32_t nw, G1XYZZ* d_out) {
+    hipLaunchKernelGGL(HIP_KERNEL_NAME(zkc_fold_mul<Fq>), dim3((nw + 63) / 64), dim3(64), 0, ctx->stream, tbl, d_scalars, d_wires, nw, 0, d_out, 0u);
+    ZKC_HIP_CHECK(ctx, hipGetLastError());
+    return ZKC_OK;
 }
 int fold_group_sums_g1_ws(zkc_ctx* ctx, const G1Affine* tbl, const uint32_t* s, const uint32_t* w, uint32_t nw, const uint32_t* gs, uint32_t ng, G1XYZZ* d_tmp, G1XYZZ* d_out, G1XYZZ* h_out) {
     return fold_group_sums_ws<Fq>(ctx, tbl, s, w, nw, 0, gs, ng, d_tmp, d_out, h_out, 0u, ctx->stream);
@@ -609,7 +615,7 @@
     uint64_t alg_bytes = 0; uint32_t maxcount = 0;
     uint64_t streamed_bytes = 0;
     for (int j = 0; j < nj; j++) {
-        alg_bytes += (uint64_t)jl.job[j].tbl_count * (sizeof(Affine<F>) + 32);
+        alg_bytes += (uint64_t)(jl.job[j].vmap ? jl.job[j].tbl_count : std::min(jl.job[j].tbl_count, jl.job[j].count)) * (sizeof(Affine<F>) + 32);
         streamed_bytes += (uint64_t)jl.job[j].count * (sizeof(Affine<F>) + 32);
         maxcount = std::max(maxcount, jl.job[j].count);
     }
diff --git a/zk-franchise-proof-circuit_amd/csrc/zkc_ntt.hip b/zk-franchise-proof-circuit_amd/csrc/zkc_ntt.hip
--- a/zk-franchise-proof-circuit_amd/csrc/zkc_ntt.hip
+++ b/zk-franchise-proof-circuit_amd/csrc/zkc_ntt.hip
@@ -26,8 +26,8 @@
     st_fr(wm + (size_t)blockIdx.y * wm_stride + i, ld_fr(wtns_std + (size_t)blockIdx.y * wtns_stride + i) * r2);
 }
 extern "C" __global__ void __launch_bounds__(256)
-zkc_abc_fill(const uint4* __restrict__ tmpl, uint4* __restrict__ abc, uint32_t per) {
-    uint4* __restrict__ dst = abc + (size_t)blockIdx.y * per;
+zkc_abc_fill(const uint4* __restrict__ tmpl, uint4* __restrict__ abc, uint32_t per, uint32_t stride) {
+    uint4* __restrict__ dst = abc + (size_t)blockIdx.y * stride;
     for (uint32_t i = blockIdx.x * blockDim.x + threadIdx.x; i < per; i += gridDim.x * blockDim.x) dst[i] = tmpl[i];
 }
 extern "C" __global__ void __launch_bounds__(256)
@@ -66,12 +66,7 @@
     st_fr(a + 2 * (size_t)n + i, ld_fr(a + i) * ld_fr(a + n + i));
 }
 struct JoinDom { static constexpr L9 D27 = f29_dominator<FrParams>(1u << 29, 1u << 27); };
-extern "C" __global__ void __launch_bounds__(256)
-zkc_join_abc(const Fr* __restrict__ abc, uint32_t* __restrict__ p_std, int n) {
-    const int i = blockIdx.x * blockDim.x + threadIdx.x;
-    if (i >= n) return;
-    const Fr* a = abc + (size_t)blockIdx.y * 3 * n;
-    const Fr av = ld_fr(a + i), bv = ld_fr(a + n + i), cv = ld_fr(a + 2 * (size_t)n + i);
+__device__ __forceinline__ void join_abc_one(const Fr av, const Fr bv, const Fr cv, uint32_t* __restrict__ out_std) {
     uint32_t A[9], B[9], C[9], T[9];
     f29_from_fp_shl5(A, av.v); f29_from_fp_shl5(B, bv.v); f29_from_fp_shl5(C, cv.v);
 #pragma unroll
@@ -85,8 +80,33 @@
     r.v[0] = f29_word<0>(T); r.v[1] = f29_word<32>(T); r.v[2] = f29_word<64>(T); r.v[3] = f29_word<96>(T);
     r.v[4] = f29_word<128>(T); r.v[5] = f29_word<160>(T); r.v[6] = f29_word<192>(T); r.v[7] = f29_word<224>(T);
     fp_reduce_once<FrParams>(r.v);
-    uint4* d = reinterpret_cast<uint4*>(p_std + 8 * ((size_t)blockIdx.y * n + i));
+    uint4* d = reinterpret_cast<uint4*>(out_std);
     d[0] = make_uint4(r.v[0], r.v[1], r.v[2], r.v[3]); d[1] = make_uint4(r.v[4], r.v[5], r.v[6], r.v[7]);
+}
+extern "C" __global__ void __launch_bounds__(256)
+zkc_join_abc(const Fr* __restrict__ abc, uint32_t* __restrict__ p_std, int n) {
+    const int i = blockIdx.x * blockDim.x + threadIdx.x;
+    if (i >= n) return;
+    const Fr* a = abc + (size_t)blockIdx.y * 3 * n;
+    join_abc_one(ld_fr(a + i), ld_fr(a + n + i), ld_fr(a + 2 * (size_t)n + i), p_std + 8 * ((size_t)blockIdx.y * n + i));
+}
+extern "C" __global__ void __launch_bounds__(256)
+zkc_join_abc_ct(const Fr* __restrict__ abc, const Fr* __restrict__ c_hat, uint32_t* __restrict__ p_std, int n) {
+    const int i = blockIdx.x * blockDim.x + threadIdx.x;
+    if (i >= n) return;
+    const Fr* a = abc + (size_t)blockIdx.y * 3 * n;
+    join_abc_one(ld_fr(a + i), ld_fr(a + n + i), ld_fr(c_hat + i), p_std + 8 * ((size_t)blockIdx.y * 2 * n + i));
+}
+extern "C" __global__ void __launch_bounds__(256)
+zkc_c_rows_delta(const Fr* __restrict__ abc, const Fr* __restrict__ c_tmpl, uint32_t* __restrict__ p_std, int n, const uint32_t* __restrict__ list, uint32_t count) {
+    const uint32_t e = blockIdx.x * blockDim.x + threadIdx.x;
+    if (e >= count) return;
+    const uint32_t i = list[e];
+    const Fr* a = abc + (size_t)blockIdx.y * 3 * n;
+    const Fr dv = ld_fr(a + i) * ld_fr(a + n + i) - ld_fr(c_tmpl + i);
+    uint32_t s[8]; fp_to_std<FrParams>(s, dv);
+    uint4* d = reinterpret_cast<uint4*>(p_std + 8 * ((size_t)blockIdx.y * 2 * n + n + i));
+    d[0] = make_uint4(s[0], s[1], s[2], s[3]); d[1] = make_uint4(s[4], s[5], s[6], s[7]);
 }
 
 constexpr int NTT_TILE = 1024;
@@ -142,11 +162,12 @@
 #pragma unroll
     for (int i = 0; i < 9; i++) { p0[i] = a[i]; p1[i] = b[i]; p2[i] = c[i]; p3[i] = d[i]; }
 }
+__device__ __forceinline__ size_t ntt_vec(int ab_only) { return ab_only ? (size_t)blockIdx.y + (blockIdx.y >> 1) : (size_t)blockIdx.y; }
 extern "C" __global__ void __launch_bounds__(256)
 zkc_ntt_pass(const Fr* src_all, Fr* dst_all, const uint32_t* __restrict__ tw29, const Fr* __restrict__ scale,
-             int logn, int s0, int b, int first) {
-    const Fr* src = src_all + ((size_t)blockIdx.y << logn);
-    Fr* dst = dst_all + ((size_t)blockIdx.y << logn);
+             int logn, int s0, int b, int first, int ab_only) {
+    const Fr* src = src_all + (ntt_vec(ab_only) << logn);
+    Fr* dst = dst_all + (ntt_vec(ab_only) << logn);
     extern __shared__ uint32_t tile[];
     const int mid_n = 1 << b;
     const int lo_bits = s0;
@@ -251,9 +272,9 @@
     }
 }
 template <int RADIX>
-__device__ __forceinline__ void ntt_nr_head_body(const Fr* src_all, Fr* dst_all, const uint32_t* __restrict__ tw29, int logn, int q0, int b) {
-    const Fr* src = src_all + ((size_t)blockIdx.y << logn);
-    Fr* dst = dst_all + ((size_t)blockIdx.y << logn);
+__device__ __forceinline__ void ntt_nr_head_body(const Fr* src_all, Fr* dst_all, const uint32_t* __restrict__ tw29, int logn, int q0, int b, int ab_only) {
+    const Fr* src = src_all + (ntt_vec(ab_only) << logn);
+    Fr* dst = dst_all + (ntt_vec(ab_only) << logn);
     extern __shared__ uint32_t tile[];
     const int mid_n = 1 << b, sh = logn - q0 - b, lo_t = NTT_TILE >> b, elems = mid_n * lo_t;
     const int bpp = (1 << sh) / lo_t;
@@ -278,12 +299,12 @@
     }
 }
 extern "C" __global__ void __launch_bounds__(256)
-zkc_ntt_nr_head(const Fr* src_all, Fr* dst_all, const uint32_t* __restrict__ tw29, int logn, int q0, int b) { ntt_nr_head_body<1>(src_all, dst_all, tw29, logn, q0, b); }
-extern "C" __global__ void __launch_bounds__(256)
-zkc_ntt_nr_head_r4(const Fr* src_all, Fr* dst_all, const uint32_t* __restrict__ tw29, int logn, int q0, int b) { ntt_nr_head_body<4>(src_all, dst_all, tw29, logn, q0, b); }
-extern "C" __global__ void __launch_bounds__(256)
-zkc_ntt_mid(Fr* __restrict__ data_all, const uint32_t* __restrict__ tw_inv29, const uint32_t* __restrict__ tw_fwd29, const Fr* __restrict__ scale_br, int logn) {
-    Fr* __restrict__ data = data_all + ((size_t)blockIdx.y << logn);
+zkc_ntt_nr_head(const Fr* src_all, Fr* dst_all, const uint32_t* __restrict__ tw29, int logn, int q0, int b, int ab_only) { ntt_nr_head_body<1>(src_all, dst_all, tw29, logn, q0, b, ab_only); }
+extern "C" __global__ void __launch_bounds__(256)
+zkc_ntt_nr_head_r4(const Fr* src_all, Fr* dst_all, const uint32_t* __restrict__ tw29, int logn, int q0, int b, int ab_only) { ntt_nr_head_body<4>(src_all, dst_all, tw29, logn, q0, b, ab_only); }
+extern "C" __global__ void __launch_bounds__(256)
+zkc_ntt_mid(Fr* __restrict__ data_all, const uint32_t* __restrict__ tw_inv29, const uint32_t* __restrict__ tw_fwd29, const Fr* __restrict__ scale_br, int logn, int ab_only) {
+    Fr* __restrict__ data = data_all + (ntt_vec(ab_only) << logn);
     extern __shared__ uint32_t tile[];
     constexpr int B = 9, MID = 1 << B, NSUB = NTT_TILE / MID;
     const size_t base = (size_t)blockIdx.x * NTT_TILE;
@@ -344,18 +365,19 @@
     ZKC_HIP_CHECK(ctx, hipGetLastError());
     return ZKC_OK;
 }
-int ntt_pair_run(zkc_ctx* ctx, hipStream_t st, Fr* data, const uint32_t* tw_inv29, const uint32_t* tw_fwd29, const Fr* scale_br, int logn, int nvec) {
+int ntt_pair_run(zkc_ctx* ctx, hipStream_t st, Fr* data, const uint32_t* tw_inv29, const uint32_t* tw_fwd29, const Fr* scale_br, int logn, int nvec, bool ab_only) {
+    const int ab = ab_only ? 1 : 0;
     if (logn < 12 || logn > 27) return zkc_fail(ctx, ZKC_ERR_BAD_ARG, "ntt_pair_run: 12 <= logn <= 27");
     const int bh = logn - 9;
     const int b1 = bh <= 9 ? bh : (bh + 1) / 2, b2 = bh - b1;
     const unsigned blocks = (1u << logn) / NTT_TILE;
     const int radix = (int)sw::value<sw::ZKC_NTT_RADIX>(4);
     auto head = radix >= 4 ? zkc_ntt_nr_head_r4 : zkc_ntt_nr_head;
-    hipLaunchKernelGGL(head, dim3(blocks, nvec), dim3(256), (size_t)NTT_TILE * 36, st, (const Fr*)data, data, tw_inv29, logn, 0, b1);
-    if (b2) hipLaunchKernelGGL(head, dim3(blocks, nvec), dim3(256), (size_t)NTT_TILE * 36, st, (const Fr*)data, data, tw_inv29, logn, b1, b2);
-    hipLaunchKernelGGL(zkc_ntt_mid, dim3(blocks, nvec), dim3(256), (size_t)NTT_TILE * 36, st, data, tw_inv29, tw_fwd29, scale_br, logn);
-    hipLaunchKernelGGL(zkc_ntt_pass, dim3(blocks, nvec), dim3(256), (size_t)NTT_TILE * 36, st, (const Fr*)data, data, tw_fwd29, (const Fr*)nullptr, logn, 9, b1, 0);
-    if (b2) hipLaunchKernelGGL(zkc_ntt_pass, dim3(blocks, nvec), dim3(256), (size_t)NTT_TILE * 36, st, (const Fr*)data, data, tw_fwd29, (const Fr*)nullptr, logn, 9 + b1, b2, 0);
+    hipLaunchKernelGGL(head, dim3(blocks, nvec), dim3(256), (size_t)NTT_TILE * 36, st, (const Fr*)data, data, tw_inv29, logn, 0, b1, ab);
+    if (b2) hipLaunchKernelGGL(head, dim3(blocks, nvec), dim3(256), (size_t)NTT_TILE * 36, st, (const Fr*)data, data, tw_inv29, logn, b1, b2, ab);
+    hipLaunchKernelGGL(zkc_ntt_mid, dim3(blocks, nvec), dim3(256), (size_t)NTT_TILE * 36, st, data, tw_inv29, tw_fwd29, scale_br, logn, ab);
+    hipLaunchKernelGGL(zkc_ntt_pass, dim3(blocks, nvec), dim3(256), (size_t)NTT_TILE * 36, st, (const Fr*)data, data, tw_fwd29, (const Fr*)nullptr, logn, 9, b1, 0, ab);
+    if (b2) hipLaunchKernelGGL(zkc_ntt_pass, dim3(blocks, nvec), dim3(256), (size_t)NTT_TILE * 36, st, (const Fr*)data, data, tw_fwd29, (const Fr*)nullptr, logn, 9 + b1, b2, 0, ab);
     hipError_t e = hipGetLastError();
     if (e != hipSuccess) return zkc_fail(ctx, ZKC_ERR_HIP, std::string("ntt_pair_run: ") + hipGetErrorString(e));
     return ZKC_OK;
@@ -394,7 +416,7 @@
         const int nblocks = (1 << logn) / ((1 << b) * lo_t);
         const bool last = s0 + b == logn;
         hipLaunchKernelGGL(zkc_ntt_pass, dim3(nblocks, nvec), dim3(256), (size_t)(1 << b) * lo_t * 36, st,
-                           first ? src : dst, dst, tw29, last ? scale : nullptr, logn, s0, b, first ? 1 : 0);
+                           first ? src : dst, dst, tw29, last ? scale : nullptr, logn, s0, b, first ? 1 : 0, 0);
         hipError_t e = hipGetLastError();
         if (e != hipSuccess) return zkc_fail(ctx, ZKC_ERR_HIP, std::string("zkc_ntt_pass: ") + hipGetErrorString(e));
         s0 += b; first = false;
diff --git a/zk-franchise-proof-circuit_amd/csrc/zkc_pass_plan.h b/zk-franchise-proof-circuit_amd/csrc/zkc_pass_plan.h
--- a/zk-franchise-proof-circuit_amd/csrc/zkc_pass_plan.h
+++ b/zk-franchise-proof-circuit_amd/csrc/zkc_pass_plan.h
@@ -92,6 +92,35 @@
     return {{w, nullptr, nv, p.oA, nv, 0}, {w, nullptr, nv, p.oB1, nv, 0}, {w + 8ull * (np + 1), nullptr, nc, p.oC, nc, 0}};
 }
 
+struct CRowsIn {
+    int mode;
+    uint32_t beta_milli;
+    bool wide_table;
+    bool abc_folded, early;
+    uint32_t k;
+    int logn;
+    size_t section_entries;
+    size_t cap_p_words;
+};
+inline bool c_rows_rule(uint32_t k, int nw_h, uint32_t n, int logn, uint32_t beta_milli) { return (uint64_t)k * (uint64_t)nw_h * 1000u <= (uint64_t)beta_milli * n * (uint64_t)logn; }
+inline bool c_rows_candidate(const KeyShape& key, const PassShape& p, int nb, const CRowsIn& in) {
+    if (in.mode == 0 || !in.wide_table || !in.abc_folded || in.early || p.tree || nb <= 2) return false;
+    return in.mode == 2 || c_rows_rule(in.k, msm_nw(key.c_h), key.n, in.logn, in.beta_milli);
+}
+inline bool c_rows(const KeyShape& key, const PassShape& p, int nb, const LaneCaps& cap, const CRowsIn& in) {
+    if (!c_rows_candidate(key, p, nb, in)) return false;
+    const int nw_h = msm_nw(key.c_h);
+    if (in.section_entries + (size_t)nb * nw_h * ((size_t)key.n + in.k) > cap.w1_entries) return false;
+    if ((size_t)nb * 16 * key.n > in.cap_p_words) return false;
+    return true;
+}
+inline std::vector<uint32_t> h_vmap(uint32_t n, const uint32_t* crows, uint32_t k) {
+    std::vector<uint32_t> v((size_t)n + k);
+    for (uint32_t i = 0; i < n; i++) v[i] = i;
+    for (uint32_t i = 0; i < k; i++) v[(size_t)n + i] = n + crows[i];
+    return v;
+}
+
 struct StreamOrder {
     bool mv_prefetch;
     bool mv_done;
diff --git a/zk-franchise-proof-circuit_amd/csrc/zkc_prove.hip b/zk-franchise-proof-circuit_amd/csrc/zkc_prove.hip
--- a/zk-franchise-proof-circuit_amd/csrc/zkc_prove.hip
+++ b/zk-franchise-proof-circuit_amd/csrc/zkc_prove.hip
@@ -12,17 +12,17 @@
 
 using namespace zkc;
 
-void zkc::matvec_launch(zkc_zkey* zk, Fr* d_abc, Fr* d_wm, const uint32_t* d_wtns0, int nb, hipStream_t mv, const zkc_zkey::Fold::AbcRows* al) {
+void zkc::matvec_launch(zkc_zkey* zk, Fr* d_abc, Fr* d_wm, const uint32_t* d_wtns0, int nb, hipStream_t mv, const zkc_zkey::Fold::AbcRows* al, bool c_rows) {
     const uint32_t n = zk->n, nv = zk->nVars;
     const bool units = zk->n_unit_coeffs > 0 && nv <= 3 * (size_t)n && sw::on<sw::ZKC_MATVEC_UNITS>();
     const Fr* wm = units ? (const Fr*)d_wm : (const Fr*)nullptr;
     if (al) {
-        const uint32_t per = 6 * n;
-        hipLaunchKernelGGL(zkc_abc_fill, dim3((per + 1023) / 1024, nb), dim3(256), 0, mv, (const uint4*)zk->fold.d_abc_tmpl, (uint4*)d_abc, per);
+        const uint32_t stride = 6 * n, per = c_rows ? 4 * n : stride;
+        hipLaunchKernelGGL(zkc_abc_fill, dim3((per + 1023) / 1024, nb), dim3(256), 0, mv, (const uint4*)zk->fold.d_abc_tmpl, (uint4*)d_abc, per, stride);
         if (units && al->nW) hipLaunchKernelGGL(zkc_wtns_mont_list, dim3((al->nW + 255) / 256, nb), dim3(256), 0, mv, (const Fr*)d_wtns0, (size_t)nv, d_wm, 3 * (size_t)n, al->d + al->offW, al->nW);
         if (al->nrows) hipLaunchKernelGGL(zkc_matvec_jds, dim3((al->nrows + 63 * al->nlong + 255) / 256, nb), dim3(256), 0, mv, zk->d_perm, zk->d_rowlen, zk->d_jdptr, zk->d_col, zk->d_val,
                                           (const Fr*)d_wtns0, (size_t)nv, d_abc, (int)n, al->nlong, wm, 3 * (size_t)n, (const uint32_t*)al->d, al->nrows);
-        if (al->nC) hipLaunchKernelGGL(zkc_pointwise_mul, dim3((al->nC + 255) / 256, nb), dim3(256), 0, mv, d_abc, (int)n, (const uint32_t*)(al->d + al->offC), al->nC);
+        if (al->nC && !c_rows) hipLaunchKernelGGL(zkc_pointwise_mul, dim3((al->nC + 255) / 256, nb), dim3(256), 0, mv, d_abc, (int)n, (const uint32_t*)(al->d + al->offC), al->nC);
         return;
     }
     if (units) hipLaunchKernelGGL(zkc_wtns_mont, dim3((nv + 255) / 256, nb), dim3(256), 0, mv, (const Fr*)d_wtns0, (size_t)nv, d_wm, 3 * (size_t)n, nv);
@@ -60,7 +60,8 @@
     const uint32_t n = zk->n, nv = zk->nVars; const int NWS = msm_nw(zk->c_sec), NWB = msm_nw(zk->c_h);
     const size_t per_proof_entries = (size_t)NWS * 3 * nv + (size_t)NWB * n;
     const size_t per_proof_buckets = 3 * (size_t)msm_half(std::max(zk->c_sec, zk->c_deep)) + msm_half(zk->c_h);
-    LaneNeed nd; nd.abc = 3 * (size_t)n * inflight; nd.p = 8 * (size_t)n * inflight; nd.fin = finalize_scratch_bytes(inflight); nd.bs = 2 * 2 * 8 * (size_t)nv;
+    LaneNeed nd; nd.abc = 3 * (size_t)n * inflight; nd.fin = finalize_scratch_bytes(inflight); nd.bs = 2 * 2 * 8 * (size_t)nv;
+    nd.p = (zk->h_rows == 2 * n ? 16 : 8) * (size_t)n * inflight;
     nd.e1 = per_proof_entries * inflight; nd.b1 = per_proof_buckets * inflight; nd.j1 = 4 * inflight;
     nd.e2 = (size_t)NWS * nv * inflight; nd.b2 = (size_t)msm_half(std::max(zk->c_sec, zk->c_deep)) * inflight; nd.j2 = inflight;
     return nd;
@@ -225,16 +226,18 @@
     zk->c_h = std::max(zk->c_h, std::max(zk->c_sec, zk->c_deep));
     const int NWB = msm_nw(zk->c_h);
     zk->offA = 0; zk->offB1 = NWS * nv; zk->offC = 2 * NWS * nv; zk->offH = 2 * NWS * nv + NWS * nc;
+    zk->c_rows_mode = (int)sw::value<sw::ZKC_C_ROWS>(1); zk->c_rows_beta = (uint32_t)sw::value<sw::ZKC_C_ROWS_BETA>(120);
+    zk->h_rows = (zk->c_rows_mode != 0 && !zk->fold.abc_cls.empty() && zk->logn >= 12 && (uint64_t)NWB * 2 * n < (1ull << 23) && !sw::on<sw::ZKC_NTT_SEPARATE>()) ? 2 * n : n;
     const int NWD = zk->c_deep ? msm_nw(zk->c_deep) : 0;
-    zk->offA_deep = zk->offH + NWB * n; zk->offB1_deep = zk->offA_deep + NWD * nv; zk->offC_deep = zk->offB1_deep + NWD * nv;
-    const size_t g1_points = (size_t)NWS * (2 * (size_t)nv + nc) + (size_t)NWB * n + (size_t)NWD * (2 * (size_t)nv + nc);
+    zk->offA_deep = zk->offH + NWB * zk->h_rows; zk->offB1_deep = zk->offA_deep + NWD * nv; zk->offC_deep = zk->offB1_deep + NWD * nv;
+    const size_t g1_points = (size_t)NWS * (2 * (size_t)nv + nc) + (size_t)NWB * zk->h_rows + (size_t)NWD * (2 * (size_t)nv + nc);
     if (g1_points >= (1ull << 31)) return bail(zkc_fail(ctx, ZKC_ERR_FORMAT, "zkey too large for 31-bit point indices"));
     if ((rc = dmalloc(ctx, &zk->d_g1, g1_points)) || (rc = dmalloc(ctx, &zk->d_g2, (size_t)NWS * nv))) return bail(rc);
     ZKC_UP(zk->d_g1 + zk->offA, sec[5], 64ull * nv); ZKC_UP(zk->d_g1 + zk->offB1, sec[6], 64ull * nv);
     ZKC_UP(zk->d_g1 + zk->offC, sec[8], 64ull * nc); ZKC_UP(zk->d_g1 + zk->offH, sec[9], 64ull * n);
     ZKC_UP(zk->d_g2, sec[7], 128ull * nv);
     if ((rc = msm_precompute_g1(ctx, nv, zk->d_g1 + zk->offA, zk->c_sec)) || (rc = msm_precompute_g1(ctx, nv, zk->d_g1 + zk->offB1, zk->c_sec)) ||
-        (rc = msm_precompute_g1(ctx, nc, zk->d_g1 + zk->offC, zk->c_sec)) || (rc = msm_precompute_g1(ctx, n, zk->d_g1 + zk->offH, zk->c_h)) ||
+        (rc = msm_precompute_g1(ctx, nc, zk->d_g1 + zk->offC, zk->c_sec)) || (rc = msm_precompute_g1(ctx, n, zk->d_g1 + zk->offH, zk->c_h, zk->h_rows)) ||
         (rc = msm_precompute_g2(ctx, nv, zk->d_g2, zk->c_sec))) return bail(rc);
     if ((rc = dmalloc(ctx, &zk->d_g2_29, G2ROW_WORDS * (size_t)NWS * nv)) || (rc = msm_g2_table29(ctx, zk->d_g2, zk->d_g2_29, (size_t)NWS * nv))) return bail(rc);
     if (zk->c_deep) {
@@ -300,25 +303,33 @@
     return ZKC_OK;
 }
 
-static int h_matvec_dev(zkc_zkey* zk, zkc_lane& L, const uint32_t* d_wtns0, int nb, hipStream_t mv, const zkc_zkey::Fold::AbcRows* al = nullptr) {
+static int h_matvec_dev(zkc_zkey* zk, zkc_lane& L, const uint32_t* d_wtns0, int nb, hipStream_t mv, const zkc_zkey::Fold::AbcRows* al = nullptr, bool c_rows = false) {
     zkc_ctx* ctx = zk->ctx; const uint32_t n = zk->n, nv = zk->nVars;
     zkc_prof_scope _ps(ctx, ZKC_PROF_MATVEC, (uint64_t)nb * ((uint64_t)zk->nCoeffs * 68 + 3ull * n * 32), mv);
-    matvec_launch(zk, L.d_abc, L.d_t, d_wtns0, nb, mv, al);
+    matvec_launch(zk, L.d_abc, L.d_t, d_wtns0, nb, mv, al, c_rows);
+    if (c_rows && al->nC) hipLaunchKernelGGL(zkc_c_rows_delta, dim3((al->nC + 255) / 256, nb), dim3(256), 0, mv, (const Fr*)L.d_abc, (const Fr*)(zk->fold.d_abc_tmpl + 2 * (size_t)n), L.d_p, (int)n,
+                                             (const uint32_t*)(al->d + al->offC), al->nC);
     ZKC_HIP_CHECK(ctx, hipGetLastError());
     return ZKC_OK;
 }
-static int h_evals_dev(zkc_zkey* zk, zkc_lane& L, hipStream_t st, const uint32_t* d_wtns0, int nb, bool with_matvec = true, const zkc_zkey::Fold::AbcRows* al = nullptr) {
+static int h_evals_dev(zkc_zkey* zk, zkc_lane& L, hipStream_t st, const uint32_t* d_wtns0, int nb, bool with_matvec = true, const zkc_zkey::Fold::AbcRows* al = nullptr, bool c_rows = false) {
     zkc_ctx* ctx = zk->ctx; const uint32_t n = zk->n;
-    if (with_matvec) { int rc0 = h_matvec_dev(zk, L, d_wtns0, nb, st, al); if (rc0) return rc0; }
+    if (c_rows && !(with_matvec && al && zk->fold.c_rows_ready)) return zkc_fail(ctx, ZKC_ERR_GENERIC, "h_evals_dev: a pass without C's transform pair needs its row lists and the key's tables (internal error)");
+    if (with_matvec) { int rc0 = h_matvec_dev(zk, L, d_wtns0, nb, st, al, c_rows); if (rc0) return rc0; }
+    const int nvec = c_rows ? 2 * nb : 3 * nb;
     zkc_prof_scope _pn(ctx, ZKC_PROF_NTT, (uint64_t)nb * (6ull * 2 * n * 32 + 4ull * n * 32), st);
     int rc;
     if (!sw::on<sw::ZKC_NTT_SEPARATE>() && zk->logn >= 12 && zk->logn <= 27) {
-        if ((rc = ntt_pair_run(ctx, st, L.d_abc, zk->d_tw_inv29, zk->d_tw_fwd29, zk->d_coset_br, (int)zk->logn, 3 * nb))) return rc;
+        if ((rc = ntt_pair_run(ctx, st, L.d_abc, zk->d_tw_inv29, zk->d_tw_fwd29, zk->d_coset_br, (int)zk->logn, nvec, c_rows))) return rc;
+        zk->fold.ntt_vectors += (uint64_t)nvec;
     } else {
-        if ((rc = ntt_run(ctx, st, L.d_abc, L.d_t, zk->d_tw_inv29, zk->d_coset, (int)zk->logn, 3 * nb))) return rc;
-        if ((rc = ntt_run(ctx, st, L.d_t, L.d_abc, zk->d_tw_fwd29, nullptr, (int)zk->logn, 3 * nb))) return rc;
-    }
-    hipLaunchKernelGGL(zkc_join_abc, dim3((n + 255) / 256, nb), dim3(256), 0, st, L.d_abc, L.d_p, (int)n);
+        if (c_rows) return zkc_fail(ctx, ZKC_ERR_GENERIC, "h_evals_dev: the two-transform form has no A / B only pass (internal error)");
+        if ((rc = ntt_run(ctx, st, L.d_abc, L.d_t, zk->d_tw_inv29, zk->d_coset, (int)zk->logn, nvec))) return rc;
+        if ((rc = ntt_run(ctx, st, L.d_t, L.d_abc, zk->d_tw_fwd29, nullptr, (int)zk->logn, nvec))) return rc;
+        zk->fold.ntt_vectors += (uint64_t)nvec;
+    }
+    if (c_rows) hipLaunchKernelGGL(zkc_join_abc_ct, dim3((n + 255) / 256, nb), dim3(256), 0, st, (const Fr*)L.d_abc, (const Fr*)zk->fold.d_c_hat, L.d_p, (int)n);
+    else hipLaunchKernelGGL(zkc_join_abc, dim3((n + 255) / 256, nb), dim3(256), 0, st, L.d_abc, L.d_p, (int)n);
     ZKC_HIP_CHECK(ctx, hipGetLastError());
     return ZKC_OK;
 }
@@ -353,11 +364,30 @@
     if (count != full) return zkc_fail(ctx, ZKC_ERR_BAD_ARG, "zkc_msm_debug: count must equal the section size");
     static thread_local MsmJobList jl; jl.clear(256, 1024, which == 2 ? (uint32_t)MSM_MAX_VW_PER_JOB : (uint32_t)MSM_MAX_VW_G1);
     const uint32_t offs[5] = {zk->offA, zk->offB1, 0, zk->offC, zk->offH};
-    jl.add((const uint32_t*)d_scalars, nullptr, count, offs[which], full, 0, which == 4 ? zk->c_h : zk->c_sec);
+    jl.add((const uint32_t*)d_scalars, nullptr, count, offs[which], which == 4 ? zk->h_rows : full, 0, which == 4 ? zk->c_h : zk->c_sec);
     int rc = which == 2 ? msm_pass_g2(zk, L0.w2, jl, 0, true, st_l0) : msm_pass_g1(zk, L0.w1, jl, 0, true, st_l0); if (rc) return rc;
     ZKC_HIP_CHECK(ctx, hipStreamSynchronize(st_l0));
     if (which == 2) wr_g2_std((uint8_t*)host_out, xyzz_to_affine(*(G2XYZZ*)L0.w2.h_results));
     else wr_g1_std((uint8_t*)host_out, xyzz_to_affine(*(G1XYZZ*)L0.w1.h_results));
+    return ZKC_OK;
+}
+
+extern "C" int zkc_debug_c_rows(zkc_zkey* zk, int what, uint32_t first, uint32_t count, void* host_out) {
+    if (!zk || !host_out || what < 0 || what > 2) return ZKC_ERR_BAD_ARG;
+    zkc_ctx* ctx = zk->ctx; const uint32_t n = zk->n;
+    ZKC_LOCK(ctx);
+    if (what == 2) { const uint64_t v[4] = {zk->fold.ntt_vectors, zk->fold.c_rows_passes, zk->fold.old_passes, zk->fold.c_rows_ready ? 1u : 0u}; memcpy(host_out, v, sizeof v); return ZKC_OK; }
+    if (zk->nLevels < 0 || zk->fold.abc_cls.empty()) return zkc_fail(ctx, ZKC_ERR_BAD_ARG, "zkc_debug_c_rows: not a census key whose buildABC folds");
+    ZKC_HIP_CHECK(ctx, hipSetDevice(ctx->device)); ZKC_HIP_CHECK(ctx, hipStreamSynchronize(ctx->stream));
+    int rc; if ((rc = fold_prepare(zk))) return rc;
+    uint32_t* tmpl = zkc_get_template(ctx, zk->nLevels); if (!tmpl) return ZKC_ERR_HIP;
+    if ((rc = abc_template(zk, tmpl))) return rc;
+    if (what == 1) { ZKC_HIP_CHECK(ctx, hipMemcpy(host_out, zk->fold.d_abc_tmpl, 96ull * n, hipMemcpyDeviceToHost)); return ZKC_OK; }
+    if (zk->h_rows != 2 * n || first >= n || count > n - first) return zkc_fail(ctx, ZKC_ERR_BAD_ARG, "zkc_debug_c_rows: no wide H table on this key, or points outside it");
+    if ((rc = c_rows_prepare(zk))) return rc;
+    std::vector<G1Affine> pts(count);
+    ZKC_HIP_CHECK(ctx, hipMemcpy(pts.data(), zk->d_g1 + zk->offH + n + first, (size_t)count * sizeof(G1Affine), hipMemcpyDeviceToHost));
+    for (uint32_t i = 0; i < count; i++) wr_g1_std((uint8_t*)host_out + 64 * (size_t)i, pts[i]);
     return ZKC_OK;
 }
 
@@ -508,12 +538,25 @@
         if (mv_done) ZKC_HIP_CHECK(ctx, hipStreamWaitEvent(st, LN.ev_mv, 0));
         zkc_zkey::Fold::AbcRows ar; const bool abc_fold = fold && !mv_done && !zk->fold.abc_cls.empty() && zk->fold.d_abc_tmpl != nullptr;
         if (abc_fold) { int Dc = 0, Ds = 0; for (int q = 0; q < nb; q++) { Dc = std::max(Dc, (int)dcq[q]); Ds = std::max(Ds, (int)dsq[q]); } if ((rc = abc_rows(zk, Dc, Ds, &ar))) return rc; }
-        if ((rc = h_evals_dev(zk, LN, st, w0, nb, !mv_done, abc_fold ? &ar : nullptr))) return rc;
+        bool c_rows = false; uint32_t* d_hv = nullptr;
+        if (abc_fold && zk->c_rows_mode != 0 && zk->h_rows == 2 * n) {
+            plan::CRowsIn ci{zk->c_rows_mode, zk->c_rows_beta, true, true, early, ar.nC, (int)zk->logn, 0, LN.cap_p};
+            if (plan::c_rows_candidate(KS, PS, nb, ci)) {
+                for (int q = 0; q < nb; q++) { zkc_zkey::Fold::VMap v0; if ((rc = fold_vmap(zk, 0, dcq[q], 0, dsq[q], &v0))) return rc; ci.section_entries += (size_t)msm_nw(KS.c_sec) * ((size_t)v0.nA + v0.nB + v0.nC); }
+                c_rows = plan::c_rows(KS, PS, nb, plan::LaneCaps{LN.w1.max_entries, LN.w1.max_buckets, LN.w1.max_jobs, LN.w2.max_entries}, ci);
+            }
+            if (c_rows) { d_hv = ar.d_hv; if ((rc = c_rows_prepare(zk))) return rc; }
+        }
+        if (fold) (c_rows ? zk->fold.c_rows_passes : zk->fold.old_passes)++;
+        if ((rc = h_evals_dev(zk, LN, st, w0, nb, !mv_done, abc_fold ? &ar : nullptr, c_rows))) return rc;
         if (st2 != st || SO.mv_prefetch) ZKC_HIP_CHECK(ctx, hipEventRecord(LN.ev_ntt, st));
         tr[2] = now_ms();
         static thread_local MsmJobList j1, j2;
         j1.clear(PS.vws, PS.vwb, MSM_MAX_VW_G1); j2.clear(PS.vw_g2, 1024, MSM_MAX_VW_PER_JOB);
-        for (int q = 0; q < nb; q++) j1.add(LN.d_p + 8 * (size_t)n * q, nullptr, n, zk->offH, n, 0, zk->c_h);
+        for (int q = 0; q < nb; q++) {
+            if (c_rows) j1.add(LN.d_p + 16 * (size_t)n * q, d_hv, n + ar.nC, zk->offH, zk->h_rows, 0, zk->c_h);
+            else j1.add(LN.d_p + 8 * (size_t)n * q, nullptr, n, zk->offH, zk->h_rows, 0, zk->c_h);
+        }
         auto add = [](MsmJobList& jl, const uint32_t* scalars, const plan::SectionView& v, int c) { jl.add(scalars, v.vmap, v.count, v.tbl_off, v.tbl_count, v.pt_shift, c); };
         BlindArgs ba{}; ba.rs = CS.d_rs + 64 * (size_t)p0; ba.nv = nv;
         for (int q = 0; q < nb; q++) {
diff --git a/zk-franchise-proof-circuit_amd/csrc/zkc_prover.h b/zk-franchise-proof-circuit_amd/csrc/zkc_prover.h
--- a/zk-franchise-proof-circuit_amd/csrc/zkc_prover.h
+++ b/zk-franchise-proof-circuit_amd/csrc/zkc_prover.h
@@ -169,6 +169,7 @@
     uint32_t* d_g2_29 = nullptr;
     uint32_t* d_g2_29_lone = nullptr;
     uint32_t offA = 0, offB1 = 0, offC = 0, offH = 0;
+    uint32_t h_rows = 0; int c_rows_mode = 1; uint32_t c_rows_beta = 120;
     int c_deep = 0; uint32_t offA_deep = 0, offB1_deep = 0, offC_deep = 0; uint32_t* d_g2_29_deep = nullptr;
     int c_h = zkc::MSM_C_BIG;
     int c_sec = zkc::MSM_C_SMALL;
@@ -206,8 +207,11 @@
         bool ready = false;
         std::vector<zkc::abc::RowClass> abc_cls; std::vector<uint32_t> abc_rowptr, abc_col, abc_perm;
         zkc::Fr* d_abc_tmpl = nullptr;
-        struct AbcRows { uint32_t* d = nullptr; uint32_t nrows = 0, nlong = 0, offC = 0, nC = 0, offW = 0, nW = 0; };
+        struct AbcRows { uint32_t* d = nullptr; uint32_t nrows = 0, nlong = 0, offC = 0, nC = 0, offW = 0, nW = 0;
+                         uint32_t* d_hv = nullptr; };
         std::map<std::pair<int, int>, AbcRows> abc_rows;
+        zkc::Fr* d_c_hat = nullptr; bool c_rows_ready = false;
+        uint64_t ntt_vectors = 0, c_rows_passes = 0, old_passes = 0;
         struct Top {
             int K = 0; uint32_t nslots = 0;
             zkc::TopCheckArgs args{};
@@ -227,7 +231,7 @@
 int ntt_twiddle_tables(zkc_ctx* ctx, int logn, bool keep_fr, TwiddleTables* out, bool with_29 = true);
 int msm_g2_window_table29(zkc_ctx* ctx, const G2Affine* d_bases, uint32_t count, int c, const char* what, uint32_t** out);
 int msm_g2_rows29(zkc_ctx* ctx, const G2Affine* d_points, size_t n, const char* what, uint32_t** out);
-int ntt_pair_run(zkc_ctx* ctx, hipStream_t st, Fr* data, const uint32_t* tw_inv29, const uint32_t* tw_fwd29, const Fr* scale_br, int logn, int nvec);
+int ntt_pair_run(zkc_ctx* ctx, hipStream_t st, Fr* data, const uint32_t* tw_inv29, const uint32_t* tw_fwd29, const Fr* scale_br, int logn, int nvec, bool ab_only = false);
 int ntt_bitrev_table(zkc_ctx* ctx, const Fr* d_src, Fr** out, int logn);
 int msm_work_alloc(zkc_ctx* ctx, MsmWork& w, size_t max_entries, size_t max_buckets, int max_jobs, bool g2);
 void msm_work_free(MsmWork& w);
@@ -250,7 +254,8 @@
 int top_seed(zkc_zkey* zk, const uint32_t* w0, const std::vector<plan::TopSeed>& seeds);
 int abc_template(zkc_zkey* zk, const uint32_t* tmpl);
 int abc_rows(zkc_zkey* zk, int Dc, int Ds, zkc_zkey::Fold::AbcRows* out);
-void matvec_launch(zkc_zkey* zk, Fr* d_abc, Fr* d_wm, const uint32_t* d_wtns0, int nb, hipStream_t mv, const zkc_zkey::Fold::AbcRows* al = nullptr);
+int c_rows_prepare(zkc_zkey* zk);
+void matvec_launch(zkc_zkey* zk, Fr* d_abc, Fr* d_wm, const uint32_t* d_wtns0, int nb, hipStream_t mv, const zkc_zkey::Fold::AbcRows* al = nullptr, bool c_rows = false);
 int prove_batch_begin(zkc_zkey* zk, int cs, const void* d_wtns, uint32_t nWitness, int B, const uint8_t* rs, bool want_publics, const void* d_inputs, int32_t* d_status,
                       int lane0 = -1, hipEvent_t wait_first = nullptr, const uint8_t* host_depths = nullptr, bool no_early = false);
 int prove_batch_finish(zkc_zkey* zk, int cs, uint8_t* proofs, uint8_t* publics);
@@ -258,7 +263,8 @@
 int zkey_load_opts(zkc_ctx* ctx, const void* zkey_bytes, size_t len, int nlanes, int max_inflight, zkc_zkey** out);
 size_t zkey_device_bytes(const zkc_zkey* zk, size_t* tables, size_t* work);
 size_t finalize_scratch_bytes(int nproofs);
-int msm_precompute_g1(zkc_ctx* ctx, uint32_t count, G1Affine* d_table, int c);
+int msm_precompute_g1(zkc_ctx* ctx, uint32_t count, G1Affine* d_table, int c, size_t window_stride = 0);
+int g1_scale_each(zkc_ctx* ctx, const G1Affine* tbl, const uint32_t* d_scalars, const uint32_t* d_wires, uint32_t nw, G1XYZZ* d_out);
 int msm_precompute_g2(zkc_ctx* ctx, uint32_t count, G2Affine* d_table, int c);
 int msm_g2_table29(zkc_ctx* ctx, const G2Affine* d_table, uint32_t* d_out, size_t count);
 int fold_group_sums_g1(zkc_ctx* ctx, const G1Affine* tbl, const uint32_t* d_scalars, const uint32_t* d_wires, uint32_t nw, int32_t pt_shift,
diff --git a/zk-franchise-proof-circuit_amd/csrc/zkc_switches.h b/zk-franchise-proof-circuit_amd/csrc/zkc_switches.h
--- a/zk-franchise-proof-circuit_amd/csrc/zkc_switches.h
+++ b/zk-franchise-proof-circuit_amd/csrc/zkc_switches.h
@@ -51,6 +51,8 @@
     X(ZKC_MATVEC_UNITS,         OFF_IF_ZERO, ANY, ANY,   PROCESS, "=0: buildABC multiplies by its +-1 coefficients instead of adding the wire")                                   \
     X(ZKC_ABC_FOLD,             OFF_IF_ZERO, ANY, ANY,   PROCESS, "=0: buildABC of a folded pass computes every row instead of copying the voter-independent ones from the template") \
     X(ZKC_TOP_FOLD,             NUMBER,      0,   12,    LIVE,    "key load: census tree levels below the root whose MSM terms are summed once per subtree instead of per voter (8; 0: off)") \
+    X(ZKC_C_ROWS,               NUMBER,      0,   2,     LIVE,    "key load: a folded pass leaves out the transform pair of C and adds its voter rows of C to the H job: 0 never, 2 wherever it is legal, 1 or unset by the rule k nw_H <= beta n log2 n") \
+    X(ZKC_C_ROWS_BETA,          NUMBER,      0,   100000, LIVE,   "key load: beta of that rule in thousandths (120)")                                                             \
     X(ZKC_MATVEC_INLINE,        SET,        ANY, ANY,   PROCESS, "set (any value, 0 included): buildABC of the next pass is not prefetched on the blinding stream")              \
     X(ZKC_MV_PREFETCH_AT_NTT,   ON_IF_ONE,   ANY, ANY,   PROCESS, "=1: that prefetch starts beside the pass' bucketing instead of beside its accumulation")                       \
     X(ZKC_EARLY_LAYOUT,         OFF_IF_ZERO, ANY, ANY,   PROCESS, "=0: one-pass calls of more than two voters wait for their fold flags instead of reading the depths off the inputs") \
```
